# vita-epfl/motion-style-transfer

Hardware: AMD Instinct MI355X
Metric: trajectories/sec fwd+bwd (Y-Net+LoRA, SDD shortterm) (higher is better)
Workload: dtype f32; 1 GPU; C2: SDD shortterm Y-Net + LoRA rank=1 on encoder[0-4], 256x256 raster, obs=8 pred=12; batch_per_gpu=32, global_batch=32, raster=256x256, obs_len=8, pred_len=12, train_net=mosa_1, parallelism=dp1, trainable_floats=8190

## Files before the change

include/ynet_hip.h:

```cpp
#ifndef YNET_HIP_H
#define YNET_HIP_H

#ifdef __cplusplus
extern "C" {
#endif

int ynet_abi_version(void);
const char* ynet_last_error(void);

long long ynet_packed_weight_floats(int cout, int cin, int K, int mode);
int ynet_pack_weight(const float* w, float* wp, int cout, int cin, int K, int mode, void* stream);

long long ynet_conv2d_workspace_floats(int B, int H, int W, int cout);
int ynet_conv2d(const float* const* src, const int* src_c, const long long* src_bs, const int* src_bmod, int nsrc,
                const float* mask, long long mask_bs, const float* wp, const float* bias,
                float* const* dst, const int* dst_c, const long long* dst_bs, int ndst,
                int B, int H, int W, int K, int relu, float* workspace, long long workspace_floats,
                void* stream);
int ynet_conv2d_pool_supported(int B, int H, int W, int cout, int K);
int ynet_conv2d_pool(const float* const* src, const int* src_c, const long long* src_bs, int nsrc, const float* wp, const float* bias,
                     float* dst, int cout, long long dst_bs, float* pooled, long long pooled_bs,
                     int B, int H, int W, int K, int relu, void* stream);
int ynet_conv2d_dgrad_relu_supported(int B, int H, int W, int dx_c, int K);
int ynet_conv2d_dgrad_relu(const float* dy, int dy_c, long long dy_bs, const float* mask, long long mask_bs, const float* wp,
                           float* dx, int dx_c, long long dx_bs, const float* relu_of, long long relu_of_bs,
                           int B, int H, int W, int K, float* workspace, long long workspace_floats, void* stream);
int ynet_conv2d_add_supported(int B, int H, int W, int cout, int K);
int ynet_conv2d_add(const float* const* src, const int* src_c, const long long* src_bs, const int* src_bmod, int nsrc,
                    const float* wp, const float* bias, float* dst, int cout, long long dst_bs,
                    int B, int H, int W, int K, int relu, const float* addend, long long addend_bs, int addend_bmod,
                    void* stream);

long long ynet_conv2d_relu_bits_words(int B, int H, int W, int cout, int K);
int ynet_conv2d_relu_bits(const float* const* src, const int* src_c, const long long* src_bs, int nsrc, const float* wp, const float* bias,
                          float* dst, int cout, long long dst_bs, unsigned* bits, int B, int H, int W, int K, void* stream);
int ynet_conv2d_dgrad_relu_bits(const float* dy, int dy_c, long long dy_bs, const float* mask, long long mask_bs, const float* wp,
                                float* dx, int dx_c, long long dx_bs, const unsigned* bits, int B, int H, int W, int K, void* stream);

int ynet_conv2d_winograd_supported(int B, int H, int W, int cin, int cout, int K);
long long ynet_winograd_filter_floats(int cin, int cout);
int ynet_winograd_filter(const float* wp, float* u, int cin, int cout, int col0, int cols_total, void* stream);
int ynet_conv2d_winograd(const float* src, long long src_bs, const float* u, const float* bias, float* dst, long long dst_bs, int cin, int cout,
                         int B, int H, int W, int relu, void* stream);
int ynet_conv2d_winograd_s2d(const float* src, long long src_bs, const float* u, float* dst, long long dst_bs, int cin, int cout, int B, int H, int W, void* stream);
int ynet_conv2d_winograd_pred_bce_supported(int B, int H, int W, int cin, int cout, int pred_cout, int kernlen);
int ynet_conv2d_winograd_pred_bce_blob(const float* src, long long src_bs, const float* u, const float* bias, const float* pred_wp, const float* pred_bias, int pred_cout,
                                       const float* target_xy, const float* blob, int kernlen, int S, float* logits, float* loss, float* dx, long long dx_bs,
                                       void* workspace, int B, int H, int W, float expected_grad, void* stream);
int ynet_conv2d_winograd_split_supported(int B, int H, int W, int cin);
int ynet_conv2d_winograd_split(const float* src, long long src_bs, const float* u, float* dst0, long long dst0_bs, int dst0_s2d, float* dst1, long long dst1_bs, int cin,
                               int B, int H, int W, void* stream);
int ynet_conv2d_winograd_dgrad_relu(const float* dy, long long dy_bs, const float* u, float* dx, long long dx_bs, const float* relu_of, long long relu_of_bs,
                                    int dy_c, int dx_c, int B, int H, int W, void* stream);
int ynet_conv2d_winograd_cat_supported(int B, int H, int W, const int* src_c, int nsrc, int cout, int K);
long long ynet_winograd_filter_cat_floats(const int* src_c, int nsrc, int cout);
int ynet_winograd_filter_cat(const float* wp, float* u, const int* src_c, int nsrc, int cout, int col0, int cols_total, void* stream);
int ynet_conv2d_winograd_cat(const float* const* src, const int* src_c, const long long* src_bs, int nsrc, const float* u, const float* bias, float* dst,
                             long long dst_bs, int cout, int B, int H, int W, int relu, void* stream);
int ynet_conv2d_winograd_cat_add(const float* const* src, const int* src_c, const long long* src_bs, int nsrc, const float* u, const float* bias, float* dst,
                                 long long dst_bs, int cout, int B, int H, int W, int relu, const float* addend, long long addend_bs, int addend_bmod,
                                 void* stream);
int ynet_conv2d_winograd_cat_pool(const float* const* src, const int* src_c, const long long* src_bs, int nsrc, const float* u, const float* bias, float* dst,
                                  long long dst_bs, float* pooled, long long pooled_bs, int cout, int B, int H, int W, int relu, void* stream);
int ynet_conv2d_winograd_cat_pool_code(const float* const* src, const int* src_c, const long long* src_bs, int nsrc, const float* u, const float* bias, float* dst,
                                       long long dst_bs, float* pooled, long long pooled_bs, unsigned char* code, int B, int H, int W, void* stream);
long long ynet_winograd_relu_bits_words(int B, int H, int W);
int ynet_conv2d_winograd_relu_bits(const float* src, long long src_bs, const float* u, const float* bias, float* dst, long long dst_bs, int cin, int B, int H, int W,
                                   unsigned* bits_out, void* stream);
int ynet_conv2d_winograd_cat_relu_bits(const float* const* src, const int* src_c, const long long* src_bs, int nsrc, const float* u, const float* bias, float* dst,
                                       long long dst_bs, int B, int H, int W, const float* addend, long long addend_bs, int addend_bmod, unsigned* bits_out,
                                       void* stream);
int ynet_conv2d_winograd_dgrad_relu_bits(const float* dy, long long dy_bs, const float* u, float* dx, long long dx_bs, const unsigned* bits, int dy_c, int B, int H,
                                         int W, void* stream);
int ynet_conv2d_winograd16_supported(int B, int H, int W, const int* src_c, int nsrc, int cout, int K);
long long ynet_winograd16_filter_floats(const int* src_c, int nsrc, int cout);
int ynet_winograd16_filter(const float* wp, float* u, const int* src_c, int nsrc, int cout, int col0, int cols_total, void* stream);
int ynet_conv2d_winograd16(const float* const* src, const int* src_c, const long long* src_bs, int nsrc, const float* u, const float* bias, float* dst,
                           long long dst_bs, int cout, int B, int H, int W, int relu, const float* relu_of, long long relu_of_bs, const float* addend,
                           long long addend_bs, int addend_bmod, float* pooled, long long pooled_bs, void* stream);
int ynet_upsample2x_conv2d_winograd_supported(int B, int H, int W, int cin, int cout, int K);
int ynet_upsample2x_conv2d_winograd(const float* src, long long src_bs, const float* u, const float* bias, float* dst, long long dst_bs, int cin, int cout, int B,
                                    int H, int W, int relu, void* stream);

#define YNET_AUTO_NO_WINOGRAD 1u
#define YNET_AUTO_NO_WINOGRAD16 2u
#define YNET_AUTO_WINOGRAD16_FOR_16 4u
#define YNET_AUTO_NO_POOL_CODE 8u
#define YNET_AUTO_NO_RELU_WBITS 16u
#define YNET_AUTO_NO_SPLIT48 32u
#define YNET_AUTO_UPCONV_BWD 64u
typedef struct YnetConvAuto {
    const float* src[4];
    int src_c[4];
    long long src_bs[4];
    int src_bmod[4];
    int nsrc;
    const float* mask;
    long long mask_bs;
    const float* wp;
    const float* bias;
    float* dst[4];
    int dst_c[4];
    long long dst_bs[4];
    int ndst;
    int B, H, W, K, relu;
    int upsample2x;
    const float* relu_of;
    long long relu_of_bs;
    float* pooled;
    long long pooled_bs;
    unsigned char* pool_code;
    const float* addend;
    long long addend_bs;
    int addend_bmod;
    unsigned* bits_out;
    const unsigned* relu_bits;
    unsigned* wbits_out;
    const unsigned* relu_wbits;
    float* cache;
    long long cache_floats;
    unsigned long long* cache_tag;
    unsigned long long wp_version;
    float* workspace;
    long long workspace_floats;
    unsigned flags;
    int dst_s2d[4];
} YnetConvAuto;
typedef struct YnetConvTaken {
    int family;
    int variant;
    int nlaunch;
    int tmpl[4][3];
    int wrote_wbits, wrote_pool_code, transformed;
    int wrote_s2d;
} YnetConvTaken;
long long ynet_conv2d_auto_cache_floats(const YnetConvAuto* desc);
long long ynet_conv2d_auto_workspace_floats(const YnetConvAuto* desc);
int ynet_conv2d_auto(const YnetConvAuto* desc, YnetConvTaken* taken, void* stream);
int ynet_conv2d_auto_plan(const YnetConvAuto* desc, YnetConvTaken* taken);

long long ynet_upconv_tables_floats(int cout, int cin, long long* keff_floats, long long* table_floats);
int ynet_upconv_tables(const float* w, int cout, int cin, float* keff_packed, float* tables, void* stream);
int ynet_upconv_dgrad_ring(const float* D, long long d_bs, const float* tables, const float* relu_of, long long relu_of_bs, float* dx, long long dx_bs,
                           int B, int C4, int cin, int h, int w, void* stream);

int ynet_conv2d_plan(int B, int H, int W, int cout, int K);

long long ynet_conv2d_wgrad_workspace_floats(int B, int H, int W, int cout, int cin, int K);
int ynet_conv2d_wgrad(const float* const* src, const int* src_c, const long long* src_bs, int nsrc,
                      const float* dy, long long dy_bs, const float* mask, long long mask_bs,
                      float* dw, float* db, float* workspace, int B, int H, int W, int cout, int K,
                      void* stream);

int ynet_lora_compose(const float* w, const float* lora_a, const float* lora_b, float scale, float* w_eff,
                      int cout, int cin, int K, int r, void* stream);
int ynet_lora_grad(const float* dw, const float* lora_a, const float* lora_b, float scale, float* d_a, float* d_b,
                   int cout, int cin, int K, int r, void* stream);

int ynet_lora_compose_pack(const float* w, const float* lora_a, const float* lora_b, float scale, float* wp_fwd,
                           float* wp_dgrad, int cout, int cin, int K, int r, void* stream);
int ynet_lora_compose_pack_multi(int n, const float* const* w, const float* const* lora_a, const float* const* lora_b,
                                 const float* scale, float* const* wp_fwd, float* const* wp_dgrad, const int* cout,
                                 const int* cin, const int* K, const int* r, void* stream);

int ynet_lora_conv2d_wgrad_supported(int cin, int cout, int K, int r, int W);
int ynet_lora_conv2d_wgrad_preferred(int cin, int cout, int K, int r, int W);
long long ynet_lora_conv2d_wgrad_workspace_floats(int cin, int cout);
int ynet_lora_conv2d_wgrad(const float* const* src, const int* src_c, const long long* src_bs, int nsrc,
                           const float* dy, long long dy_batch_stride, const float* mask, long long mask_batch_stride,
                           const float* lora_a, const float* lora_b, float scale, float* d_a, float* d_b,
                           float* workspace, int B, int H, int W, int cout, int K, int r, void* stream);

int ynet_maxpool2_fwd(const float* x, float* y, long long N, int H, int W, void* stream);
int ynet_maxpool2_bwd(const float* x, const float* dy, float* dx, long long N, int H, int W, void* stream);
int ynet_maxpool2_bwd_add(const float* x, const float* dy, const float* add0, const float* add1, float* dx, long long N,
                          int H, int W, int relu_mask, void* stream);
int ynet_maxpool2_bwd_add_code(const unsigned char* code, const float* dy, const float* add0, const float* add1, float* dx, long long N, int H, int W,
                               int relu_mask, void* stream);
int ynet_upsample2x_fwd(const float* x, float* y, long long N, int H, int W, void* stream);
int ynet_upsample2x_bwd(const float* dy, float* dx, long long N, int H, int W, void* stream);
int ynet_upsample2x_bwd_relu(const float* dy, float* dx, const float* relu_of, long long N, int H, int W, void* stream);
int ynet_avgpool_pyramid(const float* x, float* const* outs, int nlev, long long N, int H, int W, void* stream);

long long ynet_batchnorm_workspace_doubles(int C);
int ynet_batchnorm2d_fwd(const float* x, float* y, const float* gamma, const float* beta, float* running_mean, float* running_var, float* save_mean, float* save_invstd,
                         double* workspace, int B, int C, long long HW, int train, double momentum, double eps, void* stream);
int ynet_batchnorm2d_bwd(const float* dy, const float* x, const float* mean, const float* invstd, const float* gamma, float* dx, float* dgamma, float* dbeta, double* workspace,
                         int B, int C, long long HW, int train, void* stream);
int ynet_add_relu(const float* a, const float* b, float* y, long long n, int relu, void* stream);
int ynet_relu_bwd(const float* dy, const float* y, float* dx, long long n, void* stream);

long long ynet_bce_workspace_bytes(void);
int ynet_bce_logits_fwd(const float* x, const float* t, long long n, float* loss, void* workspace, void* stream);
int ynet_bce_logits_bwd(const float* x, const float* t, const float* grad_out, float* dx, long long n, void* stream);
int ynet_bce_logits_fwd_grad(const float* x, const float* t, long long n, float expected_grad, float* loss, float* dx,
                             void* workspace, void* stream);
int ynet_bce_grad_rescale(float* dx, const float* grad_out, float expected_grad, long long n, void* stream);
// ... 78 lines not shown
```

motion-style-transfer_amd/_lib.py:

```python
import ctypes
import os
import re

_HERE = os.path.dirname(os.path.abspath(__file__))
LIB_PATH = os.environ.get("YNET_HIP_LIB") or os.path.join(_HERE, "csrc", "libynet_hip.so")
HEADER_PATH = os.path.join(os.path.dirname(_HERE), "include", "ynet_hip.h")

c_fp = ctypes.c_void_p
c_i = ctypes.c_int
c_ll = ctypes.c_longlong
c_f = ctypes.c_float
PP = ctypes.POINTER(ctypes.c_void_p)
PI = ctypes.POINTER(ctypes.c_int)
PLL = ctypes.POINTER(ctypes.c_longlong)

class ConvAuto(ctypes.Structure):
    _fields_ = [("src", c_fp * 4), ("src_c", c_i * 4), ("src_bs", c_ll * 4), ("src_bmod", c_i * 4), ("nsrc", c_i),
                ("mask", c_fp), ("mask_bs", c_ll), ("wp", c_fp), ("bias", c_fp),
                ("dst", c_fp * 4), ("dst_c", c_i * 4), ("dst_bs", c_ll * 4), ("ndst", c_i),
                ("B", c_i), ("H", c_i), ("W", c_i), ("K", c_i), ("relu", c_i), ("upsample2x", c_i),
                ("relu_of", c_fp), ("relu_of_bs", c_ll), ("pooled", c_fp), ("pooled_bs", c_ll), ("pool_code", c_fp),
                ("addend", c_fp), ("addend_bs", c_ll), ("addend_bmod", c_i),
                ("bits_out", c_fp), ("relu_bits", c_fp), ("wbits_out", c_fp), ("relu_wbits", c_fp),
                ("cache", c_fp), ("cache_floats", c_ll), ("cache_tag", ctypes.POINTER(ctypes.c_ulonglong)), ("wp_version", ctypes.c_ulonglong),
                ("workspace", c_fp), ("workspace_floats", c_ll), ("flags", ctypes.c_uint), ("dst_s2d", c_i * 4)]


class ConvTaken(ctypes.Structure):
    _fields_ = [("family", c_i), ("variant", c_i), ("nlaunch", c_i), ("tmpl", (c_i * 3) * 4), ("wrote_wbits", c_i), ("wrote_pool_code", c_i),
                ("transformed", c_i), ("wrote_s2d", c_i)]


AUTO_NO_WINOGRAD, AUTO_NO_WINOGRAD16, AUTO_WINOGRAD16_FOR_16, AUTO_NO_POOL_CODE, AUTO_NO_RELU_WBITS, AUTO_NO_SPLIT48 = 1, 2, 4, 8, 16, 32
AUTO_UPCONV_BWD = 64

SIGNATURES = {
    "ynet_abi_version": (c_i, []),
    "ynet_last_error": (ctypes.c_char_p, []),
    "ynet_packed_weight_floats": (c_ll, [c_i, c_i, c_i, c_i]),
    "ynet_pack_weight": (c_i, [c_fp, c_fp, c_i, c_i, c_i, c_i, c_fp]),
    "ynet_conv2d_workspace_floats": (c_ll, [c_i, c_i, c_i, c_i]),
    "ynet_conv2d": (c_i, [PP, PI, PLL, PI, c_i, c_fp, c_ll, c_fp, c_fp, PP, PI, PLL, c_i,
                          c_i, c_i, c_i, c_i, c_i, c_fp, c_ll, c_fp]),
    "ynet_conv2d_pool_supported": (c_i, [c_i, c_i, c_i, c_i, c_i]),
    "ynet_conv2d_pool": (c_i, [PP, PI, PLL, c_i, c_fp, c_fp, c_fp, c_i, c_ll, c_fp, c_ll, c_i, c_i, c_i, c_i, c_i, c_fp]),
    "ynet_conv2d_dgrad_relu_supported": (c_i, [c_i, c_i, c_i, c_i, c_i]),
    "ynet_conv2d_dgrad_relu": (c_i, [c_fp, c_i, c_ll, c_fp, c_ll, c_fp, c_fp, c_i, c_ll, c_fp, c_ll, c_i, c_i, c_i, c_i, c_fp, c_ll, c_fp]),
    "ynet_conv2d_relu_bits_words": (c_ll, [c_i, c_i, c_i, c_i, c_i]),
    "ynet_conv2d_relu_bits": (c_i, [PP, PI, PLL, c_i, c_fp, c_fp, c_fp, c_i, c_ll, c_fp, c_i, c_i, c_i, c_i, c_fp]),
    "ynet_conv2d_dgrad_relu_bits": (c_i, [c_fp, c_i, c_ll, c_fp, c_ll, c_fp, c_fp, c_i, c_ll, c_fp, c_i, c_i, c_i, c_i, c_fp]),
    "ynet_conv2d_winograd_supported": (c_i, [c_i, c_i, c_i, c_i, c_i, c_i]),
    "ynet_winograd_filter_floats": (c_ll, [c_i, c_i]),
    "ynet_winograd_filter": (c_i, [c_fp, c_fp, c_i, c_i, c_i, c_i, c_fp]),
    "ynet_conv2d_winograd": (c_i, [c_fp, c_ll, c_fp, c_fp, c_fp, c_ll, c_i, c_i, c_i, c_i, c_i, c_i, c_fp]),
    "ynet_conv2d_winograd_s2d": (c_i, [c_fp, c_ll, c_fp, c_fp, c_ll, c_i, c_i, c_i, c_i, c_i, c_fp]),
    "ynet_conv2d_winograd_pred_bce_supported": (c_i, [c_i, c_i, c_i, c_i, c_i, c_i, c_i]),
    "ynet_conv2d_winograd_pred_bce_blob": (c_i, [c_fp, c_ll, c_fp, c_fp, c_fp, c_fp, c_i, c_fp, c_fp, c_i, c_i, c_fp, c_fp, c_fp, c_ll, c_fp, c_i, c_i, c_i,
                                                 c_f, c_fp]),
    "ynet_conv2d_winograd_split_supported": (c_i, [c_i, c_i, c_i, c_i]),
    "ynet_conv2d_winograd_split": (c_i, [c_fp, c_ll, c_fp, c_fp, c_ll, c_i, c_fp, c_ll, c_i, c_i, c_i, c_i, c_fp]),
    "ynet_upconv_dgrad_ring": (c_i, [c_fp, c_ll, c_fp, c_fp, c_ll, c_fp, c_ll, c_i, c_i, c_i, c_i, c_i, c_fp]),
    "ynet_upconv_tables_floats": (c_ll, [c_i, c_i, PLL, PLL]),
    "ynet_upconv_tables": (c_i, [c_fp, c_i, c_i, c_fp, c_fp, c_fp]),
    "ynet_conv2d_winograd_dgrad_relu": (c_i, [c_fp, c_ll, c_fp, c_fp, c_ll, c_fp, c_ll, c_i, c_i, c_i, c_i, c_i, c_fp]),
    "ynet_conv2d_winograd_cat_supported": (c_i, [c_i, c_i, c_i, PI, c_i, c_i, c_i]),
    "ynet_winograd_filter_cat_floats": (c_ll, [PI, c_i, c_i]),
    "ynet_winograd_filter_cat": (c_i, [c_fp, c_fp, PI, c_i, c_i, c_i, c_i, c_fp]),
    "ynet_conv2d_winograd_cat": (c_i, [PP, PI, PLL, c_i, c_fp, c_fp, c_fp, c_ll, c_i, c_i, c_i, c_i, c_i, c_fp]),
    "ynet_conv2d_winograd_cat_add": (c_i, [PP, PI, PLL, c_i, c_fp, c_fp, c_fp, c_ll, c_i, c_i, c_i, c_i, c_i, c_fp, c_ll, c_i, c_fp]),
    "ynet_conv2d_winograd_cat_pool": (c_i, [PP, PI, PLL, c_i, c_fp, c_fp, c_fp, c_ll, c_fp, c_ll, c_i, c_i, c_i, c_i, c_i, c_fp]),
    "ynet_conv2d_winograd_cat_pool_code": (c_i, [PP, PI, PLL, c_i, c_fp, c_fp, c_fp, c_ll, c_fp, c_ll, c_fp, c_i, c_i, c_i, c_fp]),
    "ynet_winograd_relu_bits_words": (c_ll, [c_i, c_i, c_i]),
    "ynet_conv2d_winograd_relu_bits": (c_i, [c_fp, c_ll, c_fp, c_fp, c_fp, c_ll, c_i, c_i, c_i, c_i, c_fp, c_fp]),
    "ynet_conv2d_winograd_cat_relu_bits": (c_i, [PP, PI, PLL, c_i, c_fp, c_fp, c_fp, c_ll, c_i, c_i, c_i, c_fp, c_ll, c_i, c_fp, c_fp]),
    "ynet_conv2d_winograd_dgrad_relu_bits": (c_i, [c_fp, c_ll, c_fp, c_fp, c_ll, c_fp, c_i, c_i, c_i, c_i, c_fp]),
    "ynet_upsample2x_conv2d_winograd_supported": (c_i, [c_i, c_i, c_i, c_i, c_i, c_i]),
    "ynet_upsample2x_conv2d_winograd": (c_i, [c_fp, c_ll, c_fp, c_fp, c_fp, c_ll, c_i, c_i, c_i, c_i, c_i, c_i, c_fp]),
    "ynet_conv2d_winograd16_supported": (c_i, [c_i, c_i, c_i, PI, c_i, c_i, c_i]),
    "ynet_winograd16_filter_floats": (c_ll, [PI, c_i, c_i]),
    "ynet_winograd16_filter": (c_i, [c_fp, c_fp, PI, c_i, c_i, c_i, c_i, c_fp]),
    "ynet_conv2d_winograd16": (c_i, [PP, PI, PLL, c_i, c_fp, c_fp, c_fp, c_ll, c_i, c_i, c_i, c_i, c_i, c_fp, c_ll, c_fp, c_ll, c_i, c_fp, c_ll, c_fp]),
    "ynet_conv2d_auto_cache_floats": (c_ll, [ctypes.POINTER(ConvAuto)]),
    "ynet_conv2d_auto_workspace_floats": (c_ll, [ctypes.POINTER(ConvAuto)]),
    "ynet_conv2d_auto": (c_i, [ctypes.POINTER(ConvAuto), ctypes.POINTER(ConvTaken), c_fp]),
    "ynet_conv2d_auto_plan": (c_i, [ctypes.POINTER(ConvAuto), ctypes.POINTER(ConvTaken)]),
    "ynet_conv2d_add_supported": (c_i, [c_i, c_i, c_i, c_i, c_i]),
    "ynet_conv2d_add": (c_i, [PP, PI, PLL, PI, c_i, c_fp, c_fp, c_fp, c_i, c_ll, c_i, c_i, c_i, c_i, c_i, c_fp, c_ll, c_i, c_fp]),
    "ynet_conv2d_plan": (c_i, [c_i, c_i, c_i, c_i, c_i]),
    "ynet_conv2d_wgrad_workspace_floats": (c_ll, [c_i, c_i, c_i, c_i, c_i, c_i]),
    "ynet_conv2d_wgrad": (c_i, [PP, PI, PLL, c_i, c_fp, c_ll, c_fp, c_ll, c_fp, c_fp, c_fp,
                                c_i, c_i, c_i, c_i, c_i, c_fp]),
    "ynet_lora_compose": (c_i, [c_fp, c_fp, c_fp, c_f, c_fp, c_i, c_i, c_i, c_i, c_fp]),
    "ynet_lora_grad": (c_i, [c_fp, c_fp, c_fp, c_f, c_fp, c_fp, c_i, c_i, c_i, c_i, c_fp]),
    "ynet_lora_conv2d_wgrad_supported": (c_i, [c_i, c_i, c_i, c_i, c_i]),
    "ynet_lora_conv2d_wgrad_preferred": (c_i, [c_i, c_i, c_i, c_i, c_i]),
    "ynet_lora_conv2d_wgrad_workspace_floats": (c_ll, [c_i, c_i]),
    "ynet_lora_conv2d_wgrad": (c_i, [PP, PI, PLL, c_i, c_fp, c_ll, c_fp, c_ll, c_fp, c_fp, c_f, c_fp, c_fp, c_fp,
                                     c_i, c_i, c_i, c_i, c_i, c_i, c_fp]),
    "ynet_lora_compose_pack": (c_i, [c_fp, c_fp, c_fp, c_f, c_fp, c_fp, c_i, c_i, c_i, c_i, c_fp]),
    "ynet_lora_compose_pack_multi": (c_i, [c_i, PP, PP, PP, ctypes.POINTER(c_f), PP, PP, PI, PI, PI, PI, c_fp]),
    "ynet_batch_sum": (c_i, [c_fp, c_fp, c_i, c_ll, c_ll, c_fp]),
    "ynet_adam_step": (c_i, [c_fp, c_fp, c_fp, c_i, c_i, ctypes.c_double, ctypes.c_double, ctypes.c_double, ctypes.c_double, ctypes.c_double,
                             c_i, c_fp]),
    "ynet_maxpool2_fwd": (c_i, [c_fp, c_fp, c_ll, c_i, c_i, c_fp]),
    "ynet_maxpool2_bwd": (c_i, [c_fp, c_fp, c_fp, c_ll, c_i, c_i, c_fp]),
    "ynet_maxpool2_bwd_add": (c_i, [c_fp, c_fp, c_fp, c_fp, c_fp, c_ll, c_i, c_i, c_i, c_fp]),
    "ynet_maxpool2_bwd_add_code": (c_i, [c_fp, c_fp, c_fp, c_fp, c_fp, c_ll, c_i, c_i, c_i, c_fp]),
    "ynet_upsample2x_fwd": (c_i, [c_fp, c_fp, c_ll, c_i, c_i, c_fp]),
# ... 86 lines not shown
```

motion-style-transfer_amd/csrc/conv_auto.cpp:

```cpp
#include "ynet_common.h"
#include "../../include/ynet_hip.h"
#include <stdint.h>
#include <string.h>

namespace {

struct Piece {
    float* ptr;
    int n;
    long long bs;
    int col0;
    int dst;
    int whole;
};

enum Kind { K_NONE = 0, K_WINO = 1, K_CAT = 2, K_W16 = 3 };

struct Launch {
    int kind;
    int row0;
    int cs[4], ncs;
    int cout, col0, ctot;
    long long floats;
    long long offset;
// ... 344 lines not shown
    if (a->flags & YNET_AUTO_UPCONV_BWD) return run_upconv_bwd(a, taken, stream);
    YNET_REQUIRE(a->nsrc >= 1 && a->nsrc <= 4 && a->ndst >= 1 && a->ndst <= 4 && a->wp, "conv2d_auto: 1..4 sources, 1..4 destinations and a packed filter are required");
    YNET_REQUIRE(a->B > 0 && a->H > 0 && a->W > 0 && (a->K == 1 || a->K == 3 || a->K == 5), "conv2d_auto: bad shape B %d %dx%d K %d", a->B, a->H, a->W, a->K);
    Plan p;
    if (int rc = make_plan(a, p)) return rc;
    YnetConvTaken t;
    memset(&t, 0, sizeof(t));
    t.family = p.family;
    t.variant = p.variant;
    if (p.nl) {
        YNET_REQUIRE(a->cache && a->cache_tag && a->cache_floats >= p.cache_floats && al(a->cache, 16),
                     "conv2d_auto: this launch keeps %lld floats of transformed filters (ynet_conv2d_auto_cache_floats): pass a 16-byte aligned cache of that size and its tag", p.cache_floats);
        const unsigned long long sig = signature(p);
        if (a->cache_tag[0] != sig || a->cache_tag[1] != a->wp_version) {
            if (int rc = transform(a, p, stream)) return rc;
            a->cache_tag[0] = sig;
            a->cache_tag[1] = a->wp_version;
            t.transformed = 1;
        }
    }
    return run_plan(a, p, t, taken, stream);
}

}

namespace {

int run_plan(const YnetConvAuto* a, const Plan& p, YnetConvTaken t, YnetConvTaken* taken, void* stream) {
    const int B = a->B, H = a->H, W = a->W, K = a->K, relu = a->relu ? 1 : 0;
    int ctot = 0;
    for (int i = 0; i < a->ndst; ++i) ctot += a->dst_c[i];
    const float* u0 = p.nl ? a->cache + p.l[0].offset : nullptr;
    const float* u1 = p.nl > 1 ? a->cache + p.l[1].offset : nullptr;
    auto done = [&](int rc) {
        if (!rc && taken) *taken = t;
        return rc;
    };
    auto tag = [&](int i, int x, int y, int z) {
        if (i < 4) { t.tmpl[i][0] = x; t.tmpl[i][1] = y; t.tmpl[i][2] = z; }
        t.nlaunch = i + 1;
    };
    float* ws = a->workspace_floats > 0 ? a->workspace : nullptr;
    const long long nws = ws ? a->workspace_floats : 0;

    switch (p.family) {
    case 4:
    case 5:
        tag(0, p.family == 4 ? 4 : 0, 0, 0);
        return done(ynet_upsample2x_conv2d_winograd(a->src[0], a->src_bs[0], u0, a->bias, a->dst[0], a->dst_bs[0], a->src_c[0], ctot, B, H, W, relu, stream));
    case 1: {
        if (p.variant == 23) {
            const Piece &q0 = p.pieces[0], &q1 = p.pieces[1];
            const int s2d = a->dst_s2d[q0.dst] ? 1 : 0;
            const int rc = ynet_conv2d_winograd_split(a->src[0], a->src_bs[0], u0, q0.ptr, q0.bs, s2d, q1.ptr, q1.bs, a->src_c[0], B, H, W, stream);
            if (rc) return rc;
            if (s2d) t.wrote_s2d |= 1 << q0.dst;
            tag(0, 3, a->src_c[0] / 8, s2d ? 6 : 5);
            return done(0);
        }
        const bool one32 = p.npieces == 1 && p.pieces[0].n == 32;
        unsigned* wb_out = (one32 && relu && !a->relu_of && !(a->flags & YNET_AUTO_NO_RELU_WBITS)) ? a->wbits_out : nullptr;
        const unsigned* wb_in = (one32 && a->relu_of && !relu && !a->bias && !(a->flags & YNET_AUTO_NO_RELU_WBITS)) ? a->relu_wbits : nullptr;
        const int em = wb_out ? 3 : (wb_in ? 2 : (a->relu_of ? 1 : 0));
        for (int i = 0; i < p.npieces; ++i) {
            const Piece& q = p.pieces[i];
            const float* u = a->cache + p.l[i].offset;
            const float* bias = a->bias ? a->bias + q.col0 : nullptr;
            int rc;
            const bool s2d = a->dst_s2d[q.dst] && q.whole && em == 0 && !a->bias && !relu;
            if (s2d) {
                rc = ynet_conv2d_winograd_s2d(a->src[0], a->src_bs[0], u, q.ptr, q.bs, a->src_c[0], q.n, B, H, W, stream);
                if (rc) return rc;
                t.wrote_s2d |= 1 << q.dst;
                tag(i, q.n / 16, a->src_c[0] / 8, 4);
                continue;
            }
            if (wb_out) rc = ynet_conv2d_winograd_relu_bits(a->src[0], a->src_bs[0], u, bias, q.ptr, q.bs, a->src_c[0], B, H, W, wb_out, stream);
            else if (wb_in) rc = ynet_conv2d_winograd_dgrad_relu_bits(a->src[0], a->src_bs[0], u, q.ptr, q.bs, wb_in, a->src_c[0], B, H, W, stream);
            else if (a->relu_of) {
                YNET_REQUIRE(!a->bias && !relu, "conv2d_auto: relu_of is for a data gradient (no bias, no ReLU)");
                rc = ynet_conv2d_winograd_dgrad_relu(a->src[0], a->src_bs[0], u, q.ptr, q.bs, a->relu_of, a->relu_of_bs, a->src_c[0], q.n, B, H, W, stream);
            } else rc = ynet_conv2d_winograd(a->src[0], a->src_bs[0], u, bias, q.ptr, q.bs, a->src_c[0], q.n, B, H, W, relu, stream);
            if (rc) return rc;
            tag(i, q.n / 16, a->src_c[0] / 8, em);
        }
        t.wrote_wbits = wb_out ? 1 : 0;
        return done(0);
    }
    case 2: {
        if (p.variant == 30) {
            unsigned* wb = (relu && !(a->flags & YNET_AUTO_NO_RELU_WBITS)) ? a->wbits_out : nullptr;
            tag(0, 2, wb ? 5 : 2, 0);
            t.wrote_wbits = wb ? 1 : 0;
            if (wb) return done(ynet_conv2d_winograd_cat_relu_bits(a->src, a->src_c, a->src_bs, a->nsrc, u0, a->bias, a->dst[0], a->dst_bs[0], B, H, W, a->addend, a->addend_bs, a->addend_bmod, wb, stream));
            return done(ynet_conv2d_winograd_cat_add(a->src, a->src_c, a->src_bs, a->nsrc, u0, a->bias, a->dst[0], a->dst_bs[0], 32, B, H, W, relu, a->addend, a->addend_bs, a->addend_bmod, stream));
        }
        if (p.variant == 10) {
            unsigned char* code = (relu && !(a->flags & YNET_AUTO_NO_POOL_CODE)) ? a->pool_code : nullptr;
            tag(0, 2, code ? 6 : 3, 0);
            t.wrote_pool_code = code ? 1 : 0;
            if (code) return done(ynet_conv2d_winograd_cat_pool_code(a->src, a->src_c, a->src_bs, a->nsrc, u0, a->bias, a->dst[0], a->dst_bs[0], a->pooled, a->pooled_bs, code, B, H, W, stream));
            return done(ynet_conv2d_winograd_cat_pool(a->src, a->src_c, a->src_bs, a->nsrc, u0, a->bias, a->dst[0], a->dst_bs[0], a->pooled, a->pooled_bs, 32, B, H, W, relu, stream));
        }
        unsigned* wb = (relu && !(a->flags & YNET_AUTO_NO_RELU_WBITS)) ? a->wbits_out : nullptr;
        t.wrote_wbits = wb ? 1 : 0;
        if (p.variant == 40) {
            const long long HW = (long long)H * W;
            int rc = ynet_conv2d_winograd(a->src[0], a->src_bs[0], u0, nullptr, a->dst[0], a->dst_bs[0], 32, 32, B, H, W, 0, stream);
            if (rc) return rc;
            const float* rs[4];
            int rc_[4], nr = 0;
            long long rb[4];
            if (a->src_c[0] > 32) { rs[nr] = a->src[0] + 32 * HW; rc_[nr] = a->src_c[0] - 32; rb[nr] = a->src_bs[0]; ++nr; }
            for (int i = 1; i < a->nsrc; ++i) { rs[nr] = a->src[i]; rc_[nr] = a->src_c[i]; rb[nr] = a->src_bs[i]; ++nr; }
            tag(0, 2, 4, 0);
            tag(1, 2, wb ? 5 : 2, 0);
            if (wb) return done(ynet_conv2d_winograd_cat_relu_bits(rs, rc_, rb, nr, u1, a->bias, a->dst[0], a->dst_bs[0], B, H, W, a->dst[0], a->dst_bs[0], 0, wb, stream));
            return done(ynet_conv2d_winograd_cat_add(rs, rc_, rb, nr, u1, a->bias, a->dst[0], a->dst_bs[0], 32, B, H, W, relu, a->dst[0], a->dst_bs[0], 0, stream));
        }
        tag(0, 2, wb ? 4 : 0, 0);
        if (wb) return done(ynet_conv2d_winograd_cat_relu_bits(a->src, a->src_c, a->src_bs, a->nsrc, u0, a->bias, a->dst[0], a->dst_bs[0], B, H, W, nullptr, 0, 0, wb, stream));
        return done(ynet_conv2d_winograd_cat(a->src, a->src_c, a->src_bs, a->nsrc, u0, a->bias, a->dst[0], a->dst_bs[0], 32, B, H, W, relu, stream));
    }
    case 3: {
// ... 63 lines not shown
                 !a->relu_wbits && !a->dst_s2d[0] && a->src_bmod[0] <= 0,
                 "conv2d_auto (upconv_bwd): relu_of is the only optional operand (no upsample2x, pooled, pool_code, addend, mask, bias, relu, bit masks, dst_s2d, batch modulus)");
    YNET_REQUIRE(a->K == 3 && a->src_c[0] >= 4 && (a->src_c[0] & 3) == 0 && a->dst_c[0] >= 1, "conv2d_auto (upconv_bwd): K 3, src_c[0] = 4 cout, dst_c[0] = cin (K %d, src_c %d, dst_c %d)",
                 a->K, a->src_c[0], a->dst_c[0]);
    YNET_REQUIRE(a->B > 0 && a->H >= 2 && a->W >= 2, "conv2d_auto (upconv_bwd): the low-resolution map must be at least 2 x 2 (B %d, %dx%d)", a->B, a->H, a->W);
    const int c4 = a->src_c[0], cin = a->dst_c[0];
    const long long hw = (long long)a->H * a->W;
    YNET_REQUIRE(a->src_bs[0] >= c4 * hw && a->dst_bs[0] >= cin * hw && (!a->relu_of || a->relu_of_bs >= cin * hw), "conv2d_auto (upconv_bwd): batch strides smaller than the images");
    YNET_REQUIRE((3ll * c4 * cin + c4 * 66ll + 256) * 4 <= 64 * 1024, "conv2d_auto (upconv_bwd): 4 cout %d x cin %d ring tables do not fit the ring kernel's LDS", c4, cin);
    memset(&u, 0, sizeof(u));
    u.cout = c4 / 4;
    u.cin = cin;
    long long kf = 0, tf = 0;
    YNET_REQUIRE(ynet_upconv_tables_floats(u.cout, cin, &kf, &tf) > 0, "conv2d_auto (upconv_bwd): bad shape cout %d cin %d", u.cout, cin);
    u.tab_off = (kf + 3) & ~3ll;
    u.wino_off = u.tab_off + ((tf + 3) & ~3ll);
    u.in = *a;
    u.in.flags &= ~YNET_AUTO_UPCONV_BWD;
    u.in.wp = a->cache;
    u.in.cache = a->cache ? a->cache + u.wino_off : nullptr;
    u.in.cache_floats = a->cache_floats - u.wino_off;
    u.in.cache_tag = nullptr;
    if (int rc = make_plan(&u.in, u.p)) return rc;
    u.cache_floats = u.wino_off + u.p.cache_floats;
    return 0;
}

int run_upconv_bwd(const YnetConvAuto* a, YnetConvTaken* taken, void* stream) {
    UpPlan u;
    if (int rc = make_up_plan(a, u)) return rc;
    YNET_REQUIRE(a->wp && a->src[0] && a->dst[0], "conv2d_auto (upconv_bwd): the raw filter [cout][cin][3][3], the source and the destination are required");
    YNET_REQUIRE(a->cache && a->cache_tag && a->cache_floats >= u.cache_floats && al(a->cache, 16),
                 "conv2d_auto (upconv_bwd): this call keeps %lld floats of effective filter, ring tables and transforms (ynet_conv2d_auto_cache_floats): pass a 16-byte aligned cache "
                 "of that size and its tag", u.cache_floats);
    YnetConvTaken t;
    memset(&t, 0, sizeof(t));
    t.family = u.p.family;
    t.variant = u.p.variant;
    unsigned long long sig = signature(u.p);
    for (long long v : {0x7570636f6e76ll, (long long)u.cout, (long long)u.cin}) {
        sig ^= (unsigned long long)v;
        sig *= 1099511628211ull;
    }
    sig = sig ? sig : 1;
    if (a->cache_tag[0] != sig || a->cache_tag[1] != a->wp_version) {
        if (int rc = ynet_upconv_tables(a->wp, u.cout, u.cin, a->cache, a->cache + u.tab_off, stream)) return rc;
        if (int rc = transform(&u.in, u.p, stream)) return rc;
        a->cache_tag[0] = sig;
        a->cache_tag[1] = a->wp_version;
        t.transformed = 1;
    }
    YnetConvTaken ti;
    if (int rc = run_plan(&u.in, u.p, t, &ti, stream)) return rc;
    if (int rc = ynet_upconv_dgrad_ring(a->src[0], a->src_bs[0], a->cache + u.tab_off, a->relu_of, a->relu_of_bs, a->dst[0], a->dst_bs[0], a->B, 4 * u.cout, u.cin, a->H, a->W,
                                        stream))
        return rc;
    ti.nlaunch += 1;
    if (taken) *taken = ti;
    return 0;
}

}
```

motion-style-transfer_amd/csrc/conv_wino.hip:

```cpp
#include "ynet_common.h"
#include "bce_element.h"
#include <math.h>
#include <stdlib.h>
#include <type_traits>

typedef float f32x2 __attribute__((ext_vector_type(2)));
typedef unsigned u32x2 __attribute__((ext_vector_type(2)));
typedef __attribute__((address_space(3))) void* lds_ptr_t;

#define WN_TH 16
#define WN_TW 32
#define WN_LQ 10
#define WN_ROWF 40
#define WN_PLANE_F 160
#define WN_SLOT_BYTES (320 * 16 + 16)
#define WN_RING_BYTES (2 * WN_SLOT_BYTES)
#define WN_THREADS 512

struct WinoArgs {
    const float* x;
    const f32x4* u;
    const float* bias;
    float* y;
    long long x_bs, y_bs;
    int B, H, W, relu, ntiles;
    const float* emask;
    long long emask_bs;
    unsigned* wbits;
    float* y2;
    long long y2_bs;
    const float* pw;
    const float* pb;
    int pco, pco_pad;
    const float* t_xy;
    const float* t_blob;
    int t_m, t_S;
    float* logits;
    double* partial;
    unsigned* ticket;
    float* loss;
    long long n_loss;
    float gs;
};

__device__ __forceinline__ f32x2 wn_v01(f32x2 tl, f32x2 th) {
    f32x2 r;
    asm("v_pk_add_f32 %0, %1, %2 op_sel_hi:[1,0] neg_lo:[0,1]" : "=v"(r) : "v"(tl), "v"(th));
    return r;
}
__device__ __forceinline__ f32x2 wn_v23(f32x2 tl, f32x2 th) {
    f32x2 r;
    asm("v_pk_add_f32 %0, %1, %2 op_sel:[1,0] op_sel_hi:[1,1] neg_lo:[1,0] neg_hi:[0,1]" : "=v"(r) : "v"(tl), "v"(th));
    return r;
}

template <int NCB, int EPI, int BITS = 0, bool S2D = false, int CB0 = 0, int CB1 = NCB>
__device__ __forceinline__ void wino_epilogue(f32x4 (&acc)[16][NCB], const f32x2 (&bias2)[NCB][2], float floor_v, __amdgpu_buffer_rsrc_t ry,
                                              __amdgpu_buffer_rsrc_t rm, unsigned st0, unsigned st1, unsigned so_t, unsigned sm_t, int HW, unsigned stp = 0,
                                              unsigned* wbits = nullptr, unsigned char* pcode = nullptr) {
    unsigned word = 0u;
    if constexpr (BITS == 2) word = *wbits;
#pragma unroll
    for (int cb = CB0; cb < CB1; ++cb) {
        constexpr int NB = CB1 - CB0;
        const int cd = cb - CB0;
        u32x2 mk[2][2][2];
        if constexpr (EPI == 1 || EPI == 2) {
#pragma unroll
            for (int h = 0; h < 2; ++h)
#pragma unroll
                for (int k = 0; k < 2; ++k) {
                    const unsigned sm = sm_t + (unsigned)((cd * 16 + 2 * h + k) * HW * 4);
                    mk[h][k][0] = __builtin_amdgcn_raw_buffer_load_b64(rm, st0, sm, 0);
                    mk[h][k][1] = __builtin_amdgcn_raw_buffer_load_b64(rm, st1, sm, 0);
                }
        }
#pragma unroll
        for (int h = 0; h < 2; ++h) {
            f32x2 m[16];
#pragma unroll
            for (int e = 0; e < 16; ++e)
                m[e] = h == 0 ? __builtin_shufflevector(acc[e][cb], acc[e][cb], 0, 1) : __builtin_shufflevector(acc[e][cb], acc[e][cb], 2, 3);
            m[5] = m[5] + bias2[cb][h];
            f32x2 r0[4], r1[4];
#pragma unroll
            for (int j = 0; j < 4; ++j) {
                r0[j] = m[j] + m[4 + j] + m[8 + j];
                r1[j] = m[4 + j] - m[8 + j] - m[12 + j];
            }
            const f32x2 o00 = r0[0] + r0[1] + r0[2], o01 = r0[1] - r0[2] - r0[3];
            const f32x2 o10 = r1[0] + r1[1] + r1[2], o11 = r1[1] - r1[2] - r1[3];
#pragma unroll
            for (int k = 0; k < 2; ++k) {
                f32x2 row0 = {o00[k], o01[k]}, row1 = {o10[k], o11[k]};
                if constexpr (EPI == 2) {
                    row0 += __builtin_bit_cast(f32x2, mk[h][k][0]);
                    row1 += __builtin_bit_cast(f32x2, mk[h][k][1]);
                }
                row0 = f32x2{row0[0] < floor_v ? floor_v : row0[0], row0[1] < floor_v ? floor_v : row0[1]};
                row1 = f32x2{row1[0] < floor_v ? floor_v : row1[0], row1[1] < floor_v ? floor_v : row1[1]};
                if constexpr (EPI == 1) {
                    const f32x2 m0 = __builtin_bit_cast(f32x2, mk[h][k][0]), m1 = __builtin_bit_cast(f32x2, mk[h][k][1]);
                    row0 = f32x2{m0[0] > 0.f ? row0[0] : 0.f, m0[1] > 0.f ? row0[1] : 0.f};
                    row1 = f32x2{m1[0] > 0.f ? row1[0] : 0.f, m1[1] > 0.f ? row1[1] : 0.f};
                }
                const int bit0 = ((cb * 2 + h) * 2 + k) * 4;
                if constexpr (BITS == 2) {
                    row0 = f32x2{(word >> bit0) & 1u ? row0[0] : 0.f, (word >> (bit0 + 1)) & 1u ? row0[1] : 0.f};
                    row1 = f32x2{(word >> (bit0 + 2)) & 1u ? row1[0] : 0.f, (word >> (bit0 + 3)) & 1u ? row1[1] : 0.f};
                }
                if constexpr (BITS == 1)
                    word |= (row0[0] > 0.f ? 1u << bit0 : 0u) | (row0[1] > 0.f ? 2u << bit0 : 0u) | (row1[0] > 0.f ? 4u << bit0 : 0u) | (row1[1] > 0.f ? 8u << bit0 : 0u);
                if constexpr (S2D) {
                    const unsigned hw = (unsigned)(HW >> 2), ph = (unsigned)(NB * 16) * hw * 4u;
                    const unsigned sc = so_t + (unsigned)(cd * 16 + 2 * h + k) * hw * 4u;
                    const float e00 = row0[0], e01 = row0[1], e10 = row1[0], e11 = row1[1];
                    const bool odd = __lane_id() & 1u;
                    const float g0 = __builtin_bit_cast(float, __builtin_amdgcn_update_dpp(0, __builtin_bit_cast(int, odd ? e00 : e01), 0xB1, 0xF, 0xF, false));
                    const float g1 = __builtin_bit_cast(float, __builtin_amdgcn_update_dpp(0, __builtin_bit_cast(int, odd ? e10 : e11), 0xB1, 0xF, 0xF, false));
                    const f32x2 p0 = odd ? f32x2{g0, e01} : f32x2{e00, g0}, p1 = odd ? f32x2{g1, e11} : f32x2{e10, g1};
                    const unsigned vo = st0 + (odd ? ph - 4u : 0u);
                    __builtin_amdgcn_raw_buffer_store_b64(__builtin_bit_cast(u32x2, p0), ry, vo, sc, 0);
                    __builtin_amdgcn_raw_buffer_store_b64(__builtin_bit_cast(u32x2, p1), ry, vo, sc + 2u * ph, 0);
                    continue;
                }
                const unsigned so = so_t + (unsigned)((cd * 16 + 2 * h + k) * HW * 4);
                __builtin_amdgcn_raw_buffer_store_b64(__builtin_bit_cast(u32x2, row0), ry, st0, so, 0);
                __builtin_amdgcn_raw_buffer_store_b64(__builtin_bit_cast(u32x2, row1), ry, st1, so, 0);
                if constexpr (EPI == 3) {
                    float pm = fmaxf(fmaxf(row0[0], row0[1]), fmaxf(row1[0], row1[1]));
                    if (__builtin_isunordered(row0[0], row0[1]) || __builtin_isunordered(row1[0], row1[1])) pm = __builtin_nanf("");
                    __builtin_amdgcn_raw_buffer_store_b32(__builtin_bit_cast(unsigned, pm), rm, stp, sm_t + (unsigned)((cd * 16 + 2 * h + k) * (HW >> 2) * 4), 0);
                    if constexpr (BITS == 3) {
                        float mx = row0[0];
                        unsigned arg = 0u;
                        if (row0[1] > mx || row0[1] != row0[1]) { mx = row0[1]; arg = 1u; }
                        if (row1[0] > mx || row1[0] != row1[0]) { mx = row1[0]; arg = 2u; }
                        if (row1[1] > mx || row1[1] != row1[1]) { mx = row1[1]; arg = 3u; }
                        const unsigned code = arg | (row0[0] > 0.f ? 4u : 0u) | (row0[1] > 0.f ? 8u : 0u) | (row1[0] > 0.f ? 16u : 0u) | (row1[1] > 0.f ? 32u : 0u);
                        pcode[(cd * 16 + 2 * h + k) * (HW >> 2)] = (unsigned char)code;
                    }
                }
            }
        }
    }
    if constexpr (BITS == 1) *wbits = word;
}

template <int MB, typename PosT>
__device__ __forceinline__ float wino_epilogue_pred(f32x4 (&acc)[16][2], const f32x2 (&bias2)[2][2], const f32x4* tab,
                                                    const WinoArgs& a, __amdgpu_buffer_rsrc_t rdx, __amdgpu_buffer_rsrc_t rlog, unsigned st_rm, unsigned so_rm, int b,
                                                    int py0, int px0, int kq, int H, int W, const float* blob_tab, const PosT* pos_lds) {
    const int HW = H * W;
    float yv[2][4][4];
#pragma unroll
    for (int cb = 0; cb < 2; ++cb)
#pragma unroll
        for (int h = 0; h < 2; ++h) {
            f32x2 m[16];
#pragma unroll
            for (int e = 0; e < 16; ++e)
                m[e] = h == 0 ? __builtin_shufflevector(acc[e][cb], acc[e][cb], 0, 1) : __builtin_shufflevector(acc[e][cb], acc[e][cb], 2, 3);
            m[5] = m[5] + bias2[cb][h];
            f32x2 r0[4], r1[4];
#pragma unroll
            for (int j = 0; j < 4; ++j) {
                r0[j] = m[j] + m[4 + j] + m[8 + j];
                r1[j] = m[4 + j] - m[8 + j] - m[12 + j];
            }
            const f32x2 o00 = r0[0] + r0[1] + r0[2], o01 = r0[1] - r0[2] - r0[3];
            const f32x2 o10 = r1[0] + r1[1] + r1[2], o11 = r1[1] - r1[2] - r1[3];
#pragma unroll
            for (int k = 0; k < 2; ++k) {
                const float v00 = o00[k], v01 = o01[k], v10 = o10[k], v11 = o11[k];
                yv[cb][2 * h + k][0] = v00 < 0.f ? 0.f : v00;
                yv[cb][2 * h + k][1] = v01 < 0.f ? 0.f : v01;
// ... 257 lines not shown
#pragma unroll
        for (int c = 0; c < NCH; ++c) {
            if (c + 1 < NCH || nxt < total_units) asm volatile("s_waitcnt vmcnt(5)" ::: "memory");
            else asm volatile("s_waitcnt vmcnt(0)" ::: "memory");
            const f32x4* wl = smem + c * WQ;
            const float* il = reinterpret_cast<const float*>(reinterpret_cast<const unsigned char*>(smem) + NCH * WQ * 16 + wave * WN_RING_BYTES +
                                                             (c & 1) * WN_SLOT_BYTES + 4);
#pragma unroll
            for (int s = 0; s < 2; ++s) {
                const float* ip = il + (s * 4 + kq) * WN_PLANE_F + 3 + 2 * n;
                f32x2 dl[4], dh[4];
#pragma unroll
                for (int r = 0; r < 4; ++r) {
                    dl[r] = *reinterpret_cast<const f32x2*>(ip + r * WN_ROWF);
                    dh[r] = *reinterpret_cast<const f32x2*>(ip + r * WN_ROWF + 2);
                }
                if (s == 1) {
                    asm volatile("s_waitcnt lgkmcnt(0)" ::: "memory");
                    if (c + 2 < NCH) dma_chunk(cur, c + 2);
                    else if (nxt < total_units) dma_chunk(nxt, c + 2 - NCH);
                }
                const f32x2 tl[4] = {dl[0] - dl[2], dl[1] + dl[2], dl[2] - dl[1], dl[1] - dl[3]};
                const f32x2 th[4] = {dh[0] - dh[2], dh[1] + dh[2], dh[2] - dh[1], dh[1] - dh[3]};
                f32x2 v01[4], v23[4];
#pragma unroll
                for (int i = 0; i < 4; ++i) {
                    v01[i] = wn_v01(tl[i], th[i]);
                    v23[i] = wn_v23(tl[i], th[i]);
                }
                asm volatile("s_nop 3" : "+v"(v01[0]), "+v"(v01[1]), "+v"(v01[2]), "+v"(v01[3]), "+v"(v23[0]), "+v"(v23[1]), "+v"(v23[2]), "+v"(v23[3]));
#pragma unroll
                for (int q = 0; q < 4; ++q) {
                    f32x4 w[NCB];
#pragma unroll
                    for (int cb = 0; cb < NCB; ++cb) w[cb] = wl[((s * 4 + q) * NCB + cb) * 64 + lane];
#pragma unroll
                    for (int e = 0; e < 4; ++e) {
                        const float bv = e < 2 ? v01[q][e] : v23[q][e - 2];
#pragma unroll
                        for (int cb = 0; cb < NCB; ++cb) {
                            const float av = w[cb][e];
                            if (c == 0 && s == 0) acc[q * 4 + e][cb] = __builtin_amdgcn_mfma_f32_16x16x4f32(av, bv, f32x4{0.f, 0.f, 0.f, 0.f}, 0, 0, 0);
                            else acc[q * 4 + e][cb] = __builtin_amdgcn_mfma_f32_16x16x4f32(av, bv, acc[q * 4 + e][cb], 0, 0, 0);
                        }
                    }
                }
            }
        }
        {
            const int t = tile_first + (cur >> 3) * gstride;
            const int tx = t % tiles_x, ty = (t / tiles_x) % tiles_y, b = t / (tiles_x * tiles_y);
            const unsigned so_s2d = (unsigned)(((ty * (WN_TH / 2) + (cur & 7)) * (W >> 1) + tx * (WN_TW / 2)) * 4);
            const unsigned so_rm = (unsigned)(((ty * WN_TH + 2 * (cur & 7)) * W + tx * WN_TW) * 4);
            if constexpr (EM == 7 || EM == 8) {
                static_assert((EM != 7 && EM != 8) || NCB == 2, "the predictor epilogue is the 32-channel launch's");
                const __amdgpu_buffer_rsrc_t rdx = __builtin_amdgcn_make_buffer_rsrc(a.y + (long long)b * a.y_bs, 0, y_img, 0x00020000);
                const __amdgpu_buffer_rsrc_t rlog =
                    __builtin_amdgcn_make_buffer_rsrc(a.logits + (long long)b * a.pco * HW, 0, (unsigned)(a.pco * HW * 4), 0x00020000);
                typedef typename std::conditional<EM == 7, int, short>::type PosT;
                const float* blob_lds = reinterpret_cast<const float*>(ptab + 5 * PMB * 64) + 2 * NW + 4;
                const float s_ = wino_epilogue_pred<PMB, PosT>(acc, bias2, ptab + lane, a, rdx, rlog, st_rm, so_rm, b, ty * WN_TH + 2 * (cur & 7), tx * WN_TW + 2 * n, kq, H, W,
                                                               blob_lds, reinterpret_cast<const PosT*>(blob_lds + a.t_m * a.t_m));
                acc_loss += (double)s_;
                cur = nxt;
                if (cur < total_units) nxt = next_unit();
                continue;
            }
            if constexpr (EM == 5 || EM == 6) {
                static_assert(EM < 5 || NCB == 3, "the two-destination epilogue is the 48-channel launch's");
                const __amdgpu_buffer_rsrc_t r0 = __builtin_amdgcn_make_buffer_rsrc(a.y + (long long)b * a.y_bs, 0, (unsigned)(16 * HW * 4), 0x00020000);
                const __amdgpu_buffer_rsrc_t r1 = __builtin_amdgcn_make_buffer_rsrc(a.y2 + (long long)b * a.y2_bs, 0, (unsigned)(32 * HW * 4), 0x00020000);
                if constexpr (EM == 6) wino_epilogue<NCB, 0, 0, true, 0, 1>(acc, bias2, floor_v, r0, r0, st_s2d, st_s2d, so_s2d, so_s2d, HW);
                else wino_epilogue<NCB, 0, 0, false, 0, 1>(acc, bias2, floor_v, r0, r0, st_rm, st_rm + (unsigned)(W * 4), so_rm, so_rm, HW);
                wino_epilogue<NCB, 0, 0, false, 1, 3>(acc, bias2, floor_v, r1, r1, st_rm, st_rm + (unsigned)(W * 4), so_rm, so_rm, HW);
                cur = nxt;
                if (cur < total_units) nxt = next_unit();
                continue;
            }
            const unsigned so_t = EM == 4 ? so_s2d : so_rm;
            const __amdgpu_buffer_rsrc_t ry = __builtin_amdgcn_make_buffer_rsrc(a.y + (long long)b * a.y_bs, 0, y_img, 0x00020000);
            const __amdgpu_buffer_rsrc_t rm =
                __builtin_amdgcn_make_buffer_rsrc(const_cast<float*>(EM == 1 ? a.emask + (long long)b * a.emask_bs : a.y), 0, y_img, 0x00020000);
            unsigned* wb = (EM == 2 || EM == 3) ? a.wbits + (((long long)b * (H >> 1) + (ty * (WN_TH / 2) + (cur & 7))) * tiles_x + tx) * 64 + lane : nullptr;
            wino_epilogue<NCB, EM == 1 ? 1 : 0, EM == 2 ? 2 : (EM == 3 ? 1 : 0), EM == 4>(acc, bias2, floor_v, ry, rm, st0, st1, so_t, so_t, HW, 0, wb);
        }
        cur = nxt;
        if (cur < total_units) nxt = next_unit();
    }
    if constexpr (EM == 7 || EM == 8) {
        double* wsd = reinterpret_cast<double*>(ptab + 5 * PMB * 64);
        unsigned* last = reinterpret_cast<unsigned*>(wsd + NW);
#pragma unroll
        for (int o = 32; o > 0; o >>= 1) acc_loss += __shfl_xor(acc_loss, o, 64);
        if (lane == 0) wsd[wave] = acc_loss;
        __syncthreads();
        if (tid == 0) {
            double t = 0.0;
            for (int i = 0; i < NW; ++i) t += wsd[i];
            a.partial[blockIdx.x] = t;
            __threadfence();
            *last = (atomicAdd(a.ticket, 1u) == gridDim.x - 1) ? 1u : 0u;
        }
        __syncthreads();
        if (*last) {
            __threadfence();
            double t = 0.0;
            for (unsigned i = tid; i < gridDim.x; i += NT) t += ((volatile double*)a.partial)[i];
#pragma unroll
            for (int o = 32; o > 0; o >>= 1) t += __shfl_xor(t, o, 64);
            if (lane == 0) wsd[wave] = t;
            __syncthreads();
            if (tid == 0) {
                double tt = 0.0;
                for (int i = 0; i < NW; ++i) tt += wsd[i];
                a.loss[0] = (float)(tt / (double)a.n_loss);
                *a.ticket = 0u;
            }
        }
    }
}

#define WC_SLOT_BYTES (160 * 16 + 16)
#define WC_RING_BYTES (2 * WC_SLOT_BYTES)
#define WC_MAX_SRC 3

struct WinoCatArgs {
    const float* x[WC_MAX_SRC];
    long long x_bs[WC_MAX_SRC];
    int x_c[WC_MAX_SRC];
    int nsrc, nchunks;
    const f32x4* u;
    const float* bias;
    float* y;
    long long y_bs;
    int B, H, W, relu, ntiles;
    const float* addend;
    long long addend_bs;
// ... 853 lines not shown
    static int cus_dev[YNET_MAX_DEV] = {0};
    const int slot = ynet_device_slot();
    if (!attr_dev[slot]) {
        (void)hipFuncSetAttribute(reinterpret_cast<const void*>(conv_wino_cat_kernel<2, 0>), hipFuncAttributeMaxDynamicSharedMemorySize, 14 * 8192 + 8 * WC_RING_BYTES + 16);
        (void)hipFuncSetAttribute(reinterpret_cast<const void*>(conv_wino_cat_kernel<2, 2>), hipFuncAttributeMaxDynamicSharedMemorySize, 14 * 8192 + 8 * WC_RING_BYTES + 16);
        (void)hipFuncSetAttribute(reinterpret_cast<const void*>(conv_wino_cat_kernel<2, 3>), hipFuncAttributeMaxDynamicSharedMemorySize, 14 * 8192 + 8 * WC_RING_BYTES + 16);
        (void)hipFuncSetAttribute(reinterpret_cast<const void*>(conv_wino_cat_kernel<2, 4>), hipFuncAttributeMaxDynamicSharedMemorySize, 14 * 8192 + 8 * WC_RING_BYTES + 16);
        (void)hipFuncSetAttribute(reinterpret_cast<const void*>(conv_wino_cat_kernel<2, 5>), hipFuncAttributeMaxDynamicSharedMemorySize, 14 * 8192 + 8 * WC_RING_BYTES + 16);
        (void)hipFuncSetAttribute(reinterpret_cast<const void*>(conv_wino_cat_kernel<2, 6>), hipFuncAttributeMaxDynamicSharedMemorySize, 14 * 8192 + 8 * WC_RING_BYTES + 16);
        int dev = 0, cus = 256;
        (void)hipGetDevice(&dev);
        (void)hipDeviceGetAttribute(&cus, hipDeviceAttributeMultiprocessorCount, dev);
        cus_dev[slot] = cus < 8 ? 8 : cus;
        attr_dev[slot] = true;
    }
    int grid = a.ntiles < cus_dev[slot] ? a.ntiles : cus_dev[slot];
    if (grid >= 8) grid &= ~7;
    if (wbits != nullptr && addend != nullptr) hipLaunchKernelGGL((conv_wino_cat_kernel<2, 5>), dim3(grid), dim3(WN_THREADS), lds, (hipStream_t)stream, a);
    else if (wbits != nullptr) hipLaunchKernelGGL((conv_wino_cat_kernel<2, 4>), dim3(grid), dim3(WN_THREADS), lds, (hipStream_t)stream, a);
    else if (addend != nullptr) hipLaunchKernelGGL((conv_wino_cat_kernel<2, 2>), dim3(grid), dim3(WN_THREADS), lds, (hipStream_t)stream, a);
    else if (pcode != nullptr) hipLaunchKernelGGL((conv_wino_cat_kernel<2, 6>), dim3(grid), dim3(WN_THREADS), lds, (hipStream_t)stream, a);
    else if (pool != nullptr) hipLaunchKernelGGL((conv_wino_cat_kernel<2, 3>), dim3(grid), dim3(WN_THREADS), lds, (hipStream_t)stream, a);
    else hipLaunchKernelGGL((conv_wino_cat_kernel<2, 0>), dim3(grid), dim3(WN_THREADS), lds, (hipStream_t)stream, a);
    return ynet_check_launch(what);
}

int ynet_conv2d_winograd_cat(const float* const* src, const int* src_c, const long long* src_bs, int nsrc, const float* u, const float* bias, float* dst,
                             long long dst_bs, int cout, int B, int H, int W, int relu, void* stream) {
    return wino_cat_launch(src, src_c, src_bs, nsrc, u, bias, dst, dst_bs, cout, B, H, W, relu, nullptr, 0, 0, nullptr, 0, stream, "conv2d_winograd_cat");
}

int ynet_conv2d_winograd_cat_add(const float* const* src, const int* src_c, const long long* src_bs, int nsrc, const float* u, const float* bias, float* dst,
                                 long long dst_bs, int cout, int B, int H, int W, int relu, const float* addend, long long addend_bs, int addend_bmod,
                                 void* stream) {
    YNET_REQUIRE(addend != nullptr, "conv2d_winograd_cat_add: the additive term is null");
    return wino_cat_launch(src, src_c, src_bs, nsrc, u, bias, dst, dst_bs, cout, B, H, W, relu, addend, addend_bs, addend_bmod, nullptr, 0, stream, "conv2d_winograd_cat_add");
}

int ynet_conv2d_winograd_cat_pool(const float* const* src, const int* src_c, const long long* src_bs, int nsrc, const float* u, const float* bias, float* dst,
                                  long long dst_bs, float* pooled, long long pooled_bs, int cout, int B, int H, int W, int relu, void* stream) {
    YNET_REQUIRE(pooled != nullptr, "conv2d_winograd_cat_pool: the pooled output is null");
    return wino_cat_launch(src, src_c, src_bs, nsrc, u, bias, dst, dst_bs, cout, B, H, W, relu, nullptr, 0, 0, pooled, pooled_bs, stream, "conv2d_winograd_cat_pool");
}

int ynet_conv2d_winograd_cat_pool_code(const float* const* src, const int* src_c, const long long* src_bs, int nsrc, const float* u, const float* bias, float* dst,
                                       long long dst_bs, float* pooled, long long pooled_bs, unsigned char* code, int B, int H, int W, void* stream) {
    YNET_REQUIRE(pooled != nullptr && code != nullptr, "conv2d_winograd_cat_pool_code: the pooled output or its code plane is null");
    return wino_cat_launch(src, src_c, src_bs, nsrc, u, bias, dst, dst_bs, 32, B, H, W, 1, nullptr, 0, 0, pooled, pooled_bs, stream, "conv2d_winograd_cat_pool_code",
                           nullptr, code);
}

static int wino_launch_any(const float* src, long long src_bs, const float* u, const float* bias, float* dst, long long dst_bs, const float* emask,
                           long long emask_bs, int cin, int cout, int B, int H, int W, int relu, void* stream, const char* what, unsigned* wbits = nullptr,
                           bool wbits_apply = false, bool s2d = false, float* dst2 = nullptr, long long dst2_bs = 0, int split_mode = 0) {
    YNET_REQUIRE(src && u && dst, "%s: null pointer", what);
    YNET_REQUIRE(wino_shape_ok(B, H, W, cin, cout, 3), "%s: shape B=%d %dx%d %d -> %d is not served (ask ynet_conv2d_winograd_supported)", what, B, H, W, cin,
                 cout);
    YNET_REQUIRE((reinterpret_cast<uintptr_t>(src) & 15) == 0 && (reinterpret_cast<uintptr_t>(dst) & 7) == 0 && (reinterpret_cast<uintptr_t>(u) & 15) == 0 &&
                     (src_bs & 3) == 0 && (dst_bs & 1) == 0,
                 "%s: planes must be 16-byte (input, filters) / 8-byte (output) aligned", what);
    const long long HW = (long long)H * W;
    YNET_REQUIRE((src_bs == 0 || src_bs >= cin * HW) && dst_bs >= (split_mode ? 16 : cout) * HW, "%s: batch strides smaller than the images (input: 0 = one image for the batch)", what);
    if (split_mode)
        YNET_REQUIRE(cout == 48 && dst2 != nullptr && (reinterpret_cast<uintptr_t>(dst2) & 7) == 0 && (dst2_bs & 1) == 0 && dst2_bs >= 32 * HW && bias == nullptr && !relu &&
                         wbits == nullptr && !s2d,
                     "%s: two destinations are for the plain 48-channel data gradient (16 + 32 planes, 8-byte aligned)", what);
    if (emask != nullptr)
        YNET_REQUIRE((reinterpret_cast<uintptr_t>(emask) & 7) == 0 && (emask_bs & 1) == 0 && emask_bs >= cout * HW,
                     "%s: the activation must be 8-byte aligned, its batch stride not smaller than the image", what);
    WinoArgs a{src, reinterpret_cast<const f32x4*>(u), bias, dst, src_bs, dst_bs, B, H, W, relu ? 1 : 0, B * (H / WN_TH) * (W / WN_TW), emask, emask_bs, wbits, dst2, dst2_bs};
    hipStream_t st = (hipStream_t)stream;
    if (wbits != nullptr) {
        YNET_REQUIRE(cout == 32 && emask == nullptr && (reinterpret_cast<uintptr_t>(wbits) & 3) == 0, "%s: the 1-bit mask serves 32 output channels and excludes the float mask", what);
        if (wbits_apply) return cin == 32 ? launch_wino<2, 4, 2>(a, st) : launch_wino<2, 2, 2>(a, st);
        return cin == 32 ? launch_wino<2, 4, 3>(a, st) : launch_wino<2, 2, 3>(a, st);
    }
    if (s2d) {
        YNET_REQUIRE(emask == nullptr && bias == nullptr && !relu, "%s: the space-to-depth store is for a plain data gradient", what);
        if (cout == 32) return cin == 32 ? launch_wino<2, 4, 4>(a, st) : launch_wino<2, 2, 4>(a, st);
        return cin == 32 ? launch_wino<1, 4, 4>(a, st) : launch_wino<1, 2, 4>(a, st);
    }
    if (cout == 48) {
        YNET_REQUIRE(emask == nullptr && cin == 32, "%s: the 48-channel form is plain, from 32 input channels", what);
        if (split_mode == 1) return launch_wino_nw<3, 4, 5, 4>(a, st);
        if (split_mode == 2) return launch_wino_nw<3, 4, 6, 4>(a, st);
        return launch_wino_nw<3, 4, 0, 4>(a, st);
    }
    if (emask != nullptr) {
        if (cout == 32) return cin == 32 ? launch_wino<2, 4, 1>(a, st) : launch_wino<2, 2, 1>(a, st);
        return cin == 32 ? launch_wino<1, 4, 1>(a, st) : launch_wino<1, 2, 1>(a, st);
    }
    if (cout == 32) return cin == 32 ? launch_wino<2, 4, 0>(a, st) : launch_wino<2, 2, 0>(a, st);
    return cin == 32 ? launch_wino<1, 4, 0>(a, st) : launch_wino<1, 2, 0>(a, st);
}

int ynet_conv2d_winograd(const float* src, long long src_bs, const float* u, const float* bias, float* dst, long long dst_bs, int cin, int cout,
                         int B, int H, int W, int relu, void* stream) {
    return wino_launch_any(src, src_bs, u, bias, dst, dst_bs, nullptr, 0, cin, cout, B, H, W, relu, stream, "conv2d_winograd");
}

int ynet_conv2d_winograd_s2d(const float* src, long long src_bs, const float* u, float* dst, long long dst_bs, int cin, int cout, int B, int H, int W, void* stream) {
    return wino_launch_any(src, src_bs, u, nullptr, dst, dst_bs, nullptr, 0, cin, cout, B, H, W, 0, stream, "conv2d_winograd_s2d", nullptr, false, true);
}

int ynet_conv2d_winograd_pred_bce_supported(int B, int H, int W, int cin, int cout, int pred_cout, int kernlen) {
    static const int on = getenv("YNET_CONV_PRED_BCE") ? atoi(getenv("YNET_CONV_PRED_BCE")) : 1;
    if (!(on && cin == 32 && cout == 32 && pred_cout >= 1 && pred_cout <= 32 && kernlen >= 1 && wino_shape_ok(B, H, W, cin, cout, 3))) return 0;
    const long long base = 4ll * 8 * 2 * 64 * 16 + 8ll * WN_RING_BYTES + 16 + 8 * 8 + 16;
    const long long lds = pred_cout <= 16 ? base + 5 * 64 * 16 + ((long long)kernlen * kernlen + 2ll * B * pred_cout) * 4
                                          : base + 10 * 64 * 16 + (long long)kernlen * kernlen * 4 + ((2ll * B * pred_cout * 2 + 15) & ~15ll);
    return lds <= 160 * 1024 ? 1 : 0;
}

int ynet_conv2d_winograd_pred_bce_blob(const float* src, long long src_bs, const float* u, const float* bias, const float* pred_wp, const float* pred_bias, int pred_cout,
                                       const float* target_xy, const float* blob, int kernlen, int S, float* logits, float* loss, float* dx, long long dx_bs,
                                       void* workspace, int B, int H, int W, float expected_grad, void* stream) {
    YNET_REQUIRE(src && u && pred_wp && target_xy && blob && logits && loss && dx && workspace, "conv2d_winograd_pred_bce_blob: null pointer");
    YNET_REQUIRE(ynet_conv2d_winograd_pred_bce_supported(B, H, W, 32, 32, pred_cout, kernlen), "conv2d_winograd_pred_bce_blob: B=%d %dx%d with %d predictor outputs and a %d x %d blob is not served (32 -> 32, <= 32 outputs, tables within LDS; ask ..._supported)",
                 B, H, W, pred_cout, kernlen, kernlen);
    YNET_REQUIRE(kernlen > 0 && kernlen <= S && S >= H && S >= W, "conv2d_winograd_pred_bce_blob: the target needs a blob table with 0 < kernlen <= S and S >= H, W (got kernlen %d, S %d, %dx%d)", kernlen, S, H, W);
    const long long HW = (long long)H * W;
    YNET_REQUIRE((reinterpret_cast<uintptr_t>(src) & 15) == 0 && (reinterpret_cast<uintptr_t>(u) & 15) == 0 && (reinterpret_cast<uintptr_t>(dx) & 7) == 0 &&
                     (reinterpret_cast<uintptr_t>(logits) & 7) == 0 && (src_bs & 3) == 0 && (dx_bs & 1) == 0 && (src_bs == 0 || src_bs >= 32 * HW) && dx_bs >= 32 * HW,
                 "conv2d_winograd_pred_bce_blob: planes must be 16-byte (input, filters) / 8-byte (outputs) aligned, batch strides not smaller than the images");
    WinoArgs a{src, reinterpret_cast<const f32x4*>(u), bias, dx, src_bs, dx_bs, B, H, W, 1, B * (H / WN_TH) * (W / WN_TW), nullptr, 0, nullptr, nullptr, 0};
    a.pw = pred_wp;
    a.pb = pred_bias;
    a.pco = pred_cout;
    a.pco_pad = ceil_div(pred_cout, 64) * 64;
    a.t_xy = target_xy;
    a.t_blob = blob;
    a.t_m = kernlen;
    a.t_S = S;
    a.logits = logits;
    a.partial = (double*)workspace;
    a.ticket = (unsigned*)((char*)workspace + 1024 * sizeof(double));
    a.loss = loss;
    a.n_loss = (long long)B * pred_cout * HW;
    a.gs = expected_grad / (float)a.n_loss;
    return pred_cout <= 16 ? launch_wino_nw<2, 4, 7, 8>(a, (hipStream_t)stream) : launch_wino_nw<2, 4, 8, 8>(a, (hipStream_t)stream);
}

int ynet_conv2d_winograd_split_supported(int B, int H, int W, int cin) { return (cin == 32 && wino_shape_ok(B, H, W, cin, 48, 3)) ? 1 : 0; }

int ynet_conv2d_winograd_split(const float* src, long long src_bs, const float* u, float* dst0, long long dst0_bs, int dst0_s2d, float* dst1, long long dst1_bs, int cin,
                               int B, int H, int W, void* stream) {
    return wino_launch_any(src, src_bs, u, nullptr, dst0, dst0_bs, nullptr, 0, cin, 48, B, H, W, 0, stream, "conv2d_winograd_split", nullptr, false, false, dst1, dst1_bs,
                           dst0_s2d ? 2 : 1);
}

long long ynet_winograd_relu_bits_words(int B, int H, int W) {
    if (B <= 0 || H % WN_TH || W % WN_TW) return 0;
    return (long long)B * (H / 2) * (W / WN_TW) * 64;
}

int ynet_conv2d_winograd_relu_bits(const float* src, long long src_bs, const float* u, const float* bias, float* dst, long long dst_bs, int cin, int B, int H,
                                   int W, unsigned* bits_out, void* stream) {
    YNET_REQUIRE(bits_out != nullptr, "conv2d_winograd_relu_bits: the mask output is null");
    return wino_launch_any(src, src_bs, u, bias, dst, dst_bs, nullptr, 0, cin, 32, B, H, W, 1, stream, "conv2d_winograd_relu_bits", bits_out, false);
}

int ynet_conv2d_winograd_cat_relu_bits(const float* const* src, const int* src_c, const long long* src_bs, int nsrc, const float* u, const float* bias, float* dst,
                                       long long dst_bs, int B, int H, int W, const float* addend, long long addend_bs, int addend_bmod, unsigned* bits_out,
                                       void* stream) {
    YNET_REQUIRE(bits_out != nullptr, "conv2d_winograd_cat_relu_bits: the mask output is null");
    return wino_cat_launch(src, src_c, src_bs, nsrc, u, bias, dst, dst_bs, 32, B, H, W, 1, addend, addend_bs, addend_bmod, nullptr, 0, stream,
                           "conv2d_winograd_cat_relu_bits", bits_out);
}

int ynet_conv2d_winograd_dgrad_relu_bits(const float* dy, long long dy_bs, const float* u, float* dx, long long dx_bs, const unsigned* bits, int dy_c, int B, int H,
                                         int W, void* stream) {
    YNET_REQUIRE(bits != nullptr, "conv2d_winograd_dgrad_relu_bits: the mask is null");
    return wino_launch_any(dy, dy_bs, u, nullptr, dx, dx_bs, nullptr, 0, dy_c, 32, B, H, W, 0, stream, "conv2d_winograd_dgrad_relu_bits", const_cast<unsigned*>(bits), true);
}

int ynet_conv2d_winograd_dgrad_relu(const float* dy, long long dy_bs, const float* u, float* dx, long long dx_bs, const float* relu_of, long long relu_of_bs,
                                    int dy_c, int dx_c, int B, int H, int W, void* stream) {
    YNET_REQUIRE(relu_of != nullptr, "conv2d_winograd_dgrad_relu: the activation whose ReLU backward is applied is null");
    return wino_launch_any(dy, dy_bs, u, nullptr, dx, dx_bs, relu_of, relu_of_bs, dy_c, dx_c, B, H, W, 0, stream, "conv2d_winograd_dgrad_relu");
}

}

static bool wino16_ok(int B, int H, int W, const int* src_c, int nsrc, int cout, int K) {
    static const int on = getenv("YNET_WINOGRAD") ? atoi(getenv("YNET_WINOGRAD")) : 1;
    static const int on16 = getenv("YNET_WINOGRAD16") ? atoi(getenv("YNET_WINOGRAD16")) : 1;
    if (!on || !on16 || K != 3 || B <= 0 || nsrc < 1 || nsrc > WC_MAX_SRC) return false;
    if (cout != 16 && cout != 32 && cout != 64 && cout != 128) return false;
    if (H % W6_TH || W % WN_TW || H < W6_TH || W < WN_TW) return false;
    for (int i = 0; i < nsrc; ++i)
        if (src_c[i] <= 0) return false;
    const int nch = wino_cat_padded(src_c, nsrc) / 4;
    if (nch < 2 || nch > W6_MAX_CHUNKS) return false;
    if (84ll * H * W * 4 + (W + 4) * 4 >= (1ll << 31)) return false;
    static const int min_pixels = getenv("YNET_WINOGRAD16_MIN") ? atoi(getenv("YNET_WINOGRAD16_MIN")) : (getenv("YNET_WINOGRAD_MIN") ? atoi(getenv("YNET_WINOGRAD_MIN")) : 64 * 64 * 10);
    return (long long)B * H * W >= min_pixels;
}

extern "C" {

int ynet_conv2d_winograd16_supported(int B, int H, int W, const int* src_c, int nsrc, int cout, int K) {
// ... 168 lines not shown
```

motion-style-transfer_amd/csrc/glue.hip:

```cpp
#include "ynet_common.h"
#include "bce_element.h"
#include <stdlib.h>

static inline dim3 plane_grid(long long planes, long long per_plane) {
    long long gx = (per_plane + 255) / 256;
    if (gx > 4096) gx = 4096;
    long long gy = planes < 65535 ? planes : 65535;
    while (gx * gy > (1ll << 22) && gy > 1) gy = (gy + 1) / 2;
    return dim3((unsigned)gx, (unsigned)gy);
}

static inline int grid_for(long long n, int block, int cap = 2048 * 4) {
    long long g = (n + block - 1) / block;
    if (g > cap) g = cap;
    if (g < 1) g = 1;
    return (int)g;
}

__global__ void maxpool2_fwd_kernel(const float* __restrict__ x, float* __restrict__ y, long long N, int H, int W) {
    const int Ho = H >> 1, Wo = W >> 1, per_plane = Ho * Wo;
    for (long long n = blockIdx.y; n < N; n += gridDim.y)
        for (int i = blockIdx.x * 256 + threadIdx.x; i < per_plane; i += gridDim.x * 256) {
            const int yo = i / Wo, xo = i - yo * Wo;
            const float* p = x + (n * H + 2 * yo) * W + 2 * xo;
// ... 1194 lines not shown
    if (running_mean) running_mean[c] = (float)((1.0 - momentum) * (double)running_mean[c] + momentum * m);
    if (running_var) running_var[c] = (float)((1.0 - momentum) * (double)running_var[c] + momentum * (n > 1.0 ? var * n / (n - 1.0) : var));
}

__global__ void bn_invstd_kernel(const float* __restrict__ running_var, float* invstd, int C, double eps) {
    const int c = blockIdx.x * blockDim.x + threadIdx.x;
    if (c < C) invstd[c] = (float)(1.0 / sqrt((double)running_var[c] + eps));
}

__global__ __launch_bounds__(256) void bn_apply_kernel(const float* __restrict__ x, const float* __restrict__ mean, const float* __restrict__ invstd,
                                                       const float* __restrict__ gamma, const float* __restrict__ beta, float* __restrict__ y, long long planes, int C,
                                                       long long HW) {
    const long long plane = blockIdx.y;
    if (plane >= planes) return;
    const int c = (int)(plane % C);
    const float m = mean[c], sc = invstd[c] * (gamma ? gamma[c] : 1.f), sh = beta ? beta[c] : 0.f;
    for (long long p = blockIdx.x * 256ll + threadIdx.x; p < HW; p += (long long)gridDim.x * 256) y[plane * HW + p] = (x[plane * HW + p] - m) * sc + sh;
}

__global__ __launch_bounds__(256) void bn_bwd_kernel(const float* __restrict__ dy, const float* __restrict__ x, const float* __restrict__ mean, const float* __restrict__ invstd,
                                                     const float* __restrict__ gamma, const double* __restrict__ partial, float* __restrict__ dx, float* dgamma, float* dbeta,
                                                     long long planes, int C, long long HW, double n, int train) {
    const long long plane = blockIdx.y;
    if (plane >= planes) return;
    const int c = (int)(plane % C);
    double s0 = 0.0, s1 = 0.0;
    if (partial) {
        for (int p = 0; p < BN_PARTS; ++p) { s0 += partial[2 * (c * BN_PARTS + p)]; s1 += partial[2 * (c * BN_PARTS + p) + 1]; }
        if (plane < C && blockIdx.x == 0 && threadIdx.x == 0) {
            if (dgamma) dgamma[c] = (float)s1;
            if (dbeta) dbeta[c] = (float)s0;
        }
    }
    const float m = mean[c], is = invstd[c], g = (gamma ? gamma[c] : 1.f) * is;
    const float mdy = train ? (float)(s0 / n) : 0.f, mdx = train ? (float)(s1 / n) : 0.f;
    for (long long p = blockIdx.x * 256ll + threadIdx.x; p < HW; p += (long long)gridDim.x * 256) {
        const float gy = dy[plane * HW + p];
        dx[plane * HW + p] = train ? g * (gy - mdy - (x[plane * HW + p] - m) * is * mdx) : g * gy;
    }
}

__global__ __launch_bounds__(256) void add_relu_kernel(const float* __restrict__ a, const float* __restrict__ b, float* __restrict__ y, long long n, int relu) {
    for (long long i = blockIdx.x * 256ll + threadIdx.x; i < n; i += (long long)gridDim.x * 256) {
        const float v = a[i] + b[i];
        y[i] = relu ? (v < 0.f ? 0.f : v) : v;
    }
}

__global__ __launch_bounds__(256) void relu_bwd_kernel(const float* __restrict__ dy, const float* __restrict__ y, float* __restrict__ dx, long long n) {
    for (long long i = blockIdx.x * 256ll + threadIdx.x; i < n; i += (long long)gridDim.x * 256) dx[i] = y[i] > 0.f ? dy[i] : 0.f;
}

#define RING_SEG 64
__global__ __launch_bounds__(256) void upconv_ring_kernel(const float* __restrict__ D, long long d_bs, const float* __restrict__ tab, const float* __restrict__ relu_of,
                                                          long long relu_bs, float* __restrict__ dx, long long dx_bs, int B, int C4, int cin, int h, int w,
                                                          int nseg_row, int nseg_col) {
    extern __shared__ float ring_smem[];
    float* T = ring_smem;
    float* Dt = T + 3 * C4 * cin;
    float* red = Dt + C4 * (RING_SEG + 2);
    const int per_image = 2 * nseg_row + 2 * nseg_col;
    const int b = blockIdx.x / per_image, which = blockIdx.x % per_image;
    const bool is_row = which < 2 * nseg_row;
    const int side = is_row ? which / nseg_row : (which - 2 * nseg_row) / nseg_col;
    const int seg = is_row ? which % nseg_row : (which - 2 * nseg_row) % nseg_col;
    const int len = is_row ? w : h;
    const int q0 = is_row ? seg * RING_SEG : 1 + seg * RING_SEG;
    const int q_end = is_row ? w : h - 1;
    const int fixed = is_row ? (side ? h - 1 : 0) : (side ? w - 1 : 0);
    const long long hw = (long long)h * w, tstride = (long long)C4 * cin;
    const float* Db = D + (long long)b * d_bs;
    const int tid = threadIdx.x;
    const float* tsrc = tab + (long long)((is_row ? 0 : 6) + side * 3) * tstride;
    for (int i = tid; i < 3 * C4 * cin; i += 256) T[i] = tsrc[i];
    for (int i = tid; i < C4 * (RING_SEG + 2); i += 256) {
        const int c = i / (RING_SEG + 2), k = i - c * (RING_SEG + 2), q = q0 - 1 + k;
        Dt[i] = (q >= 0 && q < len) ? Db[c * hw + (is_row ? (long long)fixed * w + q : (long long)q * w + fixed)] : 0.f;
    }
    __syncthreads();
    const int lane = tid & 63, wv = tid >> 6, m = lane & 15, kq = lane >> 4;
    const int q = q0 + wv * 16 + m;
    for (int ct = 0; ct * 16 < cin; ++ct) {
        const int cia = ct * 16 + m;
        f32x4 acc = {0.f, 0.f, 0.f, 0.f};
        for (int t = 0; t < 3; ++t)
            for (int s4 = 0; s4 < C4; s4 += 4) {
                const int c = s4 + kq;
                const float av = cia < cin ? T[((long long)t * C4 + c) * cin + cia] : 0.f;
                const float bv = Dt[c * (RING_SEG + 2) + wv * 16 + m + 2 - t];
                acc = __builtin_amdgcn_mfma_f32_16x16x4f32(av, bv, acc, 0, 0, 0);
            }
        if (q < q_end) {
#pragma unroll
            for (int e = 0; e < 4; ++e) {
                const int ci = ct * 16 + 4 * kq + e;
                if (ci >= cin) break;
                const long long o = (long long)ci * hw + (is_row ? (long long)fixed * w + q : (long long)q * w + fixed);
                if (relu_of == nullptr || relu_of[(long long)b * relu_bs + o] > 0.f) dx[(long long)b * dx_bs + o] += acc[e];
            }
        }
    }
    if (!is_row) return;
    for (int corner = 0; corner < 2; ++corner) {
        const int jc = corner ? w - 1 : 0;
        if (jc < q0 || jc >= q0 + RING_SEG) continue;
        const float* tcol = tab + (long long)(6 + corner * 3) * tstride;
        const float* tx = tab + (long long)(12 + side * 2 + corner) * tstride;
        const int nterm = 4 * C4;
        for (int ci0 = 0; ci0 < cin; ci0 += 32) {
            const int ci = ci0 + (tid & 31);
            float part = 0.f;
            for (int k = tid >> 5; k < nterm && ci < cin; k += 8) {
                const int t = k / C4, c = k - t * C4;
                float d = 0.f;
                if (t < 3) {
                    const int ii = fixed - t + 1;
                    if (ii >= 0 && ii < h) d = Db[c * hw + (long long)ii * w + jc] * tcol[((long long)t * C4 + c) * cin + ci];
                } else {
                    d = Db[c * hw + (long long)fixed * w + jc] * tx[(long long)c * cin + ci];
                }
                part += d;
            }
            __syncthreads();
            red[(tid >> 5) * 32 + (tid & 31)] = part;
            __syncthreads();
            if (tid < 32 && ci < cin) {
                float sum = 0.f;
                for (int k = 0; k < 8; ++k) sum += red[k * 32 + tid];
                const long long o = (long long)ci * hw + (long long)fixed * w + jc;
                if (relu_of == nullptr || relu_of[(long long)b * relu_bs + o] > 0.f) dx[(long long)b * dx_bs + o] += sum;
            }
        }
    }
}

extern "C" {

int ynet_maxpool2_fwd(const float* x, float* y, long long N, int H, int W, void* stream) {
    YNET_REQUIRE(x && y && N > 0 && H >= 2 && W >= 2, "maxpool2_fwd: bad arguments");
    const long long total = N * (H / 2) * (W / 2);
    hipLaunchKernelGGL(maxpool2_fwd_kernel, plane_grid(N, total / N), dim3(256), 0, (hipStream_t)stream, x, y, N, H, W);
    return ynet_check_launch("maxpool2_fwd");
}

int ynet_maxpool2_bwd(const float* x, const float* dy, float* dx, long long N, int H, int W, void* stream) {
    YNET_REQUIRE(x && dy && dx && N > 0 && H >= 2 && W >= 2, "maxpool2_bwd: bad arguments");
    const long long total = N * ((H + 1) / 2) * ((W + 1) / 2);
    hipLaunchKernelGGL(maxpool2_bwd_kernel, dim3(grid_for(total, 256)), dim3(256), 0, (hipStream_t)stream, x, dy, dx, N, H, W);
    return ynet_check_launch("maxpool2_bwd");
}

int ynet_maxpool2_bwd_add(const float* x, const float* dy, const float* add0, const float* add1, float* dx, long long N,
                          int H, int W, int relu_mask, void* stream) {
    YNET_REQUIRE(x && dy && dx && N > 0 && H >= 2 && W >= 2, "maxpool2_bwd_add: bad arguments");
    YNET_REQUIRE((H & 1) == 0 && (W & 1) == 0, "maxpool2_bwd_add: H and W must be even (got %dx%d)", H, W);
    YNET_REQUIRE((((uintptr_t)x | (uintptr_t)dx | (uintptr_t)add0 | (uintptr_t)add1) & 7) == 0, "maxpool2_bwd_add: 8-byte aligned planes required");
    const long long total = N * (H / 2) * (W / 2);
    if (relu_mask)
        hipLaunchKernelGGL(maxpool2_bwd_add_kernel<true>, plane_grid(N, total / N), dim3(256), 0, (hipStream_t)stream, x, dy, add0, add1, dx, N, H, W);
    else
        hipLaunchKernelGGL(maxpool2_bwd_add_kernel<false>, plane_grid(N, total / N), dim3(256), 0, (hipStream_t)stream, x, dy, add0, add1, dx, N, H, W);
    return ynet_check_launch("maxpool2_bwd_add");
}

int ynet_maxpool2_bwd_add_code(const unsigned char* code, const float* dy, const float* add0, const float* add1, float* dx, long long N, int H, int W,
                               int relu_mask, void* stream) {
    YNET_REQUIRE(code && dy && dx && N > 0 && H >= 2 && W >= 2, "maxpool2_bwd_add_code: bad arguments");
    YNET_REQUIRE((H & 1) == 0 && (W & 1) == 0, "maxpool2_bwd_add_code: H and W must be even (got %dx%d)", H, W);
    YNET_REQUIRE((((uintptr_t)dx | (uintptr_t)add0 | (uintptr_t)add1) & 7) == 0, "maxpool2_bwd_add_code: 8-byte aligned planes required");
    const long long total = N * (H / 2) * (W / 2);
    const float* c = reinterpret_cast<const float*>(code);
    if (relu_mask)
// ... 291 lines not shown
int ynet_resize_nearest(const int* labels, int* out, int H, int W, int Ho, int Wo, double fx, double fy, void* stream) {
    YNET_REQUIRE(labels && out && H > 0 && W > 0 && Ho > 0 && Wo > 0 && fx > 0.0 && fy > 0.0, "resize_nearest: bad arguments");
    hipLaunchKernelGGL(resize_nearest_kernel, dim3(grid_for((long long)Ho * Wo, 256)), dim3(256), 0, (hipStream_t)stream,
                       labels, out, H, W, Ho, Wo, 1.0 / fx, 1.0 / fy);
    return ynet_check_launch("resize_nearest");
}

long long ynet_batchnorm_workspace_doubles(int C) { return C > 0 ? 2ll * C * BN_PARTS : 0; }

static inline dim3 bn_plane_grid(long long planes, long long HW) {
    long long gx = (HW + 1023) / 1024;
    return dim3((unsigned)(gx < 1 ? 1 : (gx > 64 ? 64 : gx)), (unsigned)planes);
}

int ynet_batchnorm2d_fwd(const float* x, float* y, const float* gamma, const float* beta, float* running_mean, float* running_var, float* save_mean, float* save_invstd,
                         double* workspace, int B, int C, long long HW, int train, double momentum, double eps, void* stream) {
    YNET_REQUIRE(x && y && save_mean && save_invstd && B > 0 && C > 0 && HW > 0 && (long long)B * C < 65536, "batchnorm2d_fwd: bad arguments");
    hipStream_t st = (hipStream_t)stream;
    if (train) {
        YNET_REQUIRE(workspace != nullptr, "batchnorm2d_fwd: training mode needs ynet_batchnorm_workspace_doubles(C) doubles of workspace");
        hipLaunchKernelGGL(bn_reduce_kernel<0>, dim3(C * BN_PARTS), dim3(256), 0, st, x, nullptr, nullptr, nullptr, workspace, B, C, HW);
        hipLaunchKernelGGL(bn_finish_kernel, dim3((C + 63) / 64), dim3(64), 0, st, workspace, save_mean, save_invstd, running_mean, running_var, C, (double)B * (double)HW, eps, momentum);
        hipLaunchKernelGGL(bn_apply_kernel, bn_plane_grid((long long)B * C, HW), dim3(256), 0, st, x, save_mean, save_invstd, gamma, beta, y, (long long)B * C, C, HW);
    } else {
        YNET_REQUIRE(running_mean && running_var, "batchnorm2d_fwd: evaluation mode needs the running statistics");
        hipLaunchKernelGGL(bn_invstd_kernel, dim3((C + 63) / 64), dim3(64), 0, st, running_var, save_invstd, C, eps);
        hipLaunchKernelGGL(bn_apply_kernel, bn_plane_grid((long long)B * C, HW), dim3(256), 0, st, x, running_mean, save_invstd, gamma, beta, y, (long long)B * C, C, HW);
    }
    return ynet_check_launch("batchnorm2d_fwd");
}

int ynet_batchnorm2d_bwd(const float* dy, const float* x, const float* mean, const float* invstd, const float* gamma, float* dx, float* dgamma, float* dbeta, double* workspace,
                         int B, int C, long long HW, int train, void* stream) {
    YNET_REQUIRE(dy && x && mean && invstd && dx && workspace && B > 0 && C > 0 && HW > 0 && (long long)B * C < 65536, "batchnorm2d_bwd: bad arguments");
    hipStream_t st = (hipStream_t)stream;
    hipLaunchKernelGGL(bn_reduce_kernel<1>, dim3(C * BN_PARTS), dim3(256), 0, st, x, dy, mean, invstd, workspace, B, C, HW);
    hipLaunchKernelGGL(bn_bwd_kernel, bn_plane_grid((long long)B * C, HW), dim3(256), 0, st, dy, x, mean, invstd, gamma, workspace, dx, dgamma, dbeta, (long long)B * C, C, HW,
                       (double)B * (double)HW, train ? 1 : 0);
    return ynet_check_launch("batchnorm2d_bwd");
}

int ynet_add_relu(const float* a, const float* b, float* y, long long n, int relu, void* stream) {
    YNET_REQUIRE(a && b && y && n > 0, "add_relu: bad arguments");
    hipLaunchKernelGGL(add_relu_kernel, dim3(grid_for(n, 256)), dim3(256), 0, (hipStream_t)stream, a, b, y, n, relu ? 1 : 0);
    return ynet_check_launch("add_relu");
}

int ynet_relu_bwd(const float* dy, const float* y, float* dx, long long n, void* stream) {
    YNET_REQUIRE(dy && y && dx && n > 0, "relu_bwd: bad arguments");
    hipLaunchKernelGGL(relu_bwd_kernel, dim3(grid_for(n, 256)), dim3(256), 0, (hipStream_t)stream, dy, y, dx, n);
    return ynet_check_launch("relu_bwd");
}

int ynet_upconv_dgrad_ring(const float* D, long long d_bs, const float* tables, const float* relu_of, long long relu_of_bs, float* dx, long long dx_bs,
                           int B, int C4, int cin, int h, int w, void* stream) {
    YNET_REQUIRE(D && tables && dx && B > 0 && C4 > 0 && (C4 & 3) == 0 && cin > 0 && h >= 2 && w >= 2, "upconv_dgrad_ring: bad arguments (C4 = 4 cout)");
    YNET_REQUIRE(d_bs >= (long long)C4 * h * w && dx_bs >= (long long)cin * h * w && (relu_of == nullptr || relu_of_bs >= (long long)cin * h * w),
                 "upconv_dgrad_ring: batch strides smaller than the images");
    const int lds = (3 * C4 * cin + C4 * (RING_SEG + 2) + 8 * 32) * 4;
    YNET_REQUIRE(lds <= 64 * 1024, "upconv_dgrad_ring: 4 cout %d x cin %d tables do not fit the 64 KB of LDS this kernel uses", C4, cin);
    const int nseg_row = (w + RING_SEG - 1) / RING_SEG, nseg_col = h > 2 ? (h - 2 + RING_SEG - 1) / RING_SEG : 0;
    const long long blocks = (long long)B * (2 * nseg_row + 2 * nseg_col);
    YNET_REQUIRE(blocks < (1ll << 31), "upconv_dgrad_ring: too many workgroups");
    hipLaunchKernelGGL(upconv_ring_kernel, dim3((unsigned)blocks), dim3(256), lds, (hipStream_t)stream, D, d_bs, tables, relu_of, relu_of_bs, dx, dx_bs, B, C4, cin, h, w,
                       nseg_row, nseg_col);
    return ynet_check_launch("upconv_dgrad_ring");
}

int ynet_rot90_flip(const void* src, void* dst, long long N, int H, int W, int k, int flip, void* stream) {
    YNET_REQUIRE(src && dst && src != dst && N > 0 && H > 0 && W > 0 && k >= 0, "rot90_flip: bad arguments");
    YNET_REQUIRE(N * (long long)H * W < (1ll << 40), "rot90_flip: too many elements");
    hipLaunchKernelGGL(rot90_flip_kernel, dim3(grid_for(N * (long long)H * W, 256)), dim3(256), 0, (hipStream_t)stream,
                       (const unsigned*)src, (unsigned*)dst, N, H, W, k & 3, flip ? 1 : 0);
    return ynet_check_launch("rot90_flip");
}

int ynet_rot_coords(double* xy, long long n, double cx, double cy, double r00, double r01, double r10, double r11, double ox, double oy, void* stream) {
    YNET_REQUIRE(xy && n > 0, "rot_coords: bad arguments");
    hipLaunchKernelGGL(rot_coords_kernel, dim3(grid_for(n, 256)), dim3(256), 0, (hipStream_t)stream, xy, n, cx, cy, r00, r01, r10, r11, ox, oy);
    return ynet_check_launch("rot_coords");
}

static void pred_softargmax_plan(int H, int W, int* gpw, int* nchunk) {
    const int ngroups = (int)(((long long)H * W) >> 7);
    int g = ngroups / 32;
    if (g < 1) g = 1;
    *gpw = g;
    *nchunk = (ngroups + g - 1) / g;
}

int ynet_pred_softargmax_supported(int cin, int cout, int H, int W) {
    return (cin == 8 || cin == 16 || cin == 32) && cout >= 1 && cout <= 32 && H > 0 && W > 0 && (W & 3) == 0 &&
           (((long long)H * W) & 127) == 0 && (long long)H * W < (1ll << 30);
}

long long ynet_pred_softargmax_workspace_floats(long long B, int H, int W) {
    int gpw = 1, nchunk = 1;
    pred_softargmax_plan(H, W, &gpw, &nchunk);
    return B * nchunk * 128;
}

int ynet_pred_softargmax(const float* x, long long x_bs, const float* w, const float* bias, float* out, float* workspace,
                         long long B, int cin, int cout, int H, int W, void* stream) {
    YNET_REQUIRE(x && w && out && workspace && B > 0, "pred_softargmax: bad arguments");
    YNET_REQUIRE(ynet_pred_softargmax_supported(cin, cout, H, W), "pred_softargmax: cin %d cout %d %dx%d is not served (cin 8/16/32, cout <= 32, H*W %% 128 == 0, W %% 4 == 0)", cin, cout, H, W);
    YNET_REQUIRE((((uintptr_t)x | (uintptr_t)workspace) & 15) == 0 && (x_bs & 3) == 0, "pred_softargmax: x and the workspace must be 16-byte aligned");
    PredSoftArgs a{};
    a.x = x;
    a.x_bs = x_bs;
    a.w = w;
    a.bias = bias;
    a.partial = workspace;
    a.cout = cout;
    a.H = H;
    a.W = W;
    pred_softargmax_plan(H, W, &a.gpw, &a.nchunk);
    const long long blocks = B * ((a.nchunk + 3) / 4);
    YNET_REQUIRE(blocks < (1ll << 31), "pred_softargmax: too many workgroups");
    hipStream_t st = (hipStream_t)stream;
// ... 80 lines not shown
```

motion-style-transfer_amd/ops.py:

```python
import ctypes
from typing import List, Sequence

import numpy as np
import torch

from . import _lib as L

MAX_SRC = 4
_VP = ctypes.c_void_p


def _lib():
    return L.load()


def _stream():
    return _VP(torch.cuda.current_stream().cuda_stream)


def _need_gpu(t: torch.Tensor, what: str, dtypes=(torch.float32,)):
    if not torch.is_tensor(t):
        raise TypeError(f"{what}: expected a torch.Tensor, got {type(t)}")
    if not t.is_cuda:
        raise RuntimeError(f"{what}: tensor is on {t.device}; the MI355X path runs on HIP devices only "
# ... 261 lines not shown
    dev = torch.device(device)
    key = (dev.type, dev.index if dev.index is not None else torch.cuda.current_device())
    if key not in _wgrad_streams:
        _wgrad_streams[key] = torch.cuda.Stream(device=dev)
    return key, _wgrad_streams[key]


_wgrad_adds = {}


def join_wgrad_branch():
    for key, side in list(_wgrad_pending.items()):
        adds = _wgrad_adds.pop(key, None)
        if adds:
            with torch.cuda.stream(side), torch.no_grad():
                torch._foreach_add_([a for a, _ in adds], [b for _, b in adds])
        torch.cuda.current_stream(torch.device(key[0], key[1])).wait_stream(side)
    _wgrad_pending.clear()
    _wgrad_adds.clear()


_wino_allowed = _os.environ.get("YNET_WINOGRAD", "1") != "0"
_wino_eval = _os.environ.get("YNET_WINOGRAD_EVAL", "1") != "0"
wino_stats = {"launches": 0}
_wino_eval_min_hw = 0
_wino_cat_eval = True
_wino_plain_eval = True


def _wino_made(entry):
    if not torch.cuda.is_available() or torch.cuda.is_current_stream_capturing():
        return entry + (None, None)
    ev = torch.cuda.Event()
    ev.record()
    return entry + (torch.cuda.current_stream().cuda_stream, ev)


def _wino_ready(entry):
    stream, ev = entry[-2], entry[-1]
    if ev is not None and not torch.cuda.is_current_stream_capturing():
        cur = torch.cuda.current_stream()
        if cur.cuda_stream != stream and not ev.query():
            cur.wait_event(ev)
    return entry


def winograd_filter(wp: torch.Tensor, cin: int, cout: int, col0: int = 0, cols_total: int = None) -> torch.Tensor:
    lib = _lib()
    u = torch.empty(lib.ynet_winograd_filter_floats(cin, cout), device=wp.device, dtype=torch.float32)
    L.check(lib.ynet_winograd_filter(wp.data_ptr(), u.data_ptr(), cin, cout, col0, cout if cols_total is None else cols_total, _stream()), lib)
    return u


def conv2d_winograd_raw(src, u, bias, dst, cin, cout, B, H, W, relu, relu_of=None, wbits_out=None, relu_wbits=None, s2d=False):
    lib = _lib()
    if s2d:
        if bias is not None or relu or relu_of is not None or wbits_out is not None or relu_wbits is not None:
            raise ValueError("conv2d_winograd_raw: s2d is for a plain data gradient")
        L.check(lib.ynet_conv2d_winograd_s2d(src[0], src[1], u.data_ptr(), dst[0], dst[1], cin, cout, B, H, W, _stream()), lib)
        return
    if wbits_out is not None:
        if cout != 32 or not relu or relu_of is not None or relu_wbits is not None:
            raise ValueError("conv2d_winograd_raw: wbits_out is for a forward ReLU launch with 32 outputs")
        L.check(lib.ynet_conv2d_winograd_relu_bits(src[0], src[1], u.data_ptr(), bias.data_ptr() if bias is not None else None, dst[0], dst[1], cin, B, H, W,
                                                   wbits_out.data_ptr(), _stream()), lib)
        return
    if relu_wbits is not None:
        if cout != 32 or bias is not None or relu or relu_of is not None:
            raise ValueError("conv2d_winograd_raw: relu_wbits is for a data gradient with 32 outputs")
        L.check(lib.ynet_conv2d_winograd_dgrad_relu_bits(src[0], src[1], u.data_ptr(), dst[0], dst[1], relu_wbits.data_ptr(), cin, B, H, W, _stream()), lib)
        return
    if relu_of is not None:
        if bias is not None or relu:
            raise ValueError("conv2d_winograd_raw: relu_of is for a data gradient")
        L.check(lib.ynet_conv2d_winograd_dgrad_relu(src[0], src[1], u.data_ptr(), dst[0], dst[1], relu_of[0], relu_of[1], cin, cout, B, H, W, _stream()), lib)
        return
    L.check(lib.ynet_conv2d_winograd(src[0], src[1], u.data_ptr(), bias.data_ptr() if bias is not None else None, dst[0], dst[1],
                                     cin, cout, B, H, W, 1 if relu else 0, _stream()), lib)


def conv2d_winograd_pred_bce_raw(src, u, bias, pred_wp, pred_bias, pred_cout, pos, tmpl, logits, loss, dx, ws, B, H, W, expected_grad):
    lib = _lib()
    L.check(lib.ynet_conv2d_winograd_pred_bce_blob(src[0], src[2], u.data_ptr(), bias.data_ptr() if bias is not None else None, pred_wp.data_ptr(),
                                                   pred_bias.data_ptr() if pred_bias is not None else None, pred_cout, pos.data_ptr(), tmpl.blob.data_ptr(),
                                                   tmpl.blob.shape[0], tmpl.size, logits.data_ptr(), loss.data_ptr(), dx.data_ptr(), 32 * H * W, ws.data_ptr(), B, H, W,
                                                   expected_grad, _stream()), lib)


def conv2d_winograd_split_raw(src, u, dst0, dst0_s2d, dst1, cin, B, H, W):
    lib = _lib()
    L.check(lib.ynet_conv2d_winograd_split(src[0], src[1], u.data_ptr(), dst0[0], dst0[1], 1 if dst0_s2d else 0, dst1[0], dst1[1], cin, B, H, W, _stream()), lib)


def conv2d_winograd_cat_raw(srcs, u, bias, dst, B, H, W, relu, addend=None, pool=None, wbits_out=None, pool_code=None):
    lib = _lib()
    sp, sc, sb = _arrays(srcs)
    b = bias.data_ptr() if bias is not None else None
    if wbits_out is not None:
        if pool is not None or not relu:
            raise ValueError("conv2d_winograd_cat_raw: wbits_out is for a ReLU launch without the pooled copy")
        L.check(lib.ynet_conv2d_winograd_cat_relu_bits(sp, sc, sb, len(srcs), u.data_ptr(), b, dst[0], dst[1], B, H, W, addend[0] if addend else None,
                                                       addend[1] if addend else 0, addend[2] if addend else 0, wbits_out.data_ptr(), _stream()), lib)
        return
    if pool is not None and pool_code is not None:
        if not relu:
            raise ValueError("conv2d_winograd_cat_raw: pool_code is for a ReLU launch")
        L.check(lib.ynet_conv2d_winograd_cat_pool_code(sp, sc, sb, len(srcs), u.data_ptr(), b, dst[0], dst[1], pool[0], pool[1], pool_code.data_ptr(), B, H, W,
                                                       _stream()), lib)
        return
    if pool is not None:
        L.check(lib.ynet_conv2d_winograd_cat_pool(sp, sc, sb, len(srcs), u.data_ptr(), b, dst[0], dst[1], pool[0], pool[1], 32, B, H, W,
                                                  1 if relu else 0, _stream()), lib)
    elif addend is None:
        L.check(lib.ynet_conv2d_winograd_cat(sp, sc, sb, len(srcs), u.data_ptr(), b, dst[0], dst[1], 32, B, H, W, 1 if relu else 0, _stream()), lib)
    else:
        L.check(lib.ynet_conv2d_winograd_cat_add(sp, sc, sb, len(srcs), u.data_ptr(), b, dst[0], dst[1], 32, B, H, W, 1 if relu else 0,
                                                 addend[0], addend[1], addend[2], _stream()), lib)


_pool_code_allowed = _os.environ.get("YNET_POOL_CODE", "1") != "0"
_wino_relu_bits_allowed = _os.environ.get("YNET_WINOGRAD_RELU_BITS", "1") != "0"
_wino16_allowed = _os.environ.get("YNET_WINOGRAD16", "1") != "0"
_wino16_for_16 = _os.environ.get("YNET_WINOGRAD16_SLICE16", "0") != "0"
_split48_allowed = _os.environ.get("YNET_WINOGRAD_SPLIT48", "1") != "0"


def conv2d_winograd16_raw(srcs, u, bias, dst, cout, B, H, W, relu, relu_of=None, addend=None, pool=None):
    lib = _lib()
    sp, sc, sb = _arrays(srcs)
    L.check(lib.ynet_conv2d_winograd16(sp, sc, sb, len(srcs), u.data_ptr(), bias.data_ptr() if bias is not None else None, dst[0], dst[1], cout, B, H, W,
                                       1 if relu else 0, relu_of[0] if relu_of else None, relu_of[1] if relu_of else 0,
                                       addend[0] if addend else None, addend[1] if addend else 0, addend[2] if addend else 0,
                                       pool[0] if pool else None, pool[1] if pool else 0, _stream()), lib)


def _wino16_supported(srcs_c, cout, B, H, W, K=3):
    if not (_wino16_allowed and _wino_allowed and K == 3 and 1 <= len(srcs_c) <= 3):
        return False
    return bool(_lib().ynet_conv2d_winograd16_supported(B, H, W, (ctypes.c_int * len(srcs_c))(*srcs_c), len(srcs_c), cout, K))


def _wino16_filter(wino, wp, row0, cs, cout, col0, ctot):
    lib = _lib()
# ... 4 lines not shown
        ca = (ctypes.c_int * len(cs))(*cs)
        u = torch.empty(lib.ynet_winograd16_filter_floats(ca, len(cs), cout), device=wp.device, dtype=torch.float32)
        cols_pad = -(-ctot // 64) * 64
        L.check(lib.ynet_winograd16_filter(wp.data_ptr() + 4 * row0 * 9 * cols_pad, u.data_ptr(), ca, len(cs), cout, col0, ctot, _stream()), lib)
        ent = cache[key] = _wino_made((wp, u, cs))
    _wino_ready(ent)
    return ent


def _wino16(wino, wp, row0, srcs, bias, dst, cout, col0, ctot, B, H, W, relu, relu_of=None, addend=None, pool=None):
    ent = _wino16_filter(wino, wp, row0, tuple(s_[1] for s_ in srcs), cout, col0, ctot)
    conv2d_winograd16_raw(srcs, ent[1], None if bias is None else bias[col0:col0 + cout], dst, cout, B, H, W, relu, relu_of=relu_of, addend=addend, pool=pool)
    wino_stats["launches"] += 1
    wino_stats["launches16"] = wino_stats.get("launches16", 0) + 1


def _pad4(c):
    return (c + 3) & ~3


conv_auto = _os.environ.get("YNET_CONV_AUTO", "1") != "0"
_AUTO_TAG_CAT = {10: ("winograd_cat:2,3", "winograd_cat:2,6|code"), 40: ("winograd_cat:2,2", "winograd_cat:2,5|wbits"), 41: ("winograd_cat:2,0", "winograd_cat:2,4|wbits"),
                 30: ("winograd_cat:2,2", "winograd_cat:2,5|wbits")}


def _auto_tag(tk):
    if tk.family == 0:
        return None
    if tk.family == 1:
        return "winograd:" + "+".join("%d,%d,%d" % tuple(tk.tmpl[i]) for i in range(tk.nlaunch)) + ("|wbits" if tk.wrote_wbits else "")
    if tk.family == 2:
        return _AUTO_TAG_CAT[tk.variant][1 if (tk.wrote_wbits or tk.wrote_pool_code) else 0]
    if tk.family == 3:
        return "winograd16:" + "+".join("%d" % tk.tmpl[i][0] for i in range(tk.nlaunch))
    return "winograd_up:%d" % tk.family


def _auto_flags(wino):
    flags = 0
    if wino is None or not _wino_allowed:
        flags |= L.AUTO_NO_WINOGRAD
    if not _wino16_allowed:
        flags |= L.AUTO_NO_WINOGRAD16
    if _wino16_for_16:
        flags |= L.AUTO_WINOGRAD16_FOR_16
    if not _pool_code_allowed:
        flags |= L.AUTO_NO_POOL_CODE
    if not _split48_allowed:
        flags |= L.AUTO_NO_SPLIT48
    return flags


def conv2d_auto_raw(srcs, mask, wp, bias, dsts, B, H, W, K, relu, relu_of=None, pooled=None, bits_out=None, relu_bits=None, wino=None, wbits_out=None,
                    relu_wbits=None, pool_code=None, addend=None, upsample2x=False, wp_version=1, dst_s2d=None):
    lib = _lib()
    d = L.ConvAuto()
    d.nsrc, d.ndst = len(srcs), len(dsts)
    for i, s_ in enumerate(srcs):
        d.src[i], d.src_c[i], d.src_bs[i] = s_[0], s_[1], s_[2]
        d.src_bmod[i] = s_[3] if len(s_) > 3 else 0
    for i, t_ in enumerate(dsts):
        d.dst[i], d.dst_c[i], d.dst_bs[i] = t_[0], t_[1], t_[2]
        if dst_s2d is not None and dst_s2d[i]:
            d.dst_s2d[i] = 1
    if mask:
        d.mask, d.mask_bs = mask[0], mask[1]
    d.wp, d.bias = wp.data_ptr(), (bias.data_ptr() if bias is not None else None)
    d.B, d.H, d.W, d.K, d.relu, d.upsample2x = B, H, W, K, 1 if relu else 0, 1 if upsample2x else 0
    if relu_of is not None:
        d.relu_of, d.relu_of_bs = relu_of[0], relu_of[1]
    if pooled is not None:
        d.pooled, d.pooled_bs = pooled[0], pooled[1]
        if pool_code is not None:
            d.pool_code = pool_code.data_ptr()
    if addend is not None:
        d.addend, d.addend_bs, d.addend_bmod = addend[0], addend[1], addend[2]
    d.bits_out, d.relu_bits = bits_out, relu_bits
    if wbits_out is not None:
        d.wbits_out = wbits_out.data_ptr()
    if relu_wbits is not None:
        d.relu_wbits = relu_wbits.data_ptr()
    d.flags = flags = _auto_flags(wino)
    ent = None
    if wino is not None and not (flags & L.AUTO_NO_WINOGRAD):
        cache, what = wino
        need = lib.ynet_conv2d_auto_cache_floats(ctypes.byref(d))
        if need < 0:
            L.check(1, lib)
        if need > 0:
            key = "auto_" + what
            ent = cache.get(key)
            if ent is None or ent[0] is not wp or ent[1].numel() < need:
                ent = cache[key] = [wp, torch.empty(need, device=wp.device, dtype=torch.float32), (ctypes.c_ulonglong * 2)(0, 0), None, None]
            elif ent[4] is not None and not torch.cuda.is_current_stream_capturing():
                cur = torch.cuda.current_stream()
                if cur.cuda_stream != ent[3] and not ent[4].query():
                    cur.wait_event(ent[4])
            d.cache, d.cache_floats, d.cache_tag, d.wp_version = ent[1].data_ptr(), ent[1].numel(), ent[2], int(wp_version)
    if B * H * W <= 65536:
        nws = lib.ynet_conv2d_auto_workspace_floats(ctypes.byref(d))
        if nws > 0:
            key = (wp.device, torch.cuda.current_stream().cuda_stream)
            ws = _conv_ws.get(key)
            if ws is None or ws.numel() < nws:
                ws = _conv_ws[key] = torch.empty(nws, device=wp.device, dtype=torch.float32)
            d.workspace, d.workspace_floats = ws.data_ptr(), nws
    tk = L.ConvTaken()
    L.check(lib.ynet_conv2d_auto(ctypes.byref(d), ctypes.byref(tk), _stream()), lib)
    if tk.transformed and ent is not None and torch.cuda.is_available() and not torch.cuda.is_current_stream_capturing():
        ev = torch.cuda.Event()
        ev.record()
        ent[3], ent[4] = torch.cuda.current_stream().cuda_stream, ev
    if tk.family:
        wino_stats["launches"] += tk.nlaunch
        if tk.family in (3, 5):
            wino_stats["launches16"] = wino_stats.get("launches16", 0) + tk.nlaunch
    return _auto_tag(tk), tk


_dgrad_family_memo = {}


def dgrad_relu_family(B, H, W, dy_c, dx_c, K=3):
    key = (B, H, W, dy_c, dx_c, K, _wino_allowed, _wino16_allowed, _wino16_for_16)
    fam = _dgrad_family_memo.get(key)
    if fam is None:
        d, tk = L.ConvAuto(), L.ConvTaken()
        d.nsrc = d.ndst = 1
        d.src[0], d.src_c[0], d.src_bs[0] = 256, dy_c, dy_c * H * W
        d.dst[0], d.dst_c[0], d.dst_bs[0] = 256, dx_c, dx_c * H * W
        d.relu_of, d.relu_of_bs = 256, dx_c * H * W
        d.wp = 256
        d.B, d.H, d.W, d.K = B, H, W, K
        d.flags = (0 if _wino_allowed else L.AUTO_NO_WINOGRAD) | (0 if _wino16_allowed else L.AUTO_NO_WINOGRAD16) | (L.AUTO_WINOGRAD16_FOR_16 if _wino16_for_16 else 0)
        lib = _lib()
        L.check(lib.ynet_conv2d_auto_plan(ctypes.byref(d), ctypes.byref(tk)), lib)
        fam = _dgrad_family_memo[key] = int(tk.family)
    return fam


def conv2d_raw(srcs, mask, wp, bias, dsts, B, H, W, K, relu, relu_of=None, pooled=None, bits_out=None, relu_bits=None, wino=None, wbits_out=None,
               relu_wbits=None, pool_code=None, dst_s2d=None, info=None):
    if not conv_auto:
        return _conv2d_raw_py(srcs, mask, wp, bias, dsts, B, H, W, K, relu, relu_of=relu_of, pooled=pooled, bits_out=bits_out, relu_bits=relu_bits, wino=wino,
                              wbits_out=wbits_out, relu_wbits=relu_wbits, pool_code=pool_code, dst_s2d=dst_s2d, info=info)
    if wino is not None and not torch.is_grad_enabled() and (
            H * W < _wino_eval_min_hw or not (_wino_plain_eval if len(srcs) == 1 and srcs[0][1] in (16, 32) else _wino_cat_eval)):
        wino = None
    tag, tk = conv2d_auto_raw(srcs, mask, wp, bias, dsts, B, H, W, K, relu, relu_of=relu_of, pooled=pooled, bits_out=bits_out, relu_bits=relu_bits, wino=wino,
                              wbits_out=wbits_out, relu_wbits=relu_wbits, pool_code=pool_code, dst_s2d=dst_s2d)
    if info is not None:
        info["wrote_s2d"] = int(tk.wrote_s2d)
    return tag


def _conv2d_raw_py(srcs, mask, wp, bias, dsts, B, H, W, K, relu, relu_of=None, pooled=None, bits_out=None, relu_bits=None, wino=None, wbits_out=None,
                   relu_wbits=None, pool_code=None, dst_s2d=None, info=None):
    lib = _lib()
    sp, sc, sb = _arrays(srcs)
    if info is not None:
        info["wrote_s2d"] = 0
    if wino is not None and not torch.is_grad_enabled() and (
            H * W < _wino_eval_min_hw or not (_wino_plain_eval if len(srcs) == 1 and srcs[0][1] in (16, 32) else _wino_cat_eval)):
        wino = None
    if bits_out is not None:
        if len(dsts) != 1 or mask is not None or relu_of is not None or pooled is not None or not relu or _bmods(srcs) is not None:
            raise ValueError("conv2d_raw: bits_out is for a forward ReLU convolution with one destination")
        L.check(lib.ynet_conv2d_relu_bits(sp, sc, sb, len(srcs), wp.data_ptr(), bias.data_ptr() if bias is not None else None,
                                          dsts[0][0], dsts[0][1], dsts[0][2], bits_out, B, H, W, K, _stream()), lib)
        return
    if relu_bits is not None:
        if len(srcs) != 1 or len(dsts) != 1 or bias is not None or relu or relu_of is not None:
            raise ValueError("conv2d_raw: relu_bits is for a data gradient with one source and one destination")
        L.check(lib.ynet_conv2d_dgrad_relu_bits(srcs[0][0], srcs[0][1], srcs[0][2], mask[0] if mask else None, mask[1] if mask else 0,
                                                wp.data_ptr(), dsts[0][0], dsts[0][1], dsts[0][2], relu_bits, B, H, W, K, _stream()), lib)
        return
    if pooled is not None:
        if len(dsts) != 1 or mask is not None or relu_of is not None or _bmods(srcs) is not None:
            raise ValueError("conv2d_raw: pooled is for a forward convolution with one destination")
        if (wino is not None and _wino_allowed and K == 3 and dsts[0][1] == 32 and dsts[0][0] % 8 == 0 and dsts[0][2] % 2 == 0
                and all(len(s_) == 3 and s_[0] % 16 == 0 and s_[2] % 4 == 0 for s_ in srcs)):
            cs = (ctypes.c_int * len(srcs))(*[s_[1] for s_ in srcs])
            if lib.ynet_conv2d_winograd_cat_supported(B, H, W, cs, len(srcs), 32, K):
                cache, what = wino
                key = "wino_cat_" + what
                ent = cache.get(key)
                if ent is None or ent[0] is not wp or ent[2] != tuple(cs):
                    u = torch.empty(lib.ynet_winograd_filter_cat_floats(cs, len(srcs), 32), device=wp.device, dtype=torch.float32)
                    L.check(lib.ynet_winograd_filter_cat(wp.data_ptr(), u.data_ptr(), cs, len(srcs), 32, 0, 32, _stream()), lib)
                    ent = cache[key] = _wino_made((wp, u, tuple(cs)))
                _wino_ready(ent)
                code = pool_code if (relu and _pool_code_allowed) else None
                conv2d_winograd_cat_raw(srcs, ent[1], bias, (dsts[0][0], dsts[0][2]), B, H, W, relu, pool=pooled, pool_code=code)
                wino_stats["launches"] += 1
                return "winograd_cat:2,6|code" if code is not None else "winograd_cat:2,3"
        if (wino is not None and K == 3 and dsts[0][0] % 8 == 0 and dsts[0][2] % 2 == 0 and all(len(s_) == 3 and s_[0] % 16 == 0 and s_[2] % 4 == 0 for s_ in srcs)
                and _wino16_supported([s_[1] for s_ in srcs], dsts[0][1], B, H, W)):
            _wino16(wino, wp, 0, srcs, bias, (dsts[0][0], dsts[0][2]), dsts[0][1], 0, dsts[0][1], B, H, W, relu, pool=pooled)
            return "winograd16:3"
        L.check(lib.ynet_conv2d_pool(sp, sc, sb, len(srcs), wp.data_ptr(), bias.data_ptr() if bias is not None else None,
                                     dsts[0][0], dsts[0][1], dsts[0][2], pooled[0], pooled[1], B, H, W, K, 1 if relu else 0, _stream()), lib)
        return
    if (wino is not None and _wino_allowed and K == 3 and mask is None and len(srcs) == 1 and len(srcs[0]) == 3
            and srcs[0][0] % 16 == 0 and srcs[0][2] % 4 == 0 and (relu_of is None or (relu_of[0] % 8 == 0 and relu_of[1] % 2 == 0))):
        cin, ctot, HW = srcs[0][1], sum(d[1] for d in dsts), H * W
        pieces, piece_dst, c0 = [], [], 0
        for di, (ptr, c, bs) in enumerate(dsts):
            if ptr is None:
                c0 += c
                continue
            o = 0
            while c - o >= 16 and (c - o) % 16 == 0:
                n = 32 if c - o >= 32 else 16
                pieces.append((ptr + 4 * o * HW, n, bs, c0 + o))
                piece_dst.append((di, n == c))
                o += n
            if o != c:
                pieces = None
                break
            c0 += c
        if (_wino16_for_16 and pieces and len(pieces) == 1 and pieces[0][1] == 16 and pieces[0][0] % 8 == 0 and pieces[0][2] % 2 == 0
                and _wino16_supported([cin], 16, B, H, W)):
            ptr, n, bs, col0 = pieces[0]
            _wino16(wino, wp, 0, srcs, bias, (ptr, bs), 16, col0, ctot, B, H, W, relu, relu_of=relu_of)
            return "winograd16:%d" % (1 if relu_of is not None else 0)
        wide = any(d_[0] is not None and d_[1] >= 64 for d_ in dsts)
        if (_split48_allowed and pieces and not wide and len(pieces) == 2 and relu_of is None and bias is None and not relu and pieces[0][1] == 16 and piece_dst[0][1]
                and pieces[1][1] == 32 and piece_dst[1][1] and pieces[1][3] == pieces[0][3] + 16 and all(p_[0] % 8 == 0 and p_[2] % 2 == 0 for p_ in pieces)
                and all(lib.ynet_conv2d_winograd_supported(B, H, W, cin, p_[1], K) for p_ in pieces) and lib.ynet_conv2d_winograd_split_supported(B, H, W, cin)):
            cache, what = wino
            col0 = pieces[0][3]
            key = "wino_%s_%d_48" % (what, col0)
            ent = cache.get(key)
            if ent is None or ent[0] is not wp:
                ent = cache[key] = _wino_made((wp, winograd_filter(wp, cin, 48, col0, ctot)))
            _wino_ready(ent)
            s2d = bool(dst_s2d and dst_s2d[piece_dst[0][0]])
            conv2d_winograd_split_raw((srcs[0][0], srcs[0][2]), ent[1], (pieces[0][0], pieces[0][2]), s2d, (pieces[1][0], pieces[1][2]), cin, B, H, W)
            if s2d and info is not None:
                info["wrote_s2d"] |= 1 << piece_dst[0][0]
            wino_stats["launches"] += 1
            return "winograd:3,%d,%d" % (cin // 8, 6 if s2d else 5)
        if (pieces and not wide and len(pieces) <= (2 if relu_of is None else 1) and all(p_[0] % 8 == 0 and p_[2] % 2 == 0 for p_ in pieces)
                and all(lib.ynet_conv2d_winograd_supported(B, H, W, cin, p_[1], K) for p_ in pieces)):
            cache, what = wino
            one32 = len(pieces) == 1 and pieces[0][1] == 32
            wb_out = wbits_out if (one32 and relu and relu_of is None) else None
            wb_in = relu_wbits if (one32 and relu_of is not None and not relu and bias is None) else None
            em = 3 if wb_out is not None else (2 if wb_in is not None else (1 if relu_of is not None else 0))
            s2ds = [bool(dst_s2d and dst_s2d[di] and whole and em == 0 and bias is None and not relu) for di, whole in piece_dst]
            tag = ("winograd:" + "+".join("%d,%d,%d" % (p_[1] // 16, cin // 8, 4 if f_ else em) for p_, f_ in zip(pieces, s2ds))
                   + ("|wbits" if wb_out is not None else ""))
            for (ptr, n, bs, col0), (di, whole), s2d in zip(pieces, piece_dst, s2ds):
                key = "wino_%s_%d_%d" % (what, col0, n)
                ent = cache.get(key)
                if ent is None or ent[0] is not wp:
                    ent = cache[key] = _wino_made((wp, winograd_filter(wp, cin, n, col0, ctot)))
                _wino_ready(ent)
                conv2d_winograd_raw((srcs[0][0], srcs[0][2]), ent[1], None if bias is None else bias[col0:col0 + n], (ptr, bs), cin, n, B, H, W, relu,
                                    relu_of=None if wb_in is not None else relu_of, wbits_out=wb_out, relu_wbits=wb_in, **({"s2d": True} if s2d else {}))
                if s2d and info is not None:
                    info["wrote_s2d"] |= 1 << di
                wino_stats["launches"] += 1
            return tag
        wanted, c0 = [], 0
        for ptr, c, bs in dsts:
            if ptr is not None:
                wanted.append((ptr, c, bs, c0))
            c0 += c
        if (wanted and (relu_of is None or len(wanted) == 1) and all(w_[0] % 8 == 0 and w_[2] % 2 == 0 and _wino16_supported([cin], w_[1], B, H, W) for w_ in wanted)):
            for ptr, c, bs, col0 in wanted:
                _wino16(wino, wp, 0, srcs, bias, (ptr, bs), c, col0, ctot, B, H, W, relu, relu_of=relu_of)
            return "winograd16:" + "+".join("%d" % (1 if relu_of is not None else 0) for _ in wanted)
        if (pieces and wide and len(pieces) <= (2 if relu_of is None else 1) and all(p_[0] % 8 == 0 and p_[2] % 2 == 0 for p_ in pieces)
                and all(lib.ynet_conv2d_winograd_supported(B, H, W, cin, p_[1], K) for p_ in pieces)):
            cache, what = wino
            tag = "winograd:" + "+".join("%d,%d,%d" % (p_[1] // 16, cin // 8, 1 if relu_of is not None else 0) for p_ in pieces)
            for ptr, n, bs, col0 in pieces:
                key = "wino_%s_%d_%d" % (what, col0, n)
                ent = cache.get(key)
                if ent is None or ent[0] is not wp:
                    ent = cache[key] = _wino_made((wp, winograd_filter(wp, cin, n, col0, ctot)))
                _wino_ready(ent)
                conv2d_winograd_raw((srcs[0][0], srcs[0][2]), ent[1], None if bias is None else bias[col0:col0 + n], (ptr, bs), cin, n, B, H, W, relu,
                                    relu_of=relu_of)
                wino_stats["launches"] += 1
            return tag
    if (wino is not None and _wino_allowed and K == 3 and mask is None and relu_of is None and all(len(s_) == 3 for s_ in srcs)
            and (len(srcs) > 1 or srcs[0][1] not in (16, 32)) and all(s_[0] % 16 == 0 and s_[2] % 4 == 0 for s_ in srcs)):
        want = [d for d in dsts if d[0] is not None]
        if len(want) == 1 and len(dsts) == 1 and want[0][1] == 32 and want[0][0] % 8 == 0 and want[0][2] % 2 == 0:
            cs = (ctypes.c_int * len(srcs))(*[s_[1] for s_ in srcs])
            first = srcs[0]
            rest_c = [first[1] - 32] + [s_[1] for s_ in srcs[1:]] if first[1] >= 32 else None
            rest_c = [c for c in rest_c if c > 0] if rest_c is not None else None
            if (not lib.ynet_conv2d_winograd_cat_supported(B, H, W, cs, len(srcs), 32, K) and rest_c and len(rest_c) <= 3
                    and lib.ynet_conv2d_winograd_supported(B, H, W, 32, 32, K)
                    and lib.ynet_conv2d_winograd_cat_supported(B, H, W, (ctypes.c_int * len(rest_c))(*rest_c), len(rest_c), 32, K)):
                cache, what = wino
                key = "wino_split_" + what
                ent = cache.get(key)
                rc = (ctypes.c_int * len(rest_c))(*rest_c)
                if ent is None or ent[0] is not wp or ent[3] != tuple(rest_c):
                    cols_pad = -(-32 // 64) * 64
                    u0 = winograd_filter(wp, 32, 32, 0, 32)
                    u1 = torch.empty(lib.ynet_winograd_filter_cat_floats(rc, len(rest_c), 32), device=wp.device, dtype=torch.float32)
                    L.check(lib.ynet_winograd_filter_cat(wp.data_ptr() + 4 * 32 * 9 * cols_pad, u1.data_ptr(), rc, len(rest_c), 32, 0, 32, _stream()), lib)
                    ent = cache[key] = _wino_made((wp, u0, u1, tuple(rest_c)))
                _wino_ready(ent)
                HW = H * W
                conv2d_winograd_raw((first[0], first[2]), ent[1], None, (want[0][0], want[0][2]), 32, 32, B, H, W, False)
                rsrcs = ([(first[0] + 4 * 32 * HW, first[1] - 32, first[2])] if first[1] > 32 else []) + list(srcs[1:])
                wb_out = wbits_out if relu else None
# ... 209 lines not shown
            ia = lambda xs: (ctypes.c_int * n)(*xs)
            L.check(lib.ynet_lora_compose_pack_multi(
                n, vp([e[1].data_ptr() for e in entries]), vp([e[2].data_ptr() if e[2] is not None else None for e in entries]),
                vp([e[3].data_ptr() if e[3] is not None else None for e in entries]), (ctypes.c_float * n)(*[e[9] for e in entries]),
                vp([e[4][0].data_ptr() for e in entries]), vp([e[4][1].data_ptr() for e in entries]),
                ia([e[5] for e in entries]), ia([e[6] for e in entries]), ia([e[7] for e in entries]),
                ia([e[8] for e in entries]), _stream()), lib)
            for e in entries:
                m, w, bufs = e[0], e[1], e[4]
                cache = m._packed
                cache.clear()
                cache["key"] = _weight_key(m.weight, e[10], e[11])
                cache["lora_bufs"], cache["lora_shape"] = bufs, tuple(w.shape)
                cache["fwd"], cache["dgrad"] = bufs


refresh_lora_filters = refresh_filters


class _SkipEntry:
    __slots__ = ("ref", "shape", "stash", "consumed")


_skip_registry = {}
skip_fold = False
_skip_fold_allowed = _os.environ.get("YNET_SKIP_FOLD", "1") != "0"


_relu_outputs = {}
_premasked = {}
premask = False
premask_stats = {"unmasked_backwards": 0}
_premask_allowed = _os.environ.get("YNET_PREMASK", "1") != "0"
_relu_bits_allowed = _os.environ.get("YNET_RELU_BITS", "1") != "0"


def _is_relu_output(t: torch.Tensor) -> bool:
    e = _relu_outputs.get(t.data_ptr())
    return e is not None and e[0]() is not None and e[1] == tuple(t.shape)


class fold_skip_gradients:

    def __enter__(self):
        global skip_fold, premask, wgrad_branch
        self._prev = (skip_fold, premask, wgrad_branch)
        skip_fold = _skip_fold_allowed
        premask = _premask_allowed
        wgrad_branch = _wgrad_branch_allowed and overlap_decoders
        _relu_outputs.clear()
        _premasked.clear()
        _s2d_wanted.clear()
        _s2d_grads.clear()
        _s2d_produced.clear()
        _deferred.clear()
        _unmaterialized.clear()
        return self

    def __exit__(self, *exc):
        global skip_fold, premask, wgrad_branch
        skip_fold, premask, wgrad_branch = self._prev
        join_wgrad_branch()
        _relu_outputs.clear()
        _premasked.clear()
        _s2d_wanted.clear()
        _s2d_grads.clear()
        _s2d_produced.clear()
        _deferred.clear()
        _unmaterialized.clear()
        _blob_targets.clear()
        for k in [k for k, e in _skip_registry.items() if e.consumed or e.ref() is None or e.stash]:
            del _skip_registry[k]
        return False


def _skip_register(x: torch.Tensor):
    for k in [k for k, e in _skip_registry.items() if e.ref() is None or e.consumed]:
        del _skip_registry[k]
    e = _SkipEntry()
    e.ref, e.shape, e.stash, e.consumed = weakref.ref(x), tuple(x.shape), [], False
    _skip_registry[x.data_ptr()] = e


def _skip_entry(t: torch.Tensor):
    e = _skip_registry.get(t.data_ptr())
    if e is None:
        return None
    if e.ref() is None or e.shape != tuple(t.shape):
        del _skip_registry[t.data_ptr()]
        return None
    return e


class _Conv2dFn(torch.autograd.Function):
    @staticmethod
    def forward(ctx, meta, weight, bias, lora_a, lora_b, *srcs):
        relu, scale, cache = meta["relu"], meta.get("scale", 1.0), meta["cache"]
        _need_gpu(weight, "conv2d weight")
        cout, cin, k, _ = weight.shape
        if meta.get("bcast"):
            srcs = [s.expand(meta["batch"], -1, -1, -1) if f else s for s, f in zip(srcs, meta["bcast"])]
        descs, keep = [], []
        reps = meta.get("repeat") or [1] * len(srcs)
        for i, s in enumerate(srcs):
            t, c, bs = _plane_desc(s, f"conv2d input {i}")
            keep.append(t)
            if reps[i] > 1:
                if ctx.needs_input_grad[5 + i]:
                    raise NotImplementedError("conv2d: a batch-repeated input cannot receive a gradient")
                descs.append((t.data_ptr(), c, c * t.shape[2] * t.shape[3] if t.shape[0] == 1 else t.stride(0), t.shape[0]))
            else:
                descs.append((t.data_ptr(), c, bs))
        if len(descs) > MAX_SRC:
            raise ValueError(f"conv2d: at most {MAX_SRC} concatenated inputs (got {len(descs)})")
        if sum(d[1] for d in descs) != cin:
            raise ValueError(f"conv2d: inputs carry {sum(d[1] for d in descs)} channels, weight expects {cin}")
        B, _, H, W = keep[0].shape
        B = max(t.shape[0] * r for t, r in zip(keep, reps))
        for t, r in zip(keep, reps):
# ... 52 lines not shown
        ctx.has_lora = lora_a is not None
        ctx.save_for_backward(weight, lora_a, lora_b, y if relu else None, *keep)
        ctx.w_key = _weight_key(weight, lora_a, lora_b)
        if relu and premask:
            _relu_outputs[y.data_ptr()] = (weakref.ref(y), tuple(y.shape), bits, k, wbits)
        return y

    @staticmethod
    def backward(ctx, dy):
        weight, lora_a, lora_b, y, *srcs = ctx.saved_tensors
        meta = ctx.meta
        relu, scale, cache = meta["relu"], meta.get("scale", 1.0), meta["cache"]
        cout, cin, k, _ = weight.shape
        dy = dy.contiguous()
        B, _, H, W = dy.shape
        mask = (y.data_ptr(), cout * H * W) if relu else None
        if relu and _premasked:
            if _premasked.pop(dy.data_ptr(), None) == (y.data_ptr(), dy._version, tuple(dy.shape)):
                mask = None
                premask_stats["unmasked_backwards"] += 1
        if relu and mask is not None and _unmaterialized.get(y.data_ptr()) == tuple(y.shape):
            raise RuntimeError("conv2d backward: this convolution ran inside the fused predictor + criterion launch (its output was never written), but the gradient that "
                               "arrived does not carry its ReLU backward -- the output has another consumer, or a hook replaced its gradient: set YNET_CONV_PRED_BCE=0")
        need = ctx.needs_input_grad
        need_src = list(need[5:5 + ctx.n_src])
        d_srcs = [None] * ctx.n_src
        branch = None
        if (wgrad_branch and ctx.has_lora and dy.is_cuda and not need[1] and not (ctx.has_bias and need[2]) and (need[3] or need[4])
                and lora_a.is_leaf and lora_b.is_leaf and not lora_a._backward_hooks and not lora_b._backward_hooks
                and not getattr(lora_a, "_post_accumulate_grad_hooks", None) and not getattr(lora_b, "_post_accumulate_grad_hooks", None)):
            cur = torch.cuda.current_stream(dy.device)
            bkey, branch = _wgrad_stream(dy.device)
            branch.wait_stream(cur)
        if any(need_src) and meta.get("input_grad") is not None:
            if ctx.w_key != _weight_key(weight, lora_a, lora_b):
                raise RuntimeError("conv2d backward: a parameter was modified in place between forward and backward")
            d_srcs = _input_grad_srcs(meta, dy, y, _cached(cache, weight, lora_a, lora_b, scale, "dgrad"), srcs, need_src)
        elif any(need_src):
            if ctx.w_key != _weight_key(weight, lora_a, lora_b):
                raise RuntimeError("conv2d backward: a parameter was modified in place between forward and backward")
            wp_d = _cached(cache, weight, lora_a, lora_b, scale, "dgrad")
            dsts, want_s2d = [], []
            for i, s in enumerate(srcs):
                c = s.shape[1]
                if need_src[i]:
                    d_srcs[i] = torch.empty((B, c, H, W), device=dy.device, dtype=torch.float32)
                    dsts.append((d_srcs[i].data_ptr(), c, c * H * W))
                    w_ = _s2d_wanted.get(s.data_ptr()) if (premask and _upconv_s2d_allowed) else None
                    want_s2d.append(bool(w_ is not None and w_[0]() is not None and w_[1] == tuple(s.shape) and c == 16 and H % 2 == 0 and W % 2 == 0))
                else:
                    dsts.append((None, c, 0))
                    want_s2d.append(False)
            s2d_info = {} if any(want_s2d) else None
            s0 = srcs[0]
            emask = None
            if (premask and ctx.n_src == 1 and need_src[0] and _is_relu_output(s0) and s0.is_contiguous() and s0.shape[0] == B
                    and s0.data_ptr() % 16 == 0 and dy.data_ptr() % 16 == 0 and not (skip_fold and _skip_entry(s0) is not None)
                    and _lib().ynet_conv2d_dgrad_relu_supported(B, H, W, int(s0.shape[1]), int(k))):
                emask = (s0.data_ptr(), s0.shape[1] * H * W)
            ebits = None
            if emask is not None:
                e0 = _relu_outputs.get(s0.data_ptr())
                if (e0 is not None and e0[2] is not None and e0[3] == k and d_srcs[0].data_ptr() % 16 == 0
                        and _lib().ynet_conv2d_relu_bits_words(B, H, W, int(s0.shape[1]), int(k)) == e0[2].numel()):
                    ebits = e0[2]
            wino_em = (emask is not None and mask is None and bool(meta.get("wino")) and _wino_allowed and k == 3 and dy.data_ptr() % 16 == 0
                       and d_srcs[0].data_ptr() % 8 == 0 and s0.data_ptr() % 8 == 0 and dgrad_relu_family(B, H, W, cout, int(s0.shape[1]), int(k)) != 0)
            ewbits = None
            if wino_em and _wino_relu_bits_allowed and int(s0.shape[1]) == 32:
                e0 = _relu_outputs.get(s0.data_ptr())
                if (e0 is not None and len(e0) > 4 and e0[4] is not None and e0[4].numel() == _lib().ynet_winograd_relu_bits_words(B, H, W)
                        and _lib().ynet_conv2d_winograd_supported(B, H, W, cout, 32, int(k))):
                    ewbits = e0[4]
            if ebits is not None and not wino_em:
                premask_stats["bit_masks"] = premask_stats.get("bit_masks", 0) + 1
                conv2d_raw([(dy.data_ptr(), cout, cout * H * W)], mask, wp_d, None, dsts, B, H, W, k, False, relu_bits=ebits.data_ptr())
            else:
                if ewbits is not None:
                    premask_stats["wino_bit_masks"] = premask_stats.get("wino_bit_masks", 0) + 1
                conv2d_raw([(dy.data_ptr(), cout, cout * H * W)], mask, wp_d, None, dsts, B, H, W, k, False, relu_of=emask,
                           wino=(cache, "dgrad") if meta.get("wino") else None, relu_wbits=ewbits, dst_s2d=want_s2d if s2d_info is not None else None, info=s2d_info)
                if s2d_info:
                    for i, g_ in enumerate(d_srcs):
                        if g_ is not None and (s2d_info.get("wrote_s2d", 0) >> i) & 1:
                            _s2d_grads[g_.data_ptr()] = (g_._version, tuple(g_.shape))
                            _s2d_wanted.pop(srcs[i].data_ptr(), None)
                            _s2d_produced.add(srcs[i].data_ptr())
            if emask is not None:
                _premasked[d_srcs[0].data_ptr()] = (s0.data_ptr(), d_srcs[0]._version, tuple(d_srcs[0].shape))
            if skip_fold:
                for i, s in enumerate(srcs):
                    if d_srcs[i] is None:
                        continue
                    e = _skip_entry(s)
                    if e is not None and not e.consumed and len(e.stash) < 2:
                        ev = torch.cuda.Event()
                        ev.record(torch.cuda.current_stream(dy.device))
                        e.stash.append((d_srcs[i], ev))
                        d_srcs[i] = None
        d_w = d_b = d_a = d_bm = None
        want_w = need[1] or (ctx.has_lora and (need[3] or need[4]))
        want_b = ctx.has_bias and need[2]
        if branch is not None:
            for t in (dy, y, weight, lora_a, lora_b, *srcs):
                if t is not None:
                    t.record_stream(branch)
            with torch.cuda.stream(branch):
                if lora_conv2d_wgrad_supported(srcs, dy, weight, lora_a, preferred=True):
                    d_a, d_bm = lora_conv2d_wgrad_raw(srcs, dy, mask, weight, lora_a.detach(), lora_b.detach(), scale)
                else:
                    dw, _ = conv2d_wgrad_raw(srcs, dy, mask, weight, False)
                    d_a, d_bm = lora_grad(dw, lora_a.detach(), lora_b.detach(), scale)
                for p_, g_, want in ((lora_a, d_a, need[3]), (lora_b, d_bm, need[4])):
                    if want and p_.grad is not None:
                        _wgrad_adds.setdefault(bkey, []).append((p_.grad, g_.view_as(p_.grad)))
            for p_, g_, want in ((lora_a, d_a, need[3]), (lora_b, d_bm, need[4])):
                g_.record_stream(cur)
                if want and p_.grad is None:
                    p_.grad = g_.view_as(p_)
            d_a = d_bm = None
            _wgrad_pending[bkey] = branch
        elif want_w or want_b:
            if ctx.has_lora and not need[1] and not want_b and lora_conv2d_wgrad_supported(srcs, dy, weight, lora_a, preferred=True):
                d_a, d_bm = lora_conv2d_wgrad_raw(srcs, dy, mask, weight, lora_a.detach(), lora_b.detach(), scale)
            else:
                dw, d_b = conv2d_wgrad_raw(srcs, dy, mask, weight, want_b)
                if ctx.has_lora and (need[3] or need[4]):
                    d_a, d_bm = lora_grad(dw, lora_a.detach(), lora_b.detach(), scale)
                if need[1]:
                    d_w = dw
        return (None, d_w, d_b, d_a if need[3] else None, d_bm if need[4] else None, *d_srcs)


def conv2d_wgrad_raw(srcs, dy, mask, weight, want_b):
    lib = _lib()
    cout, cin, k, _ = weight.shape
    B, _, H, W = dy.shape
    descs = [(s.data_ptr(), s.shape[1], (s.stride(0) if s.shape[0] > 1 else s.shape[1] * H * W)) for s in srcs]
# ... 252 lines not shown
            L.check(lib.ynet_maxpool2_bwd(x.data_ptr(), dy.contiguous().data_ptr(), dx.data_ptr(), B * C, H, W, _stream()), lib)
        return dx


def max_pool2(x):
    return _MaxPool2Fn.apply(x)


class _Upsample2xFn(torch.autograd.Function):
    @staticmethod
    def forward(ctx, x):
        _need_gpu(x, "upsample2x")
        x = x.contiguous()
        B, C, H, W = x.shape
        y = torch.empty((B, C, 2 * H, 2 * W), device=x.device, dtype=torch.float32)
        lib = _lib()
        L.check(lib.ynet_upsample2x_fwd(x.data_ptr(), y.data_ptr(), B * C, H, W, _stream()), lib)
        ctx.shape = (B, C, H, W)
        ctx.premask = bool(premask and ctx.needs_input_grad[0] and _is_relu_output(x))
        ctx.save_for_backward(x if ctx.premask else None)
        return y

    @staticmethod
    def backward(ctx, dy):
        B, C, H, W = ctx.shape
        (x,) = ctx.saved_tensors
        dx = torch.empty((B, C, H, W), device=dy.device, dtype=torch.float32)
        lib = _lib()
        if ctx.premask and premask and x is not None:
            L.check(lib.ynet_upsample2x_bwd_relu(dy.contiguous().data_ptr(), dx.data_ptr(), x.data_ptr(), B * C, H, W, _stream()), lib)
            _premasked[dx.data_ptr()] = (x.data_ptr(), dx._version, tuple(dx.shape))
        else:
            L.check(lib.ynet_upsample2x_bwd(dy.contiguous().data_ptr(), dx.data_ptr(), B * C, H, W, _stream()), lib)
        return dx


def upsample2x(x):
    return _Upsample2xFn.apply(x)


_upconv_allowed = _os.environ.get("YNET_WINOGRAD_UP", "1") != "0"
upconv_stats = {"fused": 0}


def upsample2x_conv2d_raw(src, u, bias, dst, cin, cout, B, H, W, relu=False):
    lib = _lib()
    L.check(lib.ynet_upsample2x_conv2d_winograd(src[0], src[1], u.data_ptr(), bias.data_ptr() if bias is not None else None, dst[0], dst[1], cin, cout, B, H, W,
                                                1 if relu else 0, _stream()), lib)


_upconv_s2d_allowed = _os.environ.get("YNET_UPCONV_S2D", "1") != "0"
_s2d_wanted = {}
_s2d_grads = {}
_conv_pred_bce_allowed = _os.environ.get("YNET_CONV_PRED_BCE", "1") != "0"
_deferred = {}
_unmaterialized = {}
conv_pred_bce_stats = {"fused": 0, "materialized": 0}


def materialize_deferred(t):
    if not _deferred or not torch.is_tensor(t):
        return t
    e = _deferred.get(t.data_ptr())
    if e is not None and e["ref"]() is not None and e["shape"] == tuple(t.shape):
        del _deferred[t.data_ptr()]
        e["run"]()
        conv_pred_bce_stats["materialized"] += 1
    return t


_s2d_produced = set()
upconv_stats_s2d = {"backwards": 0}
_S2D_M = ((0.75, 0.25, 0.0), (0.25, 0.75, 0.75), (0.0, 0.0, 0.25)), ((0.25, 0.0, 0.0), (0.75, 0.75, 0.25), (0.0, 0.25, 0.75))
_S2D_DM = ((-0.25, 0.25, 0.0), (0.25, 0.0, 0.0)), ((0.0, 0.0, 0.25), (0.0, 0.25, -0.25))


def upconv_s2d_tables(weight, cache):
    key = ("s2d", weight.data_ptr(), weight._version)
    ent = cache.get("s2d_tables")
    if ent is None or ent[0] != key:
        with torch.no_grad():
            K = weight.detach().double()
            cout, cin = K.shape[0], K.shape[1]
            M = torch.tensor(_S2D_M, dtype=torch.float64, device=K.device)
            dM = torch.tensor(_S2D_DM, dtype=torch.float64, device=K.device)
            keff = torch.einsum("pau,oiuv,qbv->pqoiab", M, K, M).reshape(4 * cout, cin, 3, 3).float().contiguous()
            tabs = []
            for s_ in range(2):
                tabs.append(torch.einsum("pu,oiuv,qbv->bpqoi", dM[s_], K, M).reshape(3, 4 * cout, cin))
            for s_ in range(2):
                tabs.append(torch.einsum("pau,oiuv,qv->apqoi", M, K, dM[s_]).reshape(3, 4 * cout, cin))
            corners = [torch.einsum("pu,oiuv,qv->pqoi", dM[sv], K, dM[sh]).reshape(1, 4 * cout, cin) for sv in range(2) for sh in range(2)]
            tables = torch.cat(tabs + corners, 0).float().contiguous()
            ent = cache["s2d_tables"] = (key, pack_weight(keff, 1), tables, {})
    return ent[1], ent[2], ent[3]


def upconv_dgrad_raw(D, weight, dx, relu_of, B, cout, cin, h, w, cache):
    lib = _lib()
    wino = (cache, "dgrad")
    if not torch.is_grad_enabled() and (h * w < _wino_eval_min_hw or not (_wino_plain_eval if 4 * cout in (16, 32) else _wino_cat_eval)):
        wino = None
    hw = h * w
    d = L.ConvAuto()
    d.nsrc = d.ndst = 1
    d.src[0], d.src_c[0], d.src_bs[0] = D, 4 * cout, 4 * cout * hw
    d.dst[0], d.dst_c[0], d.dst_bs[0] = dx, cin, cin * hw
    if relu_of is not None:
        d.relu_of, d.relu_of_bs = relu_of, cin * hw
    d.wp = weight.data_ptr()
    d.B, d.H, d.W, d.K = B, h, w, 3
    d.flags = _auto_flags(wino) | L.AUTO_UPCONV_BWD
    need = lib.ynet_conv2d_auto_cache_floats(ctypes.byref(d))
    if need <= 0:
        L.check(1, lib)
    key = ("upconv_bwd", B, h, w, relu_of is not None, int(d.flags), int(need))
    ent = cache.get(key)
    if ent is None:
        ent = cache[key] = [torch.empty(need, device=weight.device, dtype=torch.float32), (ctypes.c_ulonglong * 2)(0, 0), None, 0]
    wkey = (weight.data_ptr(), weight._version)
    if ent[2] != wkey:
        ent[2], ent[3] = wkey, ent[3] + 1
    d.cache, d.cache_floats, d.cache_tag, d.wp_version = ent[0].data_ptr(), ent[0].numel(), ent[1], ent[3]
    if B * hw <= 65536:
        nws = lib.ynet_conv2d_auto_workspace_floats(ctypes.byref(d))
        if nws > 0:
            wkey_ = (weight.device, torch.cuda.current_stream().cuda_stream)
            ws = _conv_ws.get(wkey_)
            if ws is None or ws.numel() < nws:
                ws = _conv_ws[wkey_] = torch.empty(nws, device=weight.device, dtype=torch.float32)
            d.workspace, d.workspace_floats = ws.data_ptr(), nws
    tk = L.ConvTaken()
    L.check(lib.ynet_conv2d_auto(ctypes.byref(d), ctypes.byref(tk), _stream()), lib)
    if tk.family:
        wino_stats["launches"] += tk.nlaunch - 1
        if tk.family in (3, 5):
            wino_stats["launches16"] = wino_stats.get("launches16", 0) + tk.nlaunch - 1
    return tk


def upconv_tables(weight, cache):
    key = ("hip", weight.data_ptr(), weight._version)
    ent = cache.get("upconv_tables")
    if ent is None or ent[0] != key:
        cout, cin = int(weight.shape[0]), int(weight.shape[1])
        kf, tf = ctypes.c_longlong(0), ctypes.c_longlong(0)
        lib = _lib()
        if lib.ynet_upconv_tables_floats(cout, cin, ctypes.byref(kf), ctypes.byref(tf)) < 0:
            raise ValueError("upconv_tables: bad filter shape %s" % (tuple(weight.shape),))
        keff = torch.empty(kf.value, device=weight.device, dtype=torch.float32)
        tables = torch.empty((16, 4 * cout, cin), device=weight.device, dtype=torch.float32)
        w_ = weight.detach().contiguous()
        L.check(lib.ynet_upconv_tables(w_.data_ptr(), cout, cin, keff.data_ptr(), tables.data_ptr(), _stream()), lib)
        ent = cache["upconv_tables"] = (key, keff, tables, {}, w_)
    return ent[1], ent[2], ent[3]


class _UpConvFn(torch.autograd.Function):

    @staticmethod
    def forward(ctx, x, weight, bias, cache):
        _need_gpu(x, "upsample2x_conv2d")
        x = x.contiguous()
        B, cin, Hl, Wl = x.shape
        cout = weight.shape[0]
        H, W = 2 * Hl, 2 * Wl
        wp = _cached(cache, weight, None, None, 1.0, "fwd")
        if _lib().ynet_upsample2x_conv2d_winograd_supported(B, H, W, cin, cout, 3) == 2:
            ent = _wino16_filter((cache, "fwd"), wp, 0, (cin,), cout, 0, cout)
        else:
            key = "wino_fwd_0_%d" % cout
            ent = cache.get(key)
            if ent is None or ent[0] is not wp:
                ent = cache[key] = _wino_made((wp, winograd_filter(wp, cin, cout, 0, cout)))
            _wino_ready(ent)
        y = torch.empty((B, cout, H, W), device=x.device, dtype=torch.float32)
        upsample2x_conv2d_raw((x.data_ptr(), cin * Hl * Wl), ent[1], bias.detach() if bias is not None else None, (y.data_ptr(), cout * H * W), cin, cout, B, H, W)
        wino_stats["launches"] += 1
        upconv_stats["fused"] += 1
        ctx.cache, ctx.shape, ctx.cout = cache, (B, cin, Hl, Wl), cout
        ctx.w_key = _weight_key(weight, None, None)
        ctx.premask = bool(premask and ctx.needs_input_grad[0] and _is_relu_output(x))
        ctx.save_for_backward(weight, x if ctx.premask else None)
        if (_upconv_s2d_allowed and premask and ctx.needs_input_grad[0] and cout == 16 and x.data_ptr() % 16 == 0
                and _wino16_supported([4 * cout], cin, B, Hl, Wl)):
            _s2d_wanted[y.data_ptr()] = (weakref.ref(y), tuple(y.shape))
        ctx.y_ptr = y.data_ptr()
        return y

    @staticmethod
    def backward(ctx, dy):
        weight, x = ctx.saved_tensors
        B, cin, Hl, Wl = ctx.shape
        H, W, cout = 2 * Hl, 2 * Wl, ctx.cout
        if ctx.w_key != _weight_key(weight, None, None):
            raise RuntimeError("upsample2x_conv2d backward: the filter was modified in place between forward and backward")
        dy = dy.contiguous()
        reg = _s2d_grads.pop(dy.data_ptr(), None)
        handed = reg is not None and reg == (dy._version, tuple(dy.shape))
        if ctx.y_ptr in _s2d_produced:
            _s2d_produced.discard(ctx.y_ptr)
            if not handed:
                raise RuntimeError("upsample2x_conv2d backward: a gradient of this up-convolution's output was written space-to-depth for it, but the gradient that "
                                   "arrived is another tensor (the output has a second consumer, or a hook replaced its gradient): set YNET_UPCONV_S2D=0 for such a graph")
        if handed:
            dx = torch.empty((B, cin, Hl, Wl), device=dy.device, dtype=torch.float32)
            masked = bool(ctx.premask and premask and x is not None)
            w_ = weight.detach()
            if not w_.is_contiguous():
                w_ = ctx.cache["upconv_w"] = w_.contiguous()
            if conv_auto:
                upconv_dgrad_raw(dy.data_ptr(), w_, dx.data_ptr(), x.data_ptr() if masked else None, B, cout, cin, Hl, Wl, ctx.cache)
            else:
                wp_eff, tables, wcache = upconv_tables(w_, ctx.cache)
                conv2d_raw([(dy.data_ptr(), 4 * cout, 4 * cout * Hl * Wl)], None, wp_eff, None, [(dx.data_ptr(), cin, cin * Hl * Wl)], B, Hl, Wl, 3, False,
                           relu_of=(x.data_ptr(), cin * Hl * Wl) if masked else None, wino=(wcache, "dgrad"))
                lib = _lib()
                L.check(lib.ynet_upconv_dgrad_ring(dy.data_ptr(), 4 * cout * Hl * Wl, tables.data_ptr(), x.data_ptr() if masked else None, cin * Hl * Wl, dx.data_ptr(),
                                                   cin * Hl * Wl, B, 4 * cout, cin, Hl, Wl, _stream()), lib)
            if masked:
                _premasked[dx.data_ptr()] = (x.data_ptr(), dx._version, tuple(dx.shape))
            upconv_stats_s2d["backwards"] += 1
            return dx, None, None, None
        wp_d = _cached(ctx.cache, weight, None, None, 1.0, "dgrad")
        d_up = torch.empty((B, cin, H, W), device=dy.device, dtype=torch.float32)
        conv2d_raw([(dy.data_ptr(), cout, cout * H * W)], None, wp_d, None, [(d_up.data_ptr(), cin, cin * H * W)], B, H, W, 3, False, wino=(ctx.cache, "dgrad"))
        dx = torch.empty((B, cin, Hl, Wl), device=dy.device, dtype=torch.float32)
        lib = _lib()
        if ctx.premask and premask and x is not None:
            L.check(lib.ynet_upsample2x_bwd_relu(d_up.data_ptr(), dx.data_ptr(), x.data_ptr(), B * cin, Hl, Wl, _stream()), lib)
            _premasked[dx.data_ptr()] = (x.data_ptr(), dx._version, tuple(dx.shape))
        else:
            L.check(lib.ynet_upsample2x_bwd(d_up.data_ptr(), dx.data_ptr(), B * cin, Hl, Wl, _stream()), lib)
        return dx, None, None, None


def upsample2x_conv2d(x, conv):
    w, b = conv.weight, conv.bias
    if (_upconv_allowed and _wino_allowed and torch.is_tensor(x) and x.is_cuda and x.dim() == 4 and x.dtype == torch.float32
            and ((not torch.is_grad_enabled() and _wino_eval) or (torch.is_grad_enabled() and not w.requires_grad and (b is None or not b.requires_grad)))
            and not conv._forward_hooks and not conv._forward_pre_hooks and not conv._backward_hooks
            and tuple(w.shape[1:]) == (x.shape[1], 3, 3) and x.data_ptr() % 16 == 0
            and _lib().ynet_upsample2x_conv2d_winograd_supported(int(x.shape[0]), 2 * int(x.shape[2]), 2 * int(x.shape[3]), int(x.shape[1]), int(w.shape[0]), 3)):
        return _UpConvFn.apply(x, w, b, conv._packed)
    return conv(upsample2x(x))


def avgpool_pyramid(x: torch.Tensor, n_levels: int) -> List[torch.Tensor]:
    _need_gpu(x, "avgpool_pyramid")
    x = x.detach().contiguous()
    B, C, H, W = x.shape
    outs = [torch.empty((B, C, H >> i, W >> i), device=x.device, dtype=torch.float32) for i in range(1, n_levels)]
    if outs:
        lib = _lib()
        ptrs = (_VP * len(outs))(*[o.data_ptr() for o in outs])
        L.check(lib.ynet_avgpool_pyramid(x.data_ptr(), ctypes.cast(ptrs, L.PP), len(outs), B * C, H, W, _stream()), lib)
    return [x] + outs


class _BatchNorm2dFn(torch.autograd.Function):
    @staticmethod
    def forward(ctx, x, gamma, beta, running_mean, running_var, train, factor, eps):
        _need_gpu(x, "batch_norm2d input")
        x = x.contiguous()
        B, C, H, W = x.shape
        lib = _lib()
        y = torch.empty_like(x)
        mean, invstd = torch.empty(C, device=x.device, dtype=torch.float32), torch.empty(C, device=x.device, dtype=torch.float32)
        ws = torch.empty(lib.ynet_batchnorm_workspace_doubles(C), device=x.device, dtype=torch.float64)
        ptr = lambda t: None if t is None else t.data_ptr()
        L.check(lib.ynet_batchnorm2d_fwd(x.data_ptr(), y.data_ptr(), ptr(gamma), ptr(beta), ptr(running_mean), ptr(running_var), mean.data_ptr(), invstd.data_ptr(),
                                         ws.data_ptr(), B, C, H * W, 1 if train else 0, float(factor), float(eps), _stream()), lib)
# ... 723 lines not shown
```

Measured before the change: 5010 trajectories/s.

## Emit border column copy from s2d Winograd dgrad for upconv ring kernel

When the Winograd data-gradient kernel writes a space-to-depth destination, its edge tiles now also write the left and right border columns into a small contiguous side buffer. The up-convolution ring kernel then reads that compact buffer instead of gathering strided columns from the full gradient tensor. This targets the scattered, poorly coalesced column reads in the ring kernel. The cost is extra stores in the Winograd epilogue, an extra allocation per backward pass, and more Python bookkeeping to hand the buffer between the two backward calls.

Measured after the change: 5010 trajectories/s (median of 2 runs). About the same (-0.0%).

```diff
diff --git a/include/ynet_hip.h b/include/ynet_hip.h
--- a/include/ynet_hip.h
+++ b/include/ynet_hip.h
@@ -43,6 +43,10 @@
 int ynet_conv2d_winograd(const float* src, long long src_bs, const float* u, const float* bias, float* dst, long long dst_bs, int cin, int cout,
                          int B, int H, int W, int relu, void* stream);
 int ynet_conv2d_winograd_s2d(const float* src, long long src_bs, const float* u, float* dst, long long dst_bs, int cin, int cout, int B, int H, int W, void* stream);
+int ynet_conv2d_winograd_s2d_border(const float* src, long long src_bs, const float* u, float* dst, long long dst_bs, float* border, int cin, int cout, int B, int H, int W,
+                                    void* stream);
+int ynet_conv2d_winograd_split_border(const float* src, long long src_bs, const float* u, float* dst0, long long dst0_bs, float* dst0_border, float* dst1, long long dst1_bs,
+                                      int cin, int B, int H, int W, void* stream);
 int ynet_conv2d_winograd_pred_bce_supported(int B, int H, int W, int cin, int cout, int pred_cout, int kernlen);
 int ynet_conv2d_winograd_pred_bce_blob(const float* src, long long src_bs, const float* u, const float* bias, const float* pred_wp, const float* pred_bias, int pred_cout,
                                        const float* target_xy, const float* blob, int kernlen, int S, float* logits, float* loss, float* dx, long long dx_bs,
@@ -125,6 +129,8 @@
     long long workspace_floats;
     unsigned flags;
     int dst_s2d[4];
+    float* dst_border[4];
+    const float* src_border;
 } YnetConvAuto;
 typedef struct YnetConvTaken {
     int family;
@@ -143,6 +149,8 @@
 int ynet_upconv_tables(const float* w, int cout, int cin, float* keff_packed, float* tables, void* stream);
 int ynet_upconv_dgrad_ring(const float* D, long long d_bs, const float* tables, const float* relu_of, long long relu_of_bs, float* dx, long long dx_bs,
                            int B, int C4, int cin, int h, int w, void* stream);
+int ynet_upconv_dgrad_ring_border(const float* D, long long d_bs, const float* border, const float* tables, const float* relu_of, long long relu_of_bs, float* dx,
+                                  long long dx_bs, int B, int C4, int cin, int h, int w, void* stream);
 
 int ynet_conv2d_plan(int B, int H, int W, int cout, int K);
 
diff --git a/motion-style-transfer_amd/_lib.py b/motion-style-transfer_amd/_lib.py
--- a/motion-style-transfer_amd/_lib.py
+++ b/motion-style-transfer_amd/_lib.py
@@ -23,7 +23,8 @@
                 ("addend", c_fp), ("addend_bs", c_ll), ("addend_bmod", c_i),
                 ("bits_out", c_fp), ("relu_bits", c_fp), ("wbits_out", c_fp), ("relu_wbits", c_fp),
                 ("cache", c_fp), ("cache_floats", c_ll), ("cache_tag", ctypes.POINTER(ctypes.c_ulonglong)), ("wp_version", ctypes.c_ulonglong),
-                ("workspace", c_fp), ("workspace_floats", c_ll), ("flags", ctypes.c_uint), ("dst_s2d", c_i * 4)]
+                ("workspace", c_fp), ("workspace_floats", c_ll), ("flags", ctypes.c_uint), ("dst_s2d", c_i * 4),
+                ("dst_border", c_fp * 4), ("src_border", c_fp)]
 
 
 class ConvTaken(ctypes.Structure):
@@ -54,6 +55,9 @@
     "ynet_winograd_filter": (c_i, [c_fp, c_fp, c_i, c_i, c_i, c_i, c_fp]),
     "ynet_conv2d_winograd": (c_i, [c_fp, c_ll, c_fp, c_fp, c_fp, c_ll, c_i, c_i, c_i, c_i, c_i, c_i, c_fp]),
     "ynet_conv2d_winograd_s2d": (c_i, [c_fp, c_ll, c_fp, c_fp, c_ll, c_i, c_i, c_i, c_i, c_i, c_fp]),
+    "ynet_conv2d_winograd_s2d_border": (c_i, [c_fp, c_ll, c_fp, c_fp, c_ll, c_fp, c_i, c_i, c_i, c_i, c_i, c_fp]),
+    "ynet_conv2d_winograd_split_border": (c_i, [c_fp, c_ll, c_fp, c_fp, c_ll, c_fp, c_fp, c_ll, c_i, c_i, c_i, c_i, c_fp]),
+    "ynet_upconv_dgrad_ring_border": (c_i, [c_fp, c_ll, c_fp, c_fp, c_fp, c_ll, c_fp, c_ll, c_i, c_i, c_i, c_i, c_i, c_fp]),
     "ynet_conv2d_winograd_pred_bce_supported": (c_i, [c_i, c_i, c_i, c_i, c_i, c_i, c_i]),
     "ynet_conv2d_winograd_pred_bce_blob": (c_i, [c_fp, c_ll, c_fp, c_fp, c_fp, c_fp, c_i, c_fp, c_fp, c_i, c_i, c_fp, c_fp, c_fp, c_ll, c_fp, c_i, c_i, c_i,
                                                  c_f, c_fp]),
diff --git a/motion-style-transfer_amd/csrc/conv_auto.cpp b/motion-style-transfer_amd/csrc/conv_auto.cpp
--- a/motion-style-transfer_amd/csrc/conv_auto.cpp
+++ b/motion-style-transfer_amd/csrc/conv_auto.cpp
@@ -420,7 +420,9 @@
         if (p.variant == 23) {
             const Piece &q0 = p.pieces[0], &q1 = p.pieces[1];
             const int s2d = a->dst_s2d[q0.dst] ? 1 : 0;
-            const int rc = ynet_conv2d_winograd_split(a->src[0], a->src_bs[0], u0, q0.ptr, q0.bs, s2d, q1.ptr, q1.bs, a->src_c[0], B, H, W, stream);
+            const int rc = (s2d && a->dst_border[q0.dst])
+                               ? ynet_conv2d_winograd_split_border(a->src[0], a->src_bs[0], u0, q0.ptr, q0.bs, a->dst_border[q0.dst], q1.ptr, q1.bs, a->src_c[0], B, H, W, stream)
+                               : ynet_conv2d_winograd_split(a->src[0], a->src_bs[0], u0, q0.ptr, q0.bs, s2d, q1.ptr, q1.bs, a->src_c[0], B, H, W, stream);
             if (rc) return rc;
             if (s2d) t.wrote_s2d |= 1 << q0.dst;
             tag(0, 3, a->src_c[0] / 8, s2d ? 6 : 5);
@@ -437,7 +439,7 @@
             int rc;
             const bool s2d = a->dst_s2d[q.dst] && q.whole && em == 0 && !a->bias && !relu;
             if (s2d) {
-                rc = ynet_conv2d_winograd_s2d(a->src[0], a->src_bs[0], u, q.ptr, q.bs, a->src_c[0], q.n, B, H, W, stream);
+                rc = ynet_conv2d_winograd_s2d_border(a->src[0], a->src_bs[0], u, q.ptr, q.bs, a->dst_border[q.dst], a->src_c[0], q.n, B, H, W, stream);
                 if (rc) return rc;
                 t.wrote_s2d |= 1 << q.dst;
                 tag(i, q.n / 16, a->src_c[0] / 8, 4);
@@ -607,8 +609,8 @@
     }
     YnetConvTaken ti;
     if (int rc = run_plan(&u.in, u.p, t, &ti, stream)) return rc;
-    if (int rc = ynet_upconv_dgrad_ring(a->src[0], a->src_bs[0], a->cache + u.tab_off, a->relu_of, a->relu_of_bs, a->dst[0], a->dst_bs[0], a->B, 4 * u.cout, u.cin, a->H, a->W,
-                                        stream))
+    if (int rc = ynet_upconv_dgrad_ring_border(a->src[0], a->src_bs[0], a->src_border, a->cache + u.tab_off, a->relu_of, a->relu_of_bs, a->dst[0], a->dst_bs[0], a->B,
+                                               4 * u.cout, u.cin, a->H, a->W, stream))
         return rc;
     ti.nlaunch += 1;
     if (taken) *taken = ti;
diff --git a/motion-style-transfer_amd/csrc/conv_wino.hip b/motion-style-transfer_amd/csrc/conv_wino.hip
--- a/motion-style-transfer_amd/csrc/conv_wino.hip
+++ b/motion-style-transfer_amd/csrc/conv_wino.hip
@@ -41,7 +41,9 @@
     float* loss;
     long long n_loss;
     float gs;
+    float* border;
 };
+
 
 __device__ __forceinline__ f32x2 wn_v01(f32x2 tl, f32x2 th) {
     f32x2 r;
@@ -57,7 +59,7 @@
 template <int NCB, int EPI, int BITS = 0, bool S2D = false, int CB0 = 0, int CB1 = NCB>
 __device__ __forceinline__ void wino_epilogue(f32x4 (&acc)[16][NCB], const f32x2 (&bias2)[NCB][2], float floor_v, __amdgpu_buffer_rsrc_t ry,
                                               __amdgpu_buffer_rsrc_t rm, unsigned st0, unsigned st1, unsigned so_t, unsigned sm_t, int HW, unsigned stp = 0,
-                                              unsigned* wbits = nullptr, unsigned char* pcode = nullptr) {
+                                              unsigned* wbits = nullptr, unsigned char* pcode = nullptr, float* bd = nullptr, unsigned bd_vo = 0, unsigned bd_l4 = 0) {
     unsigned word = 0u;
     if constexpr (BITS == 2) word = *wbits;
 #pragma unroll
@@ -122,6 +124,14 @@
                     const unsigned vo = st0 + (odd ? ph - 4u : 0u);
                     __builtin_amdgcn_raw_buffer_store_b64(__builtin_bit_cast(u32x2, p0), ry, vo, sc, 0);
                     __builtin_amdgcn_raw_buffer_store_b64(__builtin_bit_cast(u32x2, p1), ry, vo, sc + 2u * ph, 0);
+                    if (bd != nullptr) {
+                        const unsigned bp = (unsigned)(NB * 16) * bd_l4, bs = (unsigned)(cd * 16 + 2 * h + k) * bd_l4;
+                        const __amdgpu_buffer_rsrc_t rb = __builtin_amdgcn_make_buffer_rsrc(bd, 0, 8u * bp, 0x00020000);
+                        __builtin_amdgcn_raw_buffer_store_b32(__builtin_bit_cast(unsigned, e00), rb, bd_vo, bs, 0);
+                        __builtin_amdgcn_raw_buffer_store_b32(__builtin_bit_cast(unsigned, e01), rb, bd_vo, bs + bp, 0);
+                        __builtin_amdgcn_raw_buffer_store_b32(__builtin_bit_cast(unsigned, e10), rb, bd_vo, bs + 2u * bp, 0);
+                        __builtin_amdgcn_raw_buffer_store_b32(__builtin_bit_cast(unsigned, e11), rb, bd_vo, bs + 3u * bp, 0);
+                    }
                     continue;
                 }
                 const unsigned so = so_t + (unsigned)((cd * 16 + 2 * h + k) * HW * 4);
@@ -485,6 +495,17 @@
             const int tx = t % tiles_x, ty = (t / tiles_x) % tiles_y, b = t / (tiles_x * tiles_y);
             const unsigned so_s2d = (unsigned)(((ty * (WN_TH / 2) + (cur & 7)) * (W >> 1) + tx * (WN_TW / 2)) * 4);
             const unsigned so_rm = (unsigned)(((ty * WN_TH + 2 * (cur & 7)) * W + tx * WN_TW) * 4);
+            float* bdp = nullptr;
+            unsigned bd_vo = 0x80000000u;
+            const unsigned bd_l4 = (unsigned)(H >> 1) * 4u;
+            if constexpr (EM == 4 || EM == 6) {
+                constexpr int PL = 4 * 16 * (EM == 6 ? 1 : NCB);
+                if (a.border != nullptr && (tx == 0 || tx == tiles_x - 1)) {
+                    bdp = a.border + (long long)b * (2 * PL) * (H >> 1) + (ty * (WN_TH / 2) + (cur & 7));
+                    if (n == 0 && tx == 0) bd_vo = (unsigned)(4 * kq) * bd_l4;
+                    if (n == 15 && tx == tiles_x - 1) bd_vo = (unsigned)(PL + 4 * kq) * bd_l4;
+                }
+            }
             if constexpr (EM == 7 || EM == 8) {
                 static_assert((EM != 7 && EM != 8) || NCB == 2, "the predictor epilogue is the 32-channel launch's");
                 const __amdgpu_buffer_rsrc_t rdx = __builtin_amdgcn_make_buffer_rsrc(a.y + (long long)b * a.y_bs, 0, y_img, 0x00020000);
@@ -503,7 +524,7 @@
                 static_assert(EM < 5 || NCB == 3, "the two-destination epilogue is the 48-channel launch's");
                 const __amdgpu_buffer_rsrc_t r0 = __builtin_amdgcn_make_buffer_rsrc(a.y + (long long)b * a.y_bs, 0, (unsigned)(16 * HW * 4), 0x00020000);
                 const __amdgpu_buffer_rsrc_t r1 = __builtin_amdgcn_make_buffer_rsrc(a.y2 + (long long)b * a.y2_bs, 0, (unsigned)(32 * HW * 4), 0x00020000);
-                if constexpr (EM == 6) wino_epilogue<NCB, 0, 0, true, 0, 1>(acc, bias2, floor_v, r0, r0, st_s2d, st_s2d, so_s2d, so_s2d, HW);
+                if constexpr (EM == 6) wino_epilogue<NCB, 0, 0, true, 0, 1>(acc, bias2, floor_v, r0, r0, st_s2d, st_s2d, so_s2d, so_s2d, HW, 0, nullptr, nullptr, bdp, bd_vo, bd_l4);
                 else wino_epilogue<NCB, 0, 0, false, 0, 1>(acc, bias2, floor_v, r0, r0, st_rm, st_rm + (unsigned)(W * 4), so_rm, so_rm, HW);
                 wino_epilogue<NCB, 0, 0, false, 1, 3>(acc, bias2, floor_v, r1, r1, st_rm, st_rm + (unsigned)(W * 4), so_rm, so_rm, HW);
                 cur = nxt;
@@ -515,7 +536,7 @@
             const __amdgpu_buffer_rsrc_t rm =
                 __builtin_amdgcn_make_buffer_rsrc(const_cast<float*>(EM == 1 ? a.emask + (long long)b * a.emask_bs : a.y), 0, y_img, 0x00020000);
             unsigned* wb = (EM == 2 || EM == 3) ? a.wbits + (((long long)b * (H >> 1) + (ty * (WN_TH / 2) + (cur & 7))) * tiles_x + tx) * 64 + lane : nullptr;
-            wino_epilogue<NCB, EM == 1 ? 1 : 0, EM == 2 ? 2 : (EM == 3 ? 1 : 0), EM == 4>(acc, bias2, floor_v, ry, rm, st0, st1, so_t, so_t, HW, 0, wb);
+            wino_epilogue<NCB, EM == 1 ? 1 : 0, EM == 2 ? 2 : (EM == 3 ? 1 : 0), EM == 4>(acc, bias2, floor_v, ry, rm, st0, st1, so_t, so_t, HW, 0, wb, nullptr, bdp, bd_vo, bd_l4);
         }
         cur = nxt;
         if (cur < total_units) nxt = next_unit();
@@ -1475,7 +1496,7 @@
 
 static int wino_launch_any(const float* src, long long src_bs, const float* u, const float* bias, float* dst, long long dst_bs, const float* emask,
                            long long emask_bs, int cin, int cout, int B, int H, int W, int relu, void* stream, const char* what, unsigned* wbits = nullptr,
-                           bool wbits_apply = false, bool s2d = false, float* dst2 = nullptr, long long dst2_bs = 0, int split_mode = 0) {
+                           bool wbits_apply = false, bool s2d = false, float* dst2 = nullptr, long long dst2_bs = 0, int split_mode = 0, float* border = nullptr) {
     YNET_REQUIRE(src && u && dst, "%s: null pointer", what);
     YNET_REQUIRE(wino_shape_ok(B, H, W, cin, cout, 3), "%s: shape B=%d %dx%d %d -> %d is not served (ask ynet_conv2d_winograd_supported)", what, B, H, W, cin,
                  cout);
@@ -1488,10 +1509,13 @@
         YNET_REQUIRE(cout == 48 && dst2 != nullptr && (reinterpret_cast<uintptr_t>(dst2) & 7) == 0 && (dst2_bs & 1) == 0 && dst2_bs >= 32 * HW && bias == nullptr && !relu &&
                          wbits == nullptr && !s2d,
                      "%s: two destinations are for the plain 48-channel data gradient (16 + 32 planes, 8-byte aligned)", what);
+    if (border != nullptr)
+        YNET_REQUIRE((s2d || split_mode == 2) && (reinterpret_cast<uintptr_t>(border) & 15) == 0, "%s: the border copy belongs to a space-to-depth destination and is 16-byte aligned", what);
     if (emask != nullptr)
         YNET_REQUIRE((reinterpret_cast<uintptr_t>(emask) & 7) == 0 && (emask_bs & 1) == 0 && emask_bs >= cout * HW,
                      "%s: the activation must be 8-byte aligned, its batch stride not smaller than the image", what);
     WinoArgs a{src, reinterpret_cast<const f32x4*>(u), bias, dst, src_bs, dst_bs, B, H, W, relu ? 1 : 0, B * (H / WN_TH) * (W / WN_TW), emask, emask_bs, wbits, dst2, dst2_bs};
+    a.border = border;
     hipStream_t st = (hipStream_t)stream;
     if (wbits != nullptr) {
         YNET_REQUIRE(cout == 32 && emask == nullptr && (reinterpret_cast<uintptr_t>(wbits) & 3) == 0, "%s: the 1-bit mask serves 32 output channels and excludes the float mask", what);
@@ -1524,6 +1548,12 @@
 
 int ynet_conv2d_winograd_s2d(const float* src, long long src_bs, const float* u, float* dst, long long dst_bs, int cin, int cout, int B, int H, int W, void* stream) {
     return wino_launch_any(src, src_bs, u, nullptr, dst, dst_bs, nullptr, 0, cin, cout, B, H, W, 0, stream, "conv2d_winograd_s2d", nullptr, false, true);
+}
+
+int ynet_conv2d_winograd_s2d_border(const float* src, long long src_bs, const float* u, float* dst, long long dst_bs, float* border, int cin, int cout, int B, int H, int W,
+                                    void* stream) {
+    return wino_launch_any(src, src_bs, u, nullptr, dst, dst_bs, nullptr, 0, cin, cout, B, H, W, 0, stream, "conv2d_winograd_s2d_border", nullptr, false, true, nullptr, 0, 0,
+                           border);
 }
 
 int ynet_conv2d_winograd_pred_bce_supported(int B, int H, int W, int cin, int cout, int pred_cout, int kernlen) {
@@ -1570,6 +1600,12 @@
                                int B, int H, int W, void* stream) {
     return wino_launch_any(src, src_bs, u, nullptr, dst0, dst0_bs, nullptr, 0, cin, 48, B, H, W, 0, stream, "conv2d_winograd_split", nullptr, false, false, dst1, dst1_bs,
                            dst0_s2d ? 2 : 1);
+}
+
+int ynet_conv2d_winograd_split_border(const float* src, long long src_bs, const float* u, float* dst0, long long dst0_bs, float* dst0_border, float* dst1, long long dst1_bs,
+                                      int cin, int B, int H, int W, void* stream) {
+    return wino_launch_any(src, src_bs, u, nullptr, dst0, dst0_bs, nullptr, 0, cin, 48, B, H, W, 0, stream, "conv2d_winograd_split_border", nullptr, false, false, dst1, dst1_bs,
+                           2, dst0_border);
 }
 
 long long ynet_winograd_relu_bits_words(int B, int H, int W) {
diff --git a/motion-style-transfer_amd/csrc/glue.hip b/motion-style-transfer_amd/csrc/glue.hip
--- a/motion-style-transfer_amd/csrc/glue.hip
+++ b/motion-style-transfer_amd/csrc/glue.hip
@@ -1270,7 +1270,8 @@
 }
 
 #define RING_SEG 64
-__global__ __launch_bounds__(256) void upconv_ring_kernel(const float* __restrict__ D, long long d_bs, const float* __restrict__ tab, const float* __restrict__ relu_of,
+__global__ __launch_bounds__(256) void upconv_ring_kernel(const float* __restrict__ D, long long d_bs, const float* __restrict__ S, const float* __restrict__ tab,
+                                                          const float* __restrict__ relu_of,
                                                           long long relu_bs, float* __restrict__ dx, long long dx_bs, int B, int C4, int cin, int h, int w,
                                                           int nseg_row, int nseg_col) {
     extern __shared__ float ring_smem[];
@@ -1291,9 +1292,29 @@
     const int tid = threadIdx.x;
     const float* tsrc = tab + (long long)((is_row ? 0 : 6) + side * 3) * tstride;
     for (int i = tid; i < 3 * C4 * cin; i += 256) T[i] = tsrc[i];
-    for (int i = tid; i < C4 * (RING_SEG + 2); i += 256) {
-        const int c = i / (RING_SEG + 2), k = i - c * (RING_SEG + 2), q = q0 - 1 + k;
-        Dt[i] = (q >= 0 && q < len) ? Db[c * hw + (is_row ? (long long)fixed * w + q : (long long)q * w + fixed)] : 0.f;
+    if (!is_row && S != nullptr) {
+        const float* Sl = S + ((long long)b * 2 + side) * C4 * h;
+        if ((h & 3) == 0) {
+            constexpr int NG = (RING_SEG + 2 + 3) / 4;
+            for (int i = tid; i < C4 * NG; i += 256) {
+                const int c = i / NG, g = i - c * NG, q = q0 - 1 + 4 * g;
+                const f32x4 v = q < h ? *reinterpret_cast<const f32x4*>(Sl + (long long)c * h + q) : f32x4{0.f, 0.f, 0.f, 0.f};
+                float* dst = Dt + c * (RING_SEG + 2) + 4 * g;
+                dst[0] = v[0];
+                dst[1] = v[1];
+                if (4 * g + 2 < RING_SEG + 2) { dst[2] = v[2]; dst[3] = v[3]; }
+            }
+        } else {
+            for (int i = tid; i < C4 * (RING_SEG + 2); i += 256) {
+                const int c = i / (RING_SEG + 2), k = i - c * (RING_SEG + 2), q = q0 - 1 + k;
+                Dt[i] = q < h ? Sl[(long long)c * h + q] : 0.f;
+            }
+        }
+    } else {
+        for (int i = tid; i < C4 * (RING_SEG + 2); i += 256) {
+            const int c = i / (RING_SEG + 2), k = i - c * (RING_SEG + 2), q = q0 - 1 + k;
+            Dt[i] = (q >= 0 && q < len) ? Db[c * hw + (is_row ? (long long)fixed * w + q : (long long)q * w + fixed)] : 0.f;
+        }
     }
     __syncthreads();
     const int lane = tid & 63, wv = tid >> 6, m = lane & 15, kq = lane >> 4;
@@ -1324,6 +1345,7 @@
         if (jc < q0 || jc >= q0 + RING_SEG) continue;
         const float* tcol = tab + (long long)(6 + corner * 3) * tstride;
         const float* tx = tab + (long long)(12 + side * 2 + corner) * tstride;
+        const float* Sc = S != nullptr ? S + ((long long)b * 2 + corner) * C4 * h : nullptr;
         const int nterm = 4 * C4;
         for (int ci0 = 0; ci0 < cin; ci0 += 32) {
             const int ci = ci0 + (tid & 31);
@@ -1333,9 +1355,9 @@
                 float d = 0.f;
                 if (t < 3) {
                     const int ii = fixed - t + 1;
-                    if (ii >= 0 && ii < h) d = Db[c * hw + (long long)ii * w + jc] * tcol[((long long)t * C4 + c) * cin + ci];
+                    if (ii >= 0 && ii < h) d = (Sc ? Sc[(long long)c * h + ii] : Db[c * hw + (long long)ii * w + jc]) * tcol[((long long)t * C4 + c) * cin + ci];
                 } else {
-                    d = Db[c * hw + (long long)fixed * w + jc] * tx[(long long)c * cin + ci];
+                    d = (Sc ? Sc[(long long)c * h + fixed] : Db[c * hw + (long long)fixed * w + jc]) * tx[(long long)c * cin + ci];
                 }
                 part += d;
             }
@@ -1733,8 +1755,9 @@
     return ynet_check_launch("relu_bwd");
 }
 
-int ynet_upconv_dgrad_ring(const float* D, long long d_bs, const float* tables, const float* relu_of, long long relu_of_bs, float* dx, long long dx_bs,
-                           int B, int C4, int cin, int h, int w, void* stream) {
+int ynet_upconv_dgrad_ring_border(const float* D, long long d_bs, const float* border, const float* tables, const float* relu_of, long long relu_of_bs, float* dx,
+                                  long long dx_bs, int B, int C4, int cin, int h, int w, void* stream) {
+    YNET_REQUIRE((reinterpret_cast<uintptr_t>(border) & 15) == 0, "upconv_dgrad_ring: the border copy must be 16-byte aligned");
     YNET_REQUIRE(D && tables && dx && B > 0 && C4 > 0 && (C4 & 3) == 0 && cin > 0 && h >= 2 && w >= 2, "upconv_dgrad_ring: bad arguments (C4 = 4 cout)");
     YNET_REQUIRE(d_bs >= (long long)C4 * h * w && dx_bs >= (long long)cin * h * w && (relu_of == nullptr || relu_of_bs >= (long long)cin * h * w),
                  "upconv_dgrad_ring: batch strides smaller than the images");
@@ -1743,9 +1766,14 @@
     const int nseg_row = (w + RING_SEG - 1) / RING_SEG, nseg_col = h > 2 ? (h - 2 + RING_SEG - 1) / RING_SEG : 0;
     const long long blocks = (long long)B * (2 * nseg_row + 2 * nseg_col);
     YNET_REQUIRE(blocks < (1ll << 31), "upconv_dgrad_ring: too many workgroups");
-    hipLaunchKernelGGL(upconv_ring_kernel, dim3((unsigned)blocks), dim3(256), lds, (hipStream_t)stream, D, d_bs, tables, relu_of, relu_of_bs, dx, dx_bs, B, C4, cin, h, w,
+    hipLaunchKernelGGL(upconv_ring_kernel, dim3((unsigned)blocks), dim3(256), lds, (hipStream_t)stream, D, d_bs, border, tables, relu_of, relu_of_bs, dx, dx_bs, B, C4, cin, h, w,
                        nseg_row, nseg_col);
     return ynet_check_launch("upconv_dgrad_ring");
+}
+
+int ynet_upconv_dgrad_ring(const float* D, long long d_bs, const float* tables, const float* relu_of, long long relu_of_bs, float* dx, long long dx_bs,
+                           int B, int C4, int cin, int h, int w, void* stream) {
+    return ynet_upconv_dgrad_ring_border(D, d_bs, nullptr, tables, relu_of, relu_of_bs, dx, dx_bs, B, C4, cin, h, w, stream);
 }
 
 int ynet_rot90_flip(const void* src, void* dst, long long N, int H, int W, int k, int flip, void* stream) {
diff --git a/motion-style-transfer_amd/ops.py b/motion-style-transfer_amd/ops.py
--- a/motion-style-transfer_amd/ops.py
+++ b/motion-style-transfer_amd/ops.py
@@ -337,12 +337,16 @@
     return u
 
 
+def _s2d_border_arg(s2d):
+    return int(s2d) if (s2d and s2d is not True) else None
+
+
 def conv2d_winograd_raw(src, u, bias, dst, cin, cout, B, H, W, relu, relu_of=None, wbits_out=None, relu_wbits=None, s2d=False):
     lib = _lib()
     if s2d:
         if bias is not None or relu or relu_of is not None or wbits_out is not None or relu_wbits is not None:
             raise ValueError("conv2d_winograd_raw: s2d is for a plain data gradient")
-        L.check(lib.ynet_conv2d_winograd_s2d(src[0], src[1], u.data_ptr(), dst[0], dst[1], cin, cout, B, H, W, _stream()), lib)
+        L.check(lib.ynet_conv2d_winograd_s2d_border(src[0], src[1], u.data_ptr(), dst[0], dst[1], _s2d_border_arg(s2d), cin, cout, B, H, W, _stream()), lib)
         return
     if wbits_out is not None:
         if cout != 32 or not relu or relu_of is not None or relu_wbits is not None:
@@ -374,6 +378,9 @@
 
 def conv2d_winograd_split_raw(src, u, dst0, dst0_s2d, dst1, cin, B, H, W):
     lib = _lib()
+    if _s2d_border_arg(dst0_s2d) is not None:
+        L.check(lib.ynet_conv2d_winograd_split_border(src[0], src[1], u.data_ptr(), dst0[0], dst0[1], _s2d_border_arg(dst0_s2d), dst1[0], dst1[1], cin, B, H, W, _stream()), lib)
+        return
     L.check(lib.ynet_conv2d_winograd_split(src[0], src[1], u.data_ptr(), dst0[0], dst0[1], 1 if dst0_s2d else 0, dst1[0], dst1[1], cin, B, H, W, _stream()), lib)
 
 
@@ -484,7 +491,7 @@
 
 
 def conv2d_auto_raw(srcs, mask, wp, bias, dsts, B, H, W, K, relu, relu_of=None, pooled=None, bits_out=None, relu_bits=None, wino=None, wbits_out=None,
-                    relu_wbits=None, pool_code=None, addend=None, upsample2x=False, wp_version=1, dst_s2d=None):
+                    relu_wbits=None, pool_code=None, addend=None, upsample2x=False, wp_version=1, dst_s2d=None, dst_border=None):
     lib = _lib()
     d = L.ConvAuto()
     d.nsrc, d.ndst = len(srcs), len(dsts)
@@ -495,6 +502,8 @@
         d.dst[i], d.dst_c[i], d.dst_bs[i] = t_[0], t_[1], t_[2]
         if dst_s2d is not None and dst_s2d[i]:
             d.dst_s2d[i] = 1
+            if dst_border is not None and dst_border[i] is not None:
+                d.dst_border[i] = dst_border[i]
     if mask:
         d.mask, d.mask_bs = mask[0], mask[1]
     d.wp, d.bias = wp.data_ptr(), (bias.data_ptr() if bias is not None else None)
@@ -572,22 +581,22 @@
 
 
 def conv2d_raw(srcs, mask, wp, bias, dsts, B, H, W, K, relu, relu_of=None, pooled=None, bits_out=None, relu_bits=None, wino=None, wbits_out=None,
-               relu_wbits=None, pool_code=None, dst_s2d=None, info=None):
+               relu_wbits=None, pool_code=None, dst_s2d=None, info=None, dst_border=None):
     if not conv_auto:
         return _conv2d_raw_py(srcs, mask, wp, bias, dsts, B, H, W, K, relu, relu_of=relu_of, pooled=pooled, bits_out=bits_out, relu_bits=relu_bits, wino=wino,
-                              wbits_out=wbits_out, relu_wbits=relu_wbits, pool_code=pool_code, dst_s2d=dst_s2d, info=info)
+                              wbits_out=wbits_out, relu_wbits=relu_wbits, pool_code=pool_code, dst_s2d=dst_s2d, info=info, dst_border=dst_border)
     if wino is not None and not torch.is_grad_enabled() and (
             H * W < _wino_eval_min_hw or not (_wino_plain_eval if len(srcs) == 1 and srcs[0][1] in (16, 32) else _wino_cat_eval)):
         wino = None
     tag, tk = conv2d_auto_raw(srcs, mask, wp, bias, dsts, B, H, W, K, relu, relu_of=relu_of, pooled=pooled, bits_out=bits_out, relu_bits=relu_bits, wino=wino,
-                              wbits_out=wbits_out, relu_wbits=relu_wbits, pool_code=pool_code, dst_s2d=dst_s2d)
+                              wbits_out=wbits_out, relu_wbits=relu_wbits, pool_code=pool_code, dst_s2d=dst_s2d, dst_border=dst_border)
     if info is not None:
         info["wrote_s2d"] = int(tk.wrote_s2d)
     return tag
 
 
 def _conv2d_raw_py(srcs, mask, wp, bias, dsts, B, H, W, K, relu, relu_of=None, pooled=None, bits_out=None, relu_bits=None, wino=None, wbits_out=None,
-                   relu_wbits=None, pool_code=None, dst_s2d=None, info=None):
+                   relu_wbits=None, pool_code=None, dst_s2d=None, info=None, dst_border=None):
     lib = _lib()
     sp, sc, sb = _arrays(srcs)
     if info is not None:
@@ -668,7 +677,8 @@
                 ent = cache[key] = _wino_made((wp, winograd_filter(wp, cin, 48, col0, ctot)))
             _wino_ready(ent)
             s2d = bool(dst_s2d and dst_s2d[piece_dst[0][0]])
-            conv2d_winograd_split_raw((srcs[0][0], srcs[0][2]), ent[1], (pieces[0][0], pieces[0][2]), s2d, (pieces[1][0], pieces[1][2]), cin, B, H, W)
+            bord = dst_border[piece_dst[0][0]] if (s2d and dst_border is not None) else None
+            conv2d_winograd_split_raw((srcs[0][0], srcs[0][2]), ent[1], (pieces[0][0], pieces[0][2]), bord if bord is not None else s2d, (pieces[1][0], pieces[1][2]), cin, B, H, W)
             if s2d and info is not None:
                 info["wrote_s2d"] |= 1 << piece_dst[0][0]
             wino_stats["launches"] += 1
@@ -690,7 +700,8 @@
                     ent = cache[key] = _wino_made((wp, winograd_filter(wp, cin, n, col0, ctot)))
                 _wino_ready(ent)
                 conv2d_winograd_raw((srcs[0][0], srcs[0][2]), ent[1], None if bias is None else bias[col0:col0 + n], (ptr, bs), cin, n, B, H, W, relu,
-                                    relu_of=None if wb_in is not None else relu_of, wbits_out=wb_out, relu_wbits=wb_in, **({"s2d": True} if s2d else {}))
+                                    relu_of=None if wb_in is not None else relu_of, wbits_out=wb_out, relu_wbits=wb_in,
+                                    **({"s2d": dst_border[di] if (dst_border is not None and dst_border[di] is not None) else True} if s2d else {}))
                 if s2d and info is not None:
                     info["wrote_s2d"] |= 1 << di
                 wino_stats["launches"] += 1
@@ -1006,6 +1017,7 @@
         _premasked.clear()
         _s2d_wanted.clear()
         _s2d_grads.clear()
+        _s2d_borders.clear()
         _s2d_produced.clear()
         _deferred.clear()
         _unmaterialized.clear()
@@ -1019,6 +1031,7 @@
         _premasked.clear()
         _s2d_wanted.clear()
         _s2d_grads.clear()
+        _s2d_borders.clear()
         _s2d_produced.clear()
         _deferred.clear()
         _unmaterialized.clear()
@@ -1177,6 +1190,8 @@
                     dsts.append((None, c, 0))
                     want_s2d.append(False)
             s2d_info = {} if any(want_s2d) else None
+            borders = [torch.empty((B, 2, 4 * d_srcs[i].shape[1], H // 2), device=dy.device, dtype=torch.float32) if (f_ and _upconv_border_allowed) else None
+                       for i, f_ in enumerate(want_s2d)] if s2d_info is not None else None
             s0 = srcs[0]
             emask = None
             if (premask and ctx.n_src == 1 and need_src[0] and _is_relu_output(s0) and s0.is_contiguous() and s0.shape[0] == B
@@ -1204,11 +1219,14 @@
                 if ewbits is not None:
                     premask_stats["wino_bit_masks"] = premask_stats.get("wino_bit_masks", 0) + 1
                 conv2d_raw([(dy.data_ptr(), cout, cout * H * W)], mask, wp_d, None, dsts, B, H, W, k, False, relu_of=emask,
-                           wino=(cache, "dgrad") if meta.get("wino") else None, relu_wbits=ewbits, dst_s2d=want_s2d if s2d_info is not None else None, info=s2d_info)
+                           wino=(cache, "dgrad") if meta.get("wino") else None, relu_wbits=ewbits, dst_s2d=want_s2d if s2d_info is not None else None, info=s2d_info,
+                           dst_border=[t_.data_ptr() if t_ is not None else None for t_ in borders] if borders is not None else None)
                 if s2d_info:
                     for i, g_ in enumerate(d_srcs):
                         if g_ is not None and (s2d_info.get("wrote_s2d", 0) >> i) & 1:
                             _s2d_grads[g_.data_ptr()] = (g_._version, tuple(g_.shape))
+                            if borders[i] is not None:
+                                _s2d_borders[g_.data_ptr()] = borders[i]
                             _s2d_wanted.pop(srcs[i].data_ptr(), None)
                             _s2d_produced.add(srcs[i].data_ptr())
             if emask is not None:
@@ -1567,6 +1585,8 @@
 _upconv_s2d_allowed = _os.environ.get("YNET_UPCONV_S2D", "1") != "0"
 _s2d_wanted = {}
 _s2d_grads = {}
+_s2d_borders = {}
+_upconv_border_allowed = _os.environ.get("YNET_UPCONV_BORDER", "1") != "0"
 _conv_pred_bce_allowed = _os.environ.get("YNET_CONV_PRED_BCE", "1") != "0"
 _deferred = {}
 _unmaterialized = {}
@@ -1624,6 +1644,9 @@
     if relu_of is not None:
         d.relu_of, d.relu_of_bs = relu_of, cin * hw
     d.wp = weight.data_ptr()
+    border = _s2d_borders.get(D)
+    if border is not None and tuple(border.shape) == (B, 2, 4 * cout, h):
+        d.src_border = border.data_ptr()
     d.B, d.H, d.W, d.K = B, h, w, 3
     d.flags = _auto_flags(wino) | L.AUTO_UPCONV_BWD
     need = lib.ynet_conv2d_auto_cache_floats(ctypes.byref(d))
@@ -1713,6 +1736,8 @@
         dy = dy.contiguous()
         reg = _s2d_grads.pop(dy.data_ptr(), None)
         handed = reg is not None and reg == (dy._version, tuple(dy.shape))
+        if not handed:
+            _s2d_borders.pop(dy.data_ptr(), None)
         if ctx.y_ptr in _s2d_produced:
             _s2d_produced.discard(ctx.y_ptr)
             if not handed:
@@ -1731,8 +1756,10 @@
                 conv2d_raw([(dy.data_ptr(), 4 * cout, 4 * cout * Hl * Wl)], None, wp_eff, None, [(dx.data_ptr(), cin, cin * Hl * Wl)], B, Hl, Wl, 3, False,
                            relu_of=(x.data_ptr(), cin * Hl * Wl) if masked else None, wino=(wcache, "dgrad"))
                 lib = _lib()
-                L.check(lib.ynet_upconv_dgrad_ring(dy.data_ptr(), 4 * cout * Hl * Wl, tables.data_ptr(), x.data_ptr() if masked else None, cin * Hl * Wl, dx.data_ptr(),
-                                                   cin * Hl * Wl, B, 4 * cout, cin, Hl, Wl, _stream()), lib)
+                border = _s2d_borders.get(dy.data_ptr())
+                L.check(lib.ynet_upconv_dgrad_ring_border(dy.data_ptr(), 4 * cout * Hl * Wl, border.data_ptr() if border is not None else None, tables.data_ptr(),
+                                                          x.data_ptr() if masked else None, cin * Hl * Wl, dx.data_ptr(), cin * Hl * Wl, B, 4 * cout, cin, Hl, Wl, _stream()), lib)
+            _s2d_borders.pop(dy.data_ptr(), None)
             if masked:
                 _premasked[dx.data_ptr()] = (x.data_ptr(), dx._version, tuple(dx.shape))
             upconv_stats_s2d["backwards"] += 1
```
